# fskovbo/OptimalControlMPS

Hardware: AMD Instinct MI355X
Metric: Hessian-rows/sec (getHessian incl. psi/xi/divT/xiH precompute), N=5 d=4 chi=80 T=2.0 (higher is better)
Workload: dtype c128/f64

## Files before the change

### optimalcontrolmps_amd/csrc/fast.hpp

```cpp
#pragma once

namespace ocg {
namespace fastp {

constexpr int kMaxOps = 16;
constexpr int kMaxDm = 4;
constexpr int kMaxDot = 16;
constexpr int kMaxGram = 4;
constexpr int kItTh = 2;
constexpr int kItF = 4;
constexpr int kItS = 4;
constexpr int kItMps = 4;

enum {
  kHNp = 0,
  kHNblk,
  kHBlk,
  kHLs,
  kHSite,
  kHSiteN,
  kHNops,
  kHZMps,
  kHZTh,
  kHZTg,
  kHZW,
  kHZX,
  kHZGt,
  kHZPh,
  kHZTot,
  kHNint,
  kHCentre,
  kHThZ,
  kHXsZ,
  kHOps,
  kHdrInts = kHOps + kMaxOps
};
enum { kOpGate = 0, kOpGaugeR = 1, kOpGaugeL = 2 };
enum {
  kOhKind = 0, kOhK, kOhDir, kOhMode,
  kOhLonely, kOhClosing, kOhNth, kOhNewBond,
  kOhMat,
  kOhGate,
  kOhNsec, kOhT,
  kOhNgrp, kOhMaxr,
  kOhO1, kOhNo1,
  kOhEq,
  kOhSecQ,
  kOhF, kOhNf,
  kOhS, kOhNs,
  kOhDot,
  kOhGrp = 24,
  kOpHdr = kOhGrp + 32
};

static_assert(kOhGrp % 4 == 0 && kOhNewBond < 8, "b128 reads of the op header");

constexpr int kOvMaxE = 128;
constexpr int kOvMaxP = 6;
enum {
  kOvL = 0, kOvQ1, kOvP, kOvNp, kOvNblk,
  kOvMaxSite,
  kOvMaxEn,
  kOvD,
  kOvEo,
  kOvEn,
  kOvPo,
  kOvSb,
  kOvElo,
  kOvEl,
  kOvLs,
  kOvBlk,
  kOvNint,
  kOvHdr = 20
};
}
}
```

### optimalcontrolmps_amd/csrc/fast_chain.hpp

```cpp
#pragma once

#include "engine_device.hpp"
#include "fast.hpp"

namespace ocg {

struct FastChain {
  using CH = Chain<64>;
  const OcgParams& P;
  const int lane;
  const bool act;
  lzp MP, TH, TG, WB, XS, GT, PH;
  LDS double *LAM, *SIG, *SIGI, *MCB, *MCF;
  LDS int* MCE;
  LDS int *DIM, *BOF, *KQ, *WIDX, *PL;
  int np, nblk, o_blk, o_ls, o_site, o_siten, nops, centre_open;
  int thz, xsz;
  double ph_u = __builtin_nan("");
  int ph_dir = -1;
  int dims_epoch = 0, bof_epoch = -1;
  int trace_op = -1;
  double m_bytes = 0, m_flops = 0;
  LDS double* PROF = nullptr;
  unsigned long long pf_last = 0;
  int pf_cur = 0;
  __device__ __forceinline__ void pf(int cat) {
#ifdef OCG_PROFILE
    if (threadIdx.x == 0 && PROF) {
      const unsigned long long t = __builtin_amdgcn_s_memtime();
      if (pf_last) PROF[pf_cur] += double(t - pf_last);
      pf_last = t;
      pf_cur = cat;
    }
#else
    (void)cat;
#endif
  }
  __device__ __forceinline__ void cnt(int slot, double v) {
#ifdef OCG_PROFILE
    if (threadIdx.x == 0 && PROF) PROF[slot] += v;
#else
    (void)slot;
    (void)v;
#endif
  }

  __device__ OCG_INLINE FastChain(const OcgParams& P_, char* base, const int* gplan, LDS double* prof = nullptr)
      : P(P_), lane(threadIdx.x & 63), act(threadIdx.x < 64), PROF(prof) {
    using namespace fastp;
    if (!gplan) return;
    np = gplan[kHNp]; nblk = gplan[kHNblk]; o_blk = gplan[kHBlk]; o_ls = gplan[kHLs]; o_site = gplan[kHSite];
    o_siten = gplan[kHSiteN]; nops = gplan[kHNops]; centre_open = gplan[kHCentre];
    thz = gplan[kHThZ]; xsz = gplan[kHXsZ];
    lzp cb{(LDS double*)base};
    MP = cb + gplan[kHZMps]; TH = cb + gplan[kHZTh]; TG = cb + gplan[kHZTg]; WB = cb + gplan[kHZW];
    XS = cb + gplan[kHZX]; GT = cb + gplan[kHZGt]; PH = cb + gplan[kHZPh];
    LDS double* db = (cb + gplan[kHZTot]).p;
    LAM = db; SIG = db + 64; SIGI = db + 128;
    MCB = db + 200; MCF = db + 200 + fastp::kMaxOps;
    LDS int* ib = (LDS int*)(db + 200 + 2 * fastp::kMaxOps);
    MCE = ib; ib += fastp::kMaxOps;
    auto al = [](int x) { return (x + 3) & ~3; };
    DIM = ib; ib += al(P.nsq);
    BOF = ib; ib += al(nblk);
    KQ = ib; ib += 64;
    WIDX = ib; ib += 64;
    ib += 4;
    PL = ib;
  }
  __device__ __forceinline__ void wsync() const {
    __builtin_amdgcn_fence(__ATOMIC_RELEASE, "workgroup");
    __builtin_amdgcn_wave_barrier();
    __builtin_amdgcn_fence(__ATOMIC_ACQUIRE, "workgroup");
  }
  __device__ __forceinline__ static i4 ld4(const LDS int* p) { return *(const LDS i4*)p; }
  __device__ __forceinline__ static int uni(int v) { return __builtin_amdgcn_readfirstlane(v); }
  __device__ OCG_INLINE void init(const int* gplan, const zc* gf, const zc* gb) {
    if (!act) return;
    const int ni = gplan[fastp::kHNint];
    for (int i = lane; i < ni; i += 64) PL[i] = gplan[i];
    for (int i = lane; i < P.gtotal; i += 64) { GT[i] = gf[i]; GT[P.gtotal + i] = gb[i]; }
    if (lane < fastp::kMaxOps) MCE[lane] = -1;
    if (lane == 0) {
      WB[64] = c2(1.0, 0.0);
      MP[np] = c2(0.0, 0.0);
      TH[thz] = c2(0.0, 0.0);
      TG[thz] = c2(0.0, 0.0);
      XS[xsz] = c2(0.0, 0.0);
    }
    wsync();
  }
  __device__ __forceinline__ int dim(int b, int q) const { return (q < 0 || q > P.Q) ? 0 : DIM[b * P.Q1 + q]; }

  __device__ OCG_INLINE void block_offsets() {
    if (bof_epoch == dims_epoch) return;
    int carry = 0;
    for (int b0 = 0; b0 < nblk; b0 += 64) {
      const int b = b0 + lane, bb = b < nblk ? b : nblk - 1;
      const i4 t = ld4(PL + o_blk + 4 * bb);
      const int sz = b < nblk ? DIM[t[1]] * DIM[t[2]] : 0;
      const int inc = wscan(sz);
      if (b < nblk) BOF[b] = carry + inc - sz;
      carry += rdlane(inc, 63);
    }
    bof_epoch = dims_epoch;
    wsync();
  }
  template <class PI, class PZ>
  __device__ OCG_INLINE void load(const PI* gdims, const PZ* gdata) {
    if (!act) return;
    pf(10);
    for (int i = lane; i < P.nsq; i += 64) DIM[i] = gdims[i];
    ++dims_epoch;
    wsync();
    block_offsets();
    i4 d[fastp::kItMps];
#pragma unroll
    for (int it = 0; it < fastp::kItMps; ++it) {
      const int x = lane + 64 * it;
      d[it] = ld4(PL + o_ls + 4 * (x < np ? x : np - 1));
    }
#pragma unroll
    for (int it = 0; it < fastp::kItMps; ++it) {
      const int x = lane + 64 * it;
      const int dl = DIM[d[it][0] & 0xffff], dr = DIM[unsigned(d[it][0]) >> 16];
      const int b = d[it][1] & 0xffff, f = unsigned(d[it][1]) >> 16, a = d[it][2] & 0xff, c = unsigned(d[it][2]) >> 8;
      const bool ok = x < np && a < dl && c < dr;
      const int idx = d[it][3] + BOF[b] - BOF[f] + a * dr + c;
      zc v = c2(0.0, 0.0);
      if (ok) v = c2(gdata[idx].x, gdata[idx].y);
      if (x < np) MP[x] = v;
    }
    wsync();
  }
  __device__ OCG_INLINE void store(int* gdims, zc* gdata, bool wt = false) {
    if (!act) return;
    pf(10);
    block_offsets();
    for (int i = lane; i < P.nsq; i += 64) {
      if (wt) __hip_atomic_store(gdims + i, DIM[i], __ATOMIC_RELAXED, __HIP_MEMORY_SCOPE_AGENT);
      else gdims[i] = DIM[i];
    }
    i4 d[fastp::kItMps];
#pragma unroll
    for (int it = 0; it < fastp::kItMps; ++it) {
      const int x = lane + 64 * it;
      d[it] = ld4(PL + o_ls + 4 * (x < np ? x : np - 1));
    }
#pragma unroll
    for (int it = 0; it < fastp::kItMps; ++it) {
      const int x = lane + 64 * it;
      const int dl = DIM[d[it][0] & 0xffff], dr = DIM[unsigned(d[it][0]) >> 16];
      const int b = d[it][1] & 0xffff, f = unsigned(d[it][1]) >> 16, a = d[it][2] & 0xff, c = unsigned(d[it][2]) >> 8;
      const int idx = d[it][3] + BOF[b] - BOF[f] + a * dr + c;
      const zc v = MP[x < np ? x : 0];
      if (x < np && a < dl && c < dr) {
        if (wt) {
          double* dd = (double*)(gdata + idx);
          __hip_atomic_store(dd, v.x, __ATOMIC_RELAXED, __HIP_MEMORY_SCOPE_AGENT);
          __hip_atomic_store(dd + 1, v.y, __ATOMIC_RELAXED, __HIP_MEMORY_SCOPE_AGENT);
        } else {
          gdata[idx] = v;
        }
      }
    }
  }

  __device__ OCG_INLINE void model_totals(double& b, double& f) const {
    b = wsum(m_bytes);
    f = wsum(m_flops);
  }
  __device__ OCG_INLINE void model_gate(int o, int i1) {
    using namespace fastp;
    if (uni(MCE[o]) == dims_epoch) {
      if (lane == 0) {
        m_bytes += MCB[o];
        m_flops += MCF[o];
      }
      return;
    }
    const int p = P.p, Q = P.Q, Q1 = P.Q1, q = lane < Q1 ? lane : 0;
    const LDS int* d0 = DIM + (i1 - 1) * Q1;
    const LDS int* d1 = DIM + i1 * Q1;
    const LDS int* d2 = DIM + (i1 + 1) * Q1;
    int l[6], a[6], r[6];
#pragma unroll
    for (int n = 0; n < 6; ++n) {
      const int qm = q - n, qp = q + n;
      const bool okm = n < p && qm >= 0, okp = n < p && qp <= Q;
      const int lm = d0[okm ? qm : 0], ap = d1[okp ? qp : 0], rp = d2[okp ? qp : 0];
      l[n] = okm ? lm : 0;
      a[n] = okp ? ap : 0;
      r[n] = okp ? rp : 0;
    }
    int R = 0, C = 0, u = 0;
    const int m = a[0], dl = l[0];
#pragma unroll
    for (int n = 0; n < 6; ++n) {
      R += l[n];
      C += r[n];
      u += dl * a[n] + m * r[n];
    }
    double fl = 0.0, by = 0.0;
    if (lane < Q1) {
      if (R == 0 || C == 0) { R = 0; C = 0; }
      const double Rd = R, Cd = C, nn = R < C ? R : C;
      fl = 8.0 * (Rd * Cd * m + Rd * Cd * p + nn * nn * (R > C ? Rd : Cd) + 2.0 * Rd * Cd * m);
      by = 32.0 * double(u);
    }
    if (lane == 0) by += 16.0 * P.gtotal;
    const double bt = wsum(by), ft = wsum(fl);
    if (lane == 0) {
      m_bytes += bt;
      m_flops += ft;
      MCB[o] = bt;
      MCF[o] = ft;
      MCE[o] = dims_epoch;
    }
  }

  __device__ OCG_INLINE void theta(const LDS int* oh) {
    using namespace fastp;
    pf(0);
    const int nth = uni(oh[kOhNth]);
    if (nth <= 64) theta_it<1>(oh, nth);
    else theta_it<kItTh>(oh, nth);
    wsync();
  }
  template <int IT>
  __device__ OCG_INLINE void theta_it(const LDS int* oh, int nth) {
    using namespace fastp;
    const LDS int* md = PL + uni(oh[kOhMat]);
    int d0[IT], d1[IT];
#pragma unroll
    for (int it = 0; it < IT; ++it) {
      const int e = lane + 64 * it, ee = e < nth ? e : nth - 1;
      d0[it] = md[2 * ee];
      d1[it] = md[2 * ee + 1];
    }
#pragma unroll
    for (int it = 0; it < IT; ++it) {
      const int e = lane + 64 * it;
      const int x1 = d0[it] & 0xffff, x2 = unsigned(d0[it]) >> 16, dm = d1[it] & 0xff, drc = unsigned(d1[it]) >> 8;
      const int dmc = dm > 0 ? dm - 1 : 0;
      zc acc = c2(0.0, 0.0);
#pragma unroll
      for (int b = 0; b < kMaxDm; ++b) {
        const int bb = b < dmc ? b : dmc;
        const zc a = MP[b < dm ? x1 + b : np], v = MP[x2 + bb * drc];
        cacc(acc, a, v);
      }
      if (e < nth) TH[e] = acc;
    }
  }
  __device__ OCG_INLINE void gate(const LDS int* oh, int forward) {
    using namespace fastp;
    pf(1);
    const int mode = uni(oh[kOhMode]), lonely = uni(oh[kOhLonely]);
    if (uni(oh[kOhNth]) <= 64) gate_mode<1>(oh, forward, mode, lonely);
    else gate_mode<kItTh>(oh, forward, mode, lonely);
    wsync();
  }
  template <int IT>
  __device__ OCG_INLINE void gate_mode(const LDS int* oh, int forward, int mode, int lonely) {
    if (mode == 0) {
      if (lonely & 1) gate_body<1, 2, IT>(oh, forward);
      else gate_body<1, 0, IT>(oh, forward);
    } else {
      if (lonely & 2) gate_body<2, 1, IT>(oh, forward);
      else gate_body<0, 1, IT>(oh, forward);
    }
  }
  template <int PRE, int POST, int IT>
  __device__ OCG_INLINE void gate_body(const LDS int* oh, int forward) {
    using namespace fastp;
    const int p = P.p, nth = uni(oh[kOhNth]);
    const LDS int* gd = PL + uni(oh[kOhGate]);
    lzp g0 = GT + (forward ? 0 : P.gtotal);
    lzp UF = PH, UT = PH + p, UFF = PH + 2 * p, UTT = PH + 2 * p + p * p;
    i4 d[IT];
#pragma unroll
    for (int it = 0; it < IT; ++it) {
      const int e = lane + 64 * it;
      d[it] = ld4(gd + 4 * (e < nth ? e : nth - 1));
    }
#pragma unroll
    for (int it = 0; it < IT; ++it) {
      const int e = lane + 64 * it;
      const unsigned h = d[it][0];
      const int sz = (h >> 16) & 15, lo = (h >> 20) & 15, a1 = (h >> 24) & 15, a2 = h >> 28, D = a1 + a2;
      lzp g = g0 + int(h & 0xffff);
      zc acc = c2(0.0, 0.0);
#pragma unroll
      for (int x = 0; x < 6; ++x) {
        const int xx = x < sz ? x : sz - 1;
        const int n1 = lo + xx, n2 = D - n1;
        const int ad = (unsigned(d[it][1 + (x >> 1)]) >> (16 * (x & 1))) & 0xffff;
        zc z = TH[x < sz ? ad : thz];
        if (PRE == 1) z = cmul(z, UFF[n1 * p + n2]);
        if (PRE == 2) z = cmul(z, UF[n2]);
        const zc gx = g[xx];
        cacc(acc, gx, z);
      }
      if (POST == 1) acc = cmul(acc, UTT[a1 * p + a2]);
      if (POST == 2) acc = cmul(acc, UT[a2]);
      if (e < nth) TG[e] = acc;
    }
  }
  __device__ OCG_INLINE void matcopy(const LDS int* oh) {
    using namespace fastp;
    pf(7);
    const int nth = uni(oh[kOhNth]);
    if (nth <= 64) matcopy_it<1>(oh, nth);
    else matcopy_it<kItTh>(oh, nth);
    wsync();
  }
  template <int IT>
  __device__ OCG_INLINE void matcopy_it(const LDS int* oh, int nth) {
    using namespace fastp;
    const LDS int* src = PL + uni(oh[kOhMat]);
    int s[IT];
#pragma unroll
    for (int it = 0; it < IT; ++it) {
      const int e = lane + 64 * it;
      s[it] = src[e < nth ? e : nth - 1];
    }
#pragma unroll
    for (int it = 0; it < IT; ++it) {
      const int e = lane + 64 * it;
      const zc v = MP[s[it]];
      if (e < nth) TH[e] = v;
    }
  }

  __device__ OCG_INLINE void decompose(const LDS int* oh, lzp M, int dir, double cutoff, int maxm, bool normalize) {
    using namespace fastp;
    pf(2);
    const i4 h2 = ld4(oh + 8), h3 = ld4(oh + 12), h4 = ld4(oh + 16), h5 = ld4(oh + 20);
    const int newb = uni(oh[kOhNewBond]);
    const int nsec = uni(h2[kOhNsec - 8]), T = uni(h2[kOhT - 8]), maxr = uni(h3[kOhMaxr - 12]),
              no1 = uni(h3[kOhNo1 - 12]), o_o1 = uni(h3[kOhO1 - 12]), o_eq = uni(h4[kOhEq - 16]),
              o_secq = uni(h4[kOhSecQ - 16]), o_f = uni(h4[kOhF - 16]), nf = uni(h4[kOhNf - 16]),
              dot = uni(h5[kOhDot - 20]);
    const int g = lane >> 4, i = (lane >> 2) & 3, j = lane & 3, rb = lane & ~15;
    const i4 ga = ld4(oh + kOhGrp + 8 * g), gb = ld4(oh + kOhGrp + 8 * g + 4);
    const i4 o1 = ld4(PL + o_o1 + 4 * (lane < no1 ? lane : 0));
    const bool ae = lane < T;
    const i4 eq = ld4(PL + o_eq + 4 * (ae ? lane : 0));
    const int sqe = PL[o_secq + (lane < nsec ? lane : 0)];
    const int at_q = newb * P.Q1 + (sqe & 255);
    const int dold = DIM[at_q];
    const bool used = ga[0] >= 0;
    const int n = used ? ga[1] : 0, side = ga[2], tho = ga[3], R = gb[0], C = gb[1], eoff = gb[2];
    const bool valid = i < n && j < n;
    zc gv = c2(0.0, 0.0);
    double lam1 = 0.0;
    {
      const int len = used ? (side == 0 ? C : R) : 0, st = side == 0 ? 1 : C;
      const int bi = side == 0 ? tho + (i < n ? i : 0) * C : tho + (i < n ? i : 0);
      const int bj = side == 0 ? tho + (j < n ? j : 0) * C : tho + (j < n ? j : 0);
      const int len1 = lane < no1 ? o1[1] : 0, b1 = o1[0], s1 = o1[2];
      switch ((dot + 1) >> 1) {
        case 0: case 1: gram_dots<2>(M, len, st, bi, bj, len1, b1, s1, gv, lam1); break;
        case 2: gram_dots<4>(M, len, st, bi, bj, len1, b1, s1, gv, lam1); break;
        case 3: gram_dots<6>(M, len, st, bi, bj, len1, b1, s1, gv, lam1); break;
        case 4: gram_dots<8>(M, len, st, bi, bj, len1, b1, s1, gv, lam1); break;
        case 5: gram_dots<10>(M, len, st, bi, bj, len1, b1, s1, gv, lam1); break;
        case 6: gram_dots<12>(M, len, st, bi, bj, len1, b1, s1, gv, lam1); break;
        case 7: gram_dots<14>(M, len, st, bi, bj, len1, b1, s1, gv, lam1); break;
        default: gram_dots<kMaxDot>(M, len, st, bi, bj, len1, b1, s1, gv, lam1); break;
      }
      if (side == 1) gv.y = -gv.y;
    }
    if (!valid) gv = c2(0.0, 0.0);
    zc w = c2(i == j ? 1.0 : 0.0, 0.0);
    pf(3);
    if (maxr > 0) jacobi(gv, w, valid, i, j, rb, n, maxr);
    cnt(22, 1.0);
    pf(4);
    if (used) WB[16 * g + 4 * i + j] = w;
    if (valid && i == j) LAM[eoff + i] = gv.x > 0 ? gv.x : 0.0;
    if (lane < no1) LAM[o1[3]] = lam1;
    wsync();
    const double lam = ae ? LAM[lane] : 0.0;
    const int i_e = eq[1], eo_e = eq[2], n_e = eq[3] & 255, bound = unsigned(eq[3]) >> 8;
    double lt[kMaxGram];
#pragma unroll
    for (int t = 0; t < kMaxGram; ++t) lt[t] = CH::bperm(lam, ((eo_e + t) & 63) << 2);
    int jb = 0;
#pragma unroll
    for (int t = 0; t < kMaxGram; ++t)
      jb += (ae & (t < n_e) & (t != i_e) & ((lt[t] > lam) | ((lt[t] == lam) & (t < i_e)))) ? 1 : 0;
    const double total = wsum(lam);
    const double cut = cutoff * total, floor_ = 1e-30 * total;
    bool disc = false;
    if (T <= maxm) {
      const double thr = fmax(cut, floor_);
      const bool small = ae && (lam < thr || lam <= floor_);
      unsigned long long Mk = __ballot(small);
      pf(18);
      cnt(17, __popcll(Mk));
      if (Mk) {
        const int nbig = T - __popcll(Mk);
        double S = lam;
        int rs = 0;
        while (Mk) {
          const int f = __ffsll((long long)Mk) - 1;
          Mk &= Mk - 1;
          const double lf = rdlane(lam, f);
          rs += (lf > lam || (lf == lam && f < lane)) ? 1 : 0;
          if (f != lane && (lf < lam || (lf == lam && f > lane))) S += lf;
        }
        disc = small && nbig + rs >= 1 && (S < cut || lam <= floor_);
      }
    } else {
      int rk = 0;
      for (int f = 0; f < T; ++f) {
        const double lf = rdlane(lam, f);
        rk += (lf > lam || (lf == lam && f < lane)) ? 1 : 0;
      }
      const int dst = ((T - 1 - rk) & 63) << 2;
      const long long lb = __double_as_longlong(lam);
      const unsigned lo = unsigned(__builtin_amdgcn_ds_permute(dst, int(lb)));
      const unsigned hi = unsigned(__builtin_amdgcn_ds_permute(dst, int(lb >> 32)));
      const double v = __longlong_as_double((long long)(((unsigned long long)hi << 32) | lo));
      const int jpos = T - 1 - lane;
      const double vv = lane < T ? v : 0.0;
      const double suf = wscan(vv);
      const bool d2 = lane < T && jpos >= 1 && (jpos >= maxm || suf < cut || vv <= floor_);
      const int m = T - __popcll(__ballot(d2));
      disc = ae && rk >= m;
    }
    pf(16);
    const bool kept = ae && !disc && jb < bound;
    if (kept) {
      const double sq = sqrt(lam);
      WIDX[eo_e + jb] = i_e;
      SIG[eo_e + jb] = sq;
      SIGI[eo_e + jb] = sq > 0 ? 1.0 / sq : 0.0;
    }
    const double kw = wsum(kept ? lam : 0.0);
    {
      const unsigned long long K = __ballot(kept);
      const int eo = (sqe >> 8) & 255, ns = (sqe >> 16) & 15;
      const int kq = __popcll((K >> eo) & ((1ull << ns) - 1));
      bool changed = false;
      if (lane < nsec) {
        changed = dold != kq;
        KQ[lane] = kq;
        DIM[at_q] = kq;
      }
      if (__ballot(changed)) ++dims_epoch;
    }
    wsync();
    pf(5);
    const double inv = (normalize && kw > 1e-32) ? 1.0 / sqrt(kw) : 1.0;
    if (nf <= 64) factors<1>(o_f, nf, M, dir, inv);
    else if (nf <= 128) factors<2>(o_f, nf, M, dir, inv);
    else if (nf <= 192) factors<3>(o_f, nf, M, dir, inv);
    else factors<kItF>(o_f, nf, M, dir, inv);
  }

  template <int IF>
  __device__ OCG_INLINE void factors(int o_f, int nf, lzp M, int dir, double inv) {
    using namespace fastp;
    i4 fd[IF];
#pragma unroll
    for (int it = 0; it < IF; ++it) {
      const int e = lane + 64 * it;
      fd[it] = ld4(PL + o_f + 4 * (e < nf ? e : nf - 1));
    }
    int kqs[IF], wvv[IF];
    double sg[IF], isg[IF];
    zc mv[IF][kMaxGram];
#pragma unroll
    for (int it = 0; it < IF; ++it) {
      const int w0 = fd[it][0], w1 = fd[it][1], w2 = fd[it][2];
      const int s = (w0 >> 16) & 15, jj = (w0 >> 20) & 15, eo = w2 & 255;
      const bool exact = (w2 >> 12) & 1;
      const int mb = w1 & 0xffff, terms = (w1 >> 16) & 31, ms = unsigned(w1) >> 21;
      kqs[it] = KQ[s];
      wvv[it] = WIDX[eo + jj];
      sg[it] = SIG[eo + jj];
      isg[it] = SIGI[eo + jj];
#pragma unroll
      for (int x = 0; x < kMaxGram; ++x) mv[it][x] = M[(exact || x >= terms) ? thz : mb + x * ms];
    }
    zc out[IF];
    int dst[IF];
#pragma unroll
    for (int it = 0; it < IF; ++it) {
      const int e = lane + 64 * it;
      const int w0 = fd[it][0], w1 = fd[it][1], w2 = fd[it][2], wbse = fd[it][3];
      const int dest = w0 & 0xffff, jj = (w0 >> 20) & 15;
      const bool isx = (w0 >> 24) & 1, scr = (w0 >> 25) & 1;
      const bool exact = (w2 >> 12) & 1;
      const int terms = exact ? 1 : (w1 >> 16) & 31;
      const int tc = terms > 0 ? terms - 1 : 0;
      const bool live = jj < kqs[it] && e < nf;
      const int wvc = live ? wvv[it] : 0;
      const int base = exact ? w1 : wbse;
      const double cs = isx ? 1.0 : -1.0;
      zc wp[kMaxGram];
#pragma unroll
      for (int x = 0; x < kMaxGram; ++x) {
        const zc t = WB[base + 4 * (x < tc ? x : tc) + wvc];
        wp[x] = c2(t.x, cs * t.y);
      }
      zc acc = c2(0.0, 0.0);
#pragma unroll
      for (int x = 0; x < kMaxGram; ++x) cacc(acc, mv[it][x], wp[x]);
      const double sig = sg[it];
      const zc we = wp[0];
      const bool scl = isx ? dir == kFromright : dir == kFromleft;
      const bool orth = isx ? dir == kFromleft : dir == kFromright;
      const double f = exact ? (scl ? sig * inv : 1.0) : (orth ? (sig > 0 ? isg[it] : 0.0) : inv);
      const zc r = cscale(exact ? we : acc, f);
      out[it] = live ? r : c2(0.0, 0.0);
      dst[it] = e < nf ? (dest | (scr ? 0x10000 : 0)) : -1;
    }
    pf(23);
#pragma unroll
    for (int it = 0; it < IF; ++it)
      if (dst[it] >= 0) ((dst[it] >> 16) ? XS : MP)[dst[it] & 0xffff] = out[it];
    wsync();
  }

  template <int K>
  __device__ __forceinline__ void gram_dots(lzp M, int len, int st, int bi, int bj, int len1, int b1, int s1, zc& gv,
                                            double& lam1) const {
    zc a[K], b[K], z[K];
#pragma unroll
    for (int c = 0; c < K; ++c) {
      const bool in = c < len, in1 = c < len1;
      a[c] = M[in ? bi + c * st : thz];
      b[c] = M[in ? bj + c * st : thz];
      z[c] = M[in1 ? b1 + c * s1 : thz];
    }
#pragma unroll
    for (int c = 0; c < K; ++c) {
      cacc(gv, a[c], cconj(b[c]));
      lam1 += cabs2(z[c]);
    }
  }

  __device__ __forceinline__ void jrot_role(zc bv, double app, double aqq, bool live, bool up, zc& jd, zc& jo,
                                            double& ds) const {
    const double mb = fmax(fabs(bv.x), fabs(bv.y)), sz = fabs(app) + fabs(aqq);
    const bool resc = live && (mb < 1e-120 || mb > 1e120 || sz > 1e120);
    double sc = 1.0;
    if (__ballot(resc)) {
      sc = resc ? ldexp(1.0, -ilogb(fmax(mb, sz))) : 1.0;
      bv = cscale(bv, sc);
      app *= sc;
      aqq *= sc;
    }
    const double r2 = live ? bv.x * bv.x + bv.y * bv.y : 1.0;
    const double rinv = CH::rsq_ref(r2), r = r2 * rinv;
    const double D = aqq - app, sg = D >= 0 ? 1.0 : -1.0;
    const double x = fma(D, D, 4.0 * r2);
    const double E = fabs(D) + x * CH::rsq_ref(x);
    const double h = CH::rsq_ref(fma(E, E, 4.0 * r2));
    const double c = E * h, s = sg * 2.0 * r * h;
    const double ex = bv.x * rinv, ey = bv.y * rinv;
    const double sh = sg * 2.0 * r2 * CH::rcp_ref(E * sc);
    jd = up ? c2(c, 0.0) : c2(ex * c, -ey * c);
    jo = up ? c2(ex * -s, -ey * -s) : c2(s, 0.0);
    ds = up ? -sh : sh;
    jd = live ? jd : c2(1.0, 0.0);
    jo = live ? jo : c2(0.0, 0.0);
    ds = live ? ds : 0.0;
  }

  __device__ OCG_INLINE void jacobi(zc& g, zc& w, bool valid, int i, int j, int rb, int n, int maxr) {
    auto at = [&](int r, int c) { return (rb + r * 4 + c) << 2; };
    double di = CH::bperm(g.x, at(i, i)), dj = CH::bperm(g.x, at(j, j));
    int arow[3], acol[3];
    bool zp[3];
#pragma unroll
    for (int rnd = 0; rnd < 3; ++rnd) {
      const int k = rnd + 1;
      int pi = i, pj = j;
      if (rnd < maxr && valid) {
        if ((i ^ k) < n) pi = i ^ k;
        if ((j ^ k) < n) pj = j ^ k;
      }
      arow[rnd] = at(i, pi);
      acol[rnd] = at(j, pj);
      zp[rnd] = pi == j && i != j;
    }
    const bool up = i < j, dg = i == j;
    int sweep = 0, nr = 0;
    bool done = false;
    for (; sweep < 40; ++sweep) {
      bool flag = false;
#pragma unroll
      for (int rnd = 0; rnd < 3; ++rnd) {
        if (rnd >= maxr) break;
        if (__ballot(valid && up && CH::jneed(cabs2(g), di, dj)) == 0) {
          done = true;
          break;
        }
        ++nr;
        const zc g01 = CH::xcol(g, rnd), g10 = CH::xrow(g, rnd);
        const zc g11 = CH::xrow(g01, rnd), w1 = CH::xcol(w, rnd);
        const zc bv = up ? g : g11;
        const double app = up ? di : dj, aqq = up ? dj : di;
        const bool need = CH::jneed(cabs2(bv), app, aqq);
        zc jd, jo;
        double ds;
        jrot_role(bv, app, aqq, need && !dg, up, jd, jo, ds);
        const zc jdc = CH::bpermz(jd, acol[rnd]), joc = CH::bpermz(jo, acol[rnd]);
        const zc jdr = CH::bpermz(jd, arow[rnd]), jor = CH::bpermz(jo, arow[rnd]);
        const double dsc = CH::bperm(ds, acol[rnd]), dsr = CH::bperm(ds, arow[rnd]);
        zc wn = cmul(w, jdc);
        cacc(wn, w1, joc);
        zc r0 = cmul(g, jdc);
        cacc(r0, g01, joc);
        zc r1 = cmul(g10, jdc);
        cacc(r1, g11, joc);
        zc out = cjmul(jdr, r0);
        cjacc(out, jor, r1);
        const double dj2 = dj + dsc, di2 = di + dsr;
        out = (zp[rnd] && need) ? c2(0.0, 0.0) : out;
        out = dg ? c2(dj2, 0.0) : out;
        if (rnd == maxr - 1) flag = valid && up && CH::jneed(cabs2(out), di2, dj2);
        g = out;
        w = wn;
        di = di2;
        dj = dj2;
      }
      if (done || __ballot(flag) == 0) break;
    }
    if (sweep == 40 && lane == 0 && P.err) atomicOr(P.err, OCG_ERR_JACOBI);
    cnt(21, 1.0);
    cnt(20, double(sweep + 1));
    cnt(30, double(nr));
#ifdef OCG_FAST_TRACE
    if (lane == 0) printf("[jacobi] op %d sweeps %d rounds %d\n", trace_op, sweep + 1, nr);
#endif
  }

  __device__ OCG_INLINE void neighbour(const LDS int* oh) {
    using namespace fastp;
    pf(25);
    const int ns = uni(oh[kOhNs]), kind = uni(oh[kOhKind]);
    if (ns <= 64) neighbour_it<1>(oh, ns, kind);
    else if (ns <= 128) neighbour_it<2>(oh, ns, kind);
    else neighbour_it<kItS>(oh, ns, kind);
  }
  template <int IT>
  __device__ OCG_INLINE void neighbour_it(const LDS int* oh, int ns, int kind) {
    using namespace fastp;
    const LDS int* sl = PL + uni(oh[kOhS]);
    i4 d[IT];
#pragma unroll
    for (int it = 0; it < IT; ++it) {
      const int e = lane + 64 * it;
      d[it] = ld4(sl + 4 * (e < ns ? e : ns - 1));
    }
    zc acc[IT];
#pragma unroll
    for (int it = 0; it < IT; ++it) {
      const int x1 = d[it][0] & 0xffff, x2 = unsigned(d[it][0]) >> 16, len = d[it][1] & 0xffff,
                s2 = unsigned(d[it][1]) >> 16;
      const int lc = len > 0 ? len - 1 : 0;
      acc[it] = c2(0.0, 0.0);
#pragma unroll
      for (int b = 0; b < kMaxDm; ++b) {
        const int bb = b < lc ? b : lc;
        const bool in = b < len;
        const zc a = (kind == kOpGaugeR) ? zc(XS[in ? x1 + b : xsz]) : zc(MP[in ? x1 + b : np]);
        const zc v = (kind == kOpGaugeR) ? zc(MP[x2 + bb * s2]) : zc(XS[x2 + bb * s2]);
        cacc(acc[it], a, v);
      }
    }
    wsync();
#pragma unroll
    for (int it = 0; it < IT; ++it)
      if (lane + 64 * it < ns) MP[d[it][2]] = acc[it];
    wsync();
  }

  __device__ __forceinline__ static void sincos_q(double x, double& s, double& c) {
    constexpr double s3 = -1.0 / 6.0, s5 = 1.0 / 120.0, s7 = -1.0 / 5040.0, s9 = 1.0 / 362880.0,
                     s11 = -1.0 / 39916800.0, s13 = 1.0 / 6227020800.0, s15 = -1.0 / 1307674368000.0,
                     s17 = 1.0 / 355687428096000.0;
    constexpr double c2_ = -0.5, c4 = 1.0 / 24.0, c6 = -1.0 / 720.0, c8 = 1.0 / 40320.0, c10 = -1.0 / 3628800.0,
                     c12 = 1.0 / 479001600.0, c14 = -1.0 / 87178291200.0, c16 = 1.0 / 20922789888000.0;
    const double z = x * x;
    const double ps = fma(z, fma(z, fma(z, fma(z, fma(z, fma(z, fma(z, s17, s15), s13), s11), s9), s7), s5), s3);
    const double pc = fma(z, fma(z, fma(z, fma(z, fma(z, fma(z, fma(z, c16, c14), c12), c10), c8), c6), c4), c2_);
    s = fma(x * z, ps, x);
    c = fma(z, pc, 1.0);
  }

  __device__ OCG_INLINE void step(double ufrom, double uto, int forward, bool final_gauge = true) {
    using namespace fastp;
    if (!act) return;
    pf(29);
    const int p = P.p;
    const double tau = forward ? P.dt : -P.dt;
    {
      const double ta = -0.25 * tau;
      const int a = lane / p, b = lane - a * p;
      const double n1 = lane < p ? double(lane) * double(lane - 1) : 0.0;
      const double n2 = lane < p * p ? double(a) * double(a - 1) + double(b) * double(b - 1) : 0.0;
      const double xf1 = ta * ufrom * n1, xt1 = ta * uto * n1, xf2 = ta * ufrom * n2, xt2 = ta * uto * n2;
      const bool big = fmax(fmax(fabs(xf1), fabs(xt1)), fmax(fabs(xf2), fabs(xt2))) > 0.78;
      double sf1, cf1, st1, ct1, sf2, cf2, st2, ct2;
      if (__ballot(big) == 0) {
        sincos_q(xf1, sf1, cf1);
        sincos_q(xt1, st1, ct1);
        sincos_q(xf2, sf2, cf2);
        sincos_q(xt2, st2, ct2);
      } else {
        sincos(xf1, &sf1, &cf1);
        sincos(xt1, &st1, &ct1);
        sincos(xf2, &sf2, &cf2);
        sincos(xt2, &st2, &ct2);
      }
      if (lane < p) {
        PH[lane] = c2(cf1, sf1);
        PH[p + lane] = c2(ct1, st1);
      }
      if (lane < p * p) {
        PH[2 * p + lane] = c2(cf2, sf2);
        PH[2 * p + p * p + lane] = c2(ct2, st2);
      }
    }
    ph_u = uto;
    ph_dir = forward;
    wsync();
    for (int o = 0; o < nops; ++o) {
      const LDS int* oh = PL + PL[kHOps + o];
      const i4 h0 = ld4(oh), h1 = ld4(oh + 4);
      if (uni(h1[1]) && !final_gauge) continue;
      const int kind = uni(h0[0]), dir = uni(h0[2]);
      trace_op = o;
      if (kind == kOpGate) {
        pf(12);
        model_gate(o, uni(h0[1]));
        theta(oh);
        gate(oh, forward);
        decompose(oh, TG, dir, P.cutoff, P.maxm, true);
      } else {
        matcopy(oh);
        decompose(oh, TH, dir, OCG_GAUGE_CUTOFF, 1 << 30, false);
        neighbour(oh);
      }
    }
    pf(9);
    const int centre = final_gauge ? 1 : centre_open;
    const int s1a = PL[o_site + 1], s1b = PL[o_site + 2];
    for (int x = s1a + lane; x < s1b; x += 64) MP[x] = cmul(MP[x], PH[p + PL[o_siten + x - s1a]]);
    wsync();
    const int ca = PL[o_site + centre], cb = PL[o_site + centre + 1];
    double acc = 0.0;
    zc v[kItMps];
#pragma unroll
    for (int it = 0; it < kItMps; ++it) {
      const int x = ca + lane + 64 * it;
      v[it] = MP[x < cb ? x : ca];
      if (x < cb) acc += cabs2(v[it]);
    }
    const double n2 = wsum(acc);
    if (n2 > 0) {
      const double f = 1.0 / sqrt(n2);
#pragma unroll
      for (int it = 0; it < kItMps; ++it) {
        const int x = ca + lane + 64 * it;
        if (x < cb) MP[x] = cscale(v[it], f);
      }
    }
    wsync();
  }
};

}
```

### optimalcontrolmps_amd/csrc/fast_plan.hpp

```cpp
#pragma once

#include <algorithm>
#include <cstdio>
#include <cstdlib>
#include <string>
#include <vector>

#include "engine.hpp"
#include "fast.hpp"

namespace ocg_host {

struct FastPlanBuild {
  std::vector<int> plan;
  std::string why_not;
};

inline FastPlanBuild build_fast_plan(const OcgParams& P, const std::vector<int>& md) {
  using namespace ocg::fastp;
  FastPlanBuild out;
  const int L = P.L, p = P.p, Q = P.Q, Q1 = P.Q1;
  auto fail = [&](const std::string& m) {
    out.plan.clear();
    out.why_not = m;
    return out;
  };
  if (P.imag) return fail("imaginary-time steps use the general engine");
  if (p > 6) return fail("local dimension above 6");
  if (Q1 > 64) return fail("more than 64 sectors");
  auto D = [&](int b, int q) { return (b < 0 || b > L || q < 0 || q > Q) ? 0 : md[size_t(b) * Q1 + q]; };
  for (int b = 0; b <= L; ++b)
    for (int q = 0; q <= Q; ++q)
      if (D(b, q) > kMaxDm) return fail("bond sector bound above the unrolled maximum");
  std::vector<int> I(kHdrInts, 0);
  auto pad = [&]() {
    while (I.size() & 3) I.push_back(0);
    return int(I.size());
  };
  auto push4 = [&](int a, int b, int c, int d) { I.push_back(a); I.push_back(b); I.push_back(c); I.push_back(d); };
  std::vector<int> poff(size_t(L + 2) * Q1 * p, -1), sbase(L + 2, 0);
  int np = 0;
  std::vector<int> blk_k, blk_q, blk_n;
  for (int k = 1; k <= L; ++k) {
    sbase[k] = np;
    for (int q = 0; q <= Q; ++q)
      for (int n = 0; n < p && q + n <= Q; ++n) {
        const int dl = D(k - 1, q), dr = D(k, q + n);
        if (dl == 0 || dr == 0) continue;
        poff[(size_t(k) * Q1 + q) * p + n] = np;
        blk_k.push_back(k); blk_q.push_back(q); blk_n.push_back(n);
        np += dl * dr;
      }
  }
  sbase[L + 1] = np;
  if (np > 64 * kItMps) return fail("padded MPS above the unrolled maximum");
  auto PO = [&](int k, int q, int n) {
    return (k < 1 || k > L || q < 0 || q > Q || n < 0 || n >= p) ? -1 : poff[(size_t(k) * Q1 + q) * p + n];
  };
  const int nblk = int(blk_k.size());
  if (nblk > 4095) return fail("too many blocks");
  std::vector<int> first(nblk);
  for (int b = 0; b < nblk; ++b) {
    first[b] = b;
    while (first[b] > 0 && blk_k[first[b] - 1] == blk_k[b]) --first[b];
  }
  const int o_blk = pad();
  for (int b = 0; b < nblk; ++b) {
    const int k = blk_k[b], q = blk_q[b], n = blk_n[b];
    push4(k | (q << 8) | (n << 16), (k - 1) * Q1 + q, k * Q1 + q + n, first[b]);
  }
  const int o_ls = pad();
  for (int b = 0; b < nblk; ++b) {
    const int k = blk_k[b], q = blk_q[b], n = blk_n[b];
    for (int a = 0; a < D(k - 1, q); ++a)
      for (int c = 0; c < D(k, q + n); ++c)
        push4(((k - 1) * Q1 + q) | ((k * Q1 + q + n) << 16), b | (first[b] << 16), a | (c << 8), P.site_base[k]);
  }
  const int o_site = pad();
  for (int k = 0; k <= L + 1; ++k) I.push_back(sbase[k]);
  const int o_siten = pad();
  for (int b = 0; b < nblk; ++b)
    if (blk_k[b] == 1)
      for (int x = 0; x < D(0, blk_q[b]) * D(1, blk_q[b] + blk_n[b]); ++x) I.push_back(blk_n[b]);

  struct Op { int kind, k, dir, mode, lonely, closing; };
  std::vector<Op> ops;
  {
    int centre = 1;
    bool mfl = true;
    for (int g = 0; g < P.ngates; ++g) {
      const int i1 = P.gate_i1[g], i2 = i1 + 1;
      const bool more = g + 1 < P.ngates;
      const int ni1 = more ? P.gate_i1[g + 1] : 0, ni2 = ni1 + 1;
      const int dir = (more && ni1 >= i2) ? 0 : 1;
      Op o{kOpGate, i1, dir, mfl ? 0 : 1, 0, 0};
      if (mfl) o.lonely = (i2 == L && L % 2 == 0) ? 1 : 0;
      else o.lonely = (L % 2 != 0 && i2 == L) ? 2 : 0;
      ops.push_back(o);
      centre = dir == 0 ? i2 : i1;
      const int target = !more ? 1 : (dir == 0 ? ni1 : ni2);
      while (centre != target) {
        if (centre < target) { ops.push_back({kOpGaugeR, centre, 0, 0, 0, more ? 0 : 1}); ++centre; }
        else { ops.push_back({kOpGaugeL, centre, 1, 0, 0, more ? 0 : 1}); --centre; }
      }
      if (more && (i2 == ni1 || i1 == ni2)) mfl = false;
    }
  }
  if (int(ops.size()) > kMaxOps) return fail("too many step operations");
  int thmax = 1, xsmax = 1, last_gate = 0;
  std::vector<int> op_off;
  for (const Op& o : ops) {
    if (o.kind == kOpGate) last_gate = o.k;
    int bl, br, prow, pcol;
    if (o.kind == kOpGate) { bl = o.k - 1; br = o.k + 1; prow = p; pcol = p; }
    else if (o.kind == kOpGaugeR) { bl = o.k - 1; br = o.k; prow = p; pcol = 1; }
    else { bl = o.k - 1; br = o.k; prow = 1; pcol = p; }
    const int newb = (o.kind == kOpGaugeL) ? o.k - 1 : o.k;
    std::vector<int> R(Q1, 0), C(Q1, 0), THO(Q1 + 1, 0);
    std::vector<std::vector<int>> RS(Q1, std::vector<int>(p, -1)), CS(Q1, std::vector<int>(p, -1));
    for (int q = 0; q <= Q; ++q) {
      for (int n = 0; n < prow; ++n) {
        const int d = D(bl, q - n);
        if (d > 0) { RS[q][n] = R[q]; R[q] += d; }
      }
      for (int n = 0; n < pcol; ++n) {
        const int d = D(br, q + n);
        if (d > 0) { CS[q][n] = C[q]; C[q] += d; }
      }
      if (R[q] == 0 || C[q] == 0) { R[q] = 0; C[q] = 0; }
      THO[q + 1] = THO[q] + R[q] * C[q];
    }
    const int nth = THO[Q1];
    thmax = std::max(thmax, nth);
    if (nth > 64 * kItTh) return fail("matricisation above the unrolled maximum");
    const int hpos = pad();
    op_off.push_back(hpos);
    I.resize(I.size() + kOpHdr, 0);
    auto setH = [&](int f, int v) { I[hpos + f] = v; };
    setH(kOhKind, o.kind); setH(kOhK, o.k); setH(kOhDir, o.dir); setH(kOhMode, o.mode);
    setH(kOhLonely, o.lonely); setH(kOhClosing, o.closing); setH(kOhNth, nth); setH(kOhNewBond, newb);
    setH(kOhMat, pad());
    for (int q = 0; q <= Q; ++q) {
      if (R[q] == 0) continue;
      for (int nr = 0; nr < prow; ++nr) {
        if (RS[q][nr] < 0) continue;
        for (int a = 0; a < D(bl, q - nr); ++a)
          for (int nc = 0; nc < pcol; ++nc) {
            if (CS[q][nc] < 0) continue;
            for (int c = 0; c < D(br, q + nc); ++c) {
              if (o.kind == kOpGate) {
                const int dm = D(o.k, q);
                const int x1 = dm > 0 ? PO(o.k, q - nr, nr) + a * dm : 0;
                const int drc = D(o.k + 1, q + nc);
                const int x2 = dm > 0 ? PO(o.k + 1, q, nc) + c : 0;
                I.push_back(x1 | (x2 << 16));
                I.push_back(dm | (drc << 8));
              } else if (o.kind == kOpGaugeR) {
                I.push_back(PO(o.k, q - nr, nr) + a * D(o.k, q) + c);
              } else {
                I.push_back(PO(o.k, q, nc) + a * D(o.k, q + nc) + c);
              }
            }
          }
      }
    }
    if (o.kind == kOpGate) {
      setH(kOhGate, pad());
      for (int q = 0; q <= Q; ++q) {
        if (R[q] == 0) continue;
        for (int a1 = 0; a1 < p; ++a1) {
          if (RS[q][a1] < 0) continue;
// ... 11 lines not shown
                    return fail("internal: gate input outside Θ");
                  const int ad = THO[qs] + (RS[qs][n1] + a) * C[qs] + CS[qs][n2] + c;
                  if (ad > 65535) return fail("Θ offset above 16 bits");
                  w[1 + x / 2] |= ad << (16 * (x & 1));
                }
                push4(w[0], w[1], w[2], w[3]);
              }
            }
        }
      }
    }
    std::vector<int> sq, secn(Q1, 0), seco(Q1, -1), secside(Q1, 0), secgrp(Q1, -1), seceoff(Q1, 0);
    int ngrp = 0, T = 0, maxn = 0;
    for (int q = 0; q <= Q; ++q) {
      if (R[q] == 0) continue;
      const int n = std::min(R[q], C[q]);
      if (n > kMaxGram) return fail("Gram block above the register Jacobi's order");
      if (std::max(R[q], C[q]) > kMaxDot) return fail("Gram dot product above the unrolled maximum");
      int grp = -1;
      if (n >= 2) {
        if (ngrp >= 4) return fail("more than four Gram blocks of order >= 2");
        grp = ngrp++;
      }
      seco[q] = int(sq.size());
      int side = R[q] < C[q] ? 0 : (R[q] > C[q] ? 1 : 0);
      if (R[q] == C[q] && o.kind == kOpGaugeR) side = 1;
      secn[q] = n; secside[q] = side; secgrp[q] = grp; seceoff[q] = T;
      sq.push_back(q);
      T += n;
      maxn = std::max(maxn, n);
    }
    const int nsec = int(sq.size());
    int maxdot = 1;
    for (int q : sq) maxdot = std::max(maxdot, std::max(R[q], C[q]));
    setH(kOhDot, maxdot);
    if (nsec > 15) return fail("more than 15 sectors");
    if (T > 64) return fail("more than 64 eigenvalues per decomposition");
    setH(kOhNsec, nsec); setH(kOhT, T); setH(kOhNgrp, ngrp);
    setH(kOhMaxr, maxn >= 3 ? 3 : (maxn == 2 ? 1 : 0));
    for (int g = 0; g < 4; ++g) I[hpos + kOhGrp + 8 * g] = -1;
    for (int s = 0; s < nsec; ++s) {
      const int q = sq[s], g = secgrp[q];
      if (g < 0) continue;
      int* G = &I[hpos + kOhGrp + 8 * g];
      G[0] = s; G[1] = secn[q]; G[2] = secside[q]; G[3] = THO[q]; G[4] = R[q]; G[5] = C[q]; G[6] = seceoff[q];
    }
    setH(kOhO1, pad());
    int no1 = 0;
    for (int s = 0; s < nsec; ++s) {
      const int q = sq[s];
      if (secn[q] != 1) continue;
      const bool rowv = secside[q] == 0;
      push4(THO[q], rowv ? C[q] : R[q], rowv ? 1 : C[q], seceoff[q]);
      ++no1;
    }
    setH(kOhNo1, no1);
    if (no1 > 64) return fail("too many order-1 sectors");
    setH(kOhEq, pad());
    for (int s = 0; s < nsec; ++s) {
      const int q = sq[s];
      for (int i = 0; i < secn[q]; ++i) push4(s, i, seceoff[q], secn[q] | (D(newb, q) << 8));
    }
    setH(kOhSecQ, pad());
    for (int s = 0; s < nsec; ++s) I.push_back(sq[s] | (seceoff[sq[s]] << 8) | (secn[sq[s]] << 16));
    std::vector<int> XS_off(Q1, 0), YS_off(Q1, 0);
    int xs_tot = 0, ys_tot = 0, nf = 0;
    setH(kOhF, pad());
    bool ok = true;
    auto pushf = [&](int dest, int q, int j, bool isx, bool scratch, int idx) {
      const int s = seco[q], n = secn[q], side = secside[q], g = secgrp[q];
      const bool exact = isx ? side == 0 : side == 1;
      const int wb = g >= 0 ? 16 * g : 64;
      int w1;
      if (exact) {
        w1 = wb + (g >= 0 ? 4 * idx : 0);
      } else if (isx) {
        w1 = (THO[q] + idx * C[q]) | (n << 16) | (1 << 21);
      } else {
        w1 = (THO[q] + idx) | (n << 16) | (C[q] << 21);
      }
      if (dest > 65535 || j > 15 || C[q] > 255 || THO[q] + idx * C[q] > 65535) ok = false;
      push4(dest | (s << 16) | (j << 20) | (isx ? 1 << 24 : 0) | (scratch ? 1 << 25 : 0), w1,
            seceoff[q] | (n << 8) | (exact ? 1 << 12 : 0), wb);
      ++nf;
    };
    for (int q = 0; q <= Q; ++q) {
      if (R[q] == 0) continue;
      const int jb = D(newb, q);
      if (o.kind == kOpGaugeL) {
        XS_off[q] = xs_tot;
        for (int row = 0; row < R[q]; ++row)
          for (int j = 0; j < jb; ++j) pushf(xs_tot + row * jb + j, q, j, true, true, row);
        xs_tot += R[q] * jb;
      } else {
        for (int nr = 0; nr < prow; ++nr) {
          if (RS[q][nr] < 0) continue;
          for (int a = 0; a < D(bl, q - nr); ++a)
            for (int j = 0; j < jb; ++j)
              pushf(PO(o.k, q - nr, nr) + a * D(o.k, q) + j, q, j, true, false, RS[q][nr] + a);
        }
      }
      if (o.kind == kOpGaugeR) {
        YS_off[q] = ys_tot;
        for (int j = 0; j < jb; ++j)
          for (int col = 0; col < C[q]; ++col) pushf(ys_tot + j * C[q] + col, q, j, false, true, col);
        ys_tot += jb * C[q];
      } else {
        const int site = (o.kind == kOpGate) ? o.k + 1 : o.k;
        for (int nc = 0; nc < pcol; ++nc) {
          if (CS[q][nc] < 0) continue;
          for (int j = 0; j < jb; ++j)
            for (int c = 0; c < D(br, q + nc); ++c)
              pushf(PO(site, q, nc) + j * D(site, q + nc) + c, q, j, false, false, CS[q][nc] + c);
        }
      }
    }
    if (!ok) return fail("factor descriptor overflow");
    if (nf > 64 * kItF) return fail("factor list above the unrolled maximum");
    setH(kOhNf, nf);
    xsmax = std::max(xsmax, std::max(xs_tot, ys_tot));
    if (o.kind != kOpGate) {
      setH(kOhS, pad());
      const int nb = (o.kind == kOpGaugeR) ? o.k + 1 : o.k - 1;
      int cnt = 0;
      for (int q = 0; q <= Q; ++q)
        for (int n = 0; n < p && q + n <= Q; ++n) {
          const int po = PO(nb, q, n);
          if (po < 0) continue;
          const int dl = D(nb - 1, q), dr = D(nb, q + n);
          for (int a = 0; a < dl; ++a)
            for (int c = 0; c < dr; ++c) {
              int x1, x2, len, s2;
              if (o.kind == kOpGaugeR) {
                len = R[q] == 0 ? 0 : D(o.k, q);
                x1 = YS_off[q] + a * C[q];
                x2 = po + c;
                s2 = dr;
              } else {
                const int qq = q + n;
                len = R[qq] == 0 ? 0 : D(o.k - 1, qq);
                x1 = po + a * dr;
                x2 = XS_off[qq] + c;
                s2 = D(newb, qq);
              }
              if (x1 > 65535 || x2 > 65535 || len > kMaxDm || s2 > 65535) return fail("product descriptor overflow");
              push4(x1 | (x2 << 16), len | (s2 << 16), po + a * dr + c, 0);
              ++cnt;
            }
        }
      if (cnt > 64 * kItS) return fail("gauge product above the unrolled maximum");
      setH(kOhNs, cnt);
    }
  }
  int zc_off = 0;
  auto take = [&](int n) { const int o = zc_off; zc_off += (n + 1) & ~1; return o; };
  I[kHNp] = np;
  I[kHNblk] = nblk;
  I[kHBlk] = o_blk;
  I[kHLs] = o_ls;
  I[kHSite] = o_site;
  I[kHSiteN] = o_siten;
  I[kHNops] = int(ops.size());
  for (size_t i = 0; i < ops.size(); ++i) I[kHOps + int(i)] = op_off[i];
  I[kHZMps] = take(np + 1);
  I[kHZTh] = take(thmax + 1);
  I[kHZTg] = take(thmax + 1);
  I[kHZW] = take(65);
  I[kHZX] = take(xsmax + 1);
  I[kHThZ] = thmax;
  I[kHXsZ] = xsmax;
  I[kHZGt] = take(2 * P.gtotal);
  I[kHZPh] = take(2 * p + 2 * p * p);
  I[kHZTot] = zc_off;
  I[kHCentre] = last_gate;
  pad();
  I[kHNint] = int(I.size());
  if (I.size() > 65535) return fail("plan too large");
  if (std::getenv("OCG_FAST_DUMP")) {
    std::fprintf(stderr, "[fast plan] np %d nblk %d ints %zu zc %d\n", np, nblk, I.size(), zc_off);
    for (size_t i = 0; i < ops.size(); ++i) {
      const int* h = &I[op_off[i]];
      std::fprintf(stderr, "[fast plan] op %zu kind %d k %d nth %d nsec %d T %d ngrp %d maxr %d dot %d no1 %d nf %d ns %d\n",
                   i, h[kOhKind], h[kOhK], h[kOhNth], h[kOhNsec], h[kOhT], h[kOhNgrp], h[kOhMaxr], h[kOhDot],
                   h[kOhNo1], h[kOhNf], h[kOhNs]);
    }
  }
  out.plan = I;
  return out;
}

constexpr int kFastDbl = 64 + 64 + 64 + 8 + 2 * ocg::fastp::kMaxOps;
inline int fast_int_words(const OcgParams& P, int nblk) {
  auto al = [](int x) { return (x + 3) & ~3; };
  return ocg::fastp::kMaxOps  + al(P.nsq) + al(nblk) + 64  + 64  + 4 ;
}
inline int fast_lds_bytes(const std::vector<int>& plan, const OcgParams& P) {
  using namespace ocg::fastp;
  return plan[kHZTot] * 16 + kFastDbl * 8 + (fast_int_words(P, plan[kHNblk]) + int(plan.size())) * 4;
}

inline std::vector<int> build_overlap_plan(const OcgParams& P, const std::vector<int>& md) {
  using namespace ocg::fastp;
  const int L = P.L, p = P.p, Q = P.Q, Q1 = P.Q1;
  auto D = [&](int b, int q) { return (b < 0 || b > L || q < 0 || q > Q) ? 0 : md[size_t(b) * Q1 + q]; };
  if (p > kOvMaxP) return {};
  std::vector<int> eo(size_t(L + 1) * Q1, 0), en(L + 1, 0);
  int maxen = 1;
  for (int b = 0; b <= L; ++b) {
    int o = 0;
    for (int q = 0; q <= Q; ++q) {
      if (D(b, q) > kMaxDm) return {};
      eo[size_t(b) * Q1 + q] = o;
      o += D(b, q) * D(b, q);
    }
    en[b] = o;
    maxen = std::max(maxen, o);
    if (o > kOvMaxE) return {};
  }
  if (en[0] != 1 || en[L] != 1) return {};
  std::vector<int> po(size_t(L + 2) * Q1 * p, -1), sb(L + 2, 0), ls, blk;
  int np = 0, maxsite = 1;
  for (int k = 1; k <= L; ++k) {
    sb[k] = np;
    const int b0 = int(blk.size());
    for (int q = 0; q <= Q; ++q)
      for (int n = 0; n < p && q + n <= Q; ++n) {
        const int dl = D(k - 1, q), dr = D(k, q + n);
        if (dl == 0 || dr == 0) continue;
        const int b = int(blk.size()), ri = (k - 1) * Q1 + q, ci = k * Q1 + q + n;
        blk.push_back(ri | (ci << 16));
        po[(size_t(k) * Q1 + q) * p + n] = np - sb[k];
        for (int a = 0; a < dl; ++a)
          for (int c = 0; c < dr; ++c) {
            ls.push_back(ri | (ci << 16));
            ls.push_back(b | (b0 << 16));
            ls.push_back(a | (c << 4) | (dl << 8) | (dr << 12) | (eo[size_t(k - 1) * Q1 + q] << 16));
            ls.push_back(P.site_base[k]);
          }
        np += dl * dr;
      }
    maxsite = std::max(maxsite, np - sb[k]);
  }
  sb[L + 1] = np;
  if (np == 0 || np > 4096 || int(blk.size()) > 32767 || (L + 1) * Q1 > 32767) return {};
  std::vector<int> elo(L + 2, 0), el;
  for (int b = 0; b <= L; ++b) {
    elo[b] = int(el.size());
    for (int q = 0; q <= Q; ++q)
      for (int c = 0; c < D(b, q); ++c)
        for (int d = 0; d < D(b, q); ++d) el.push_back(q | (c << 8) | (d << 12) | (D(b, q) << 16));
  }
  elo[L + 1] = int(el.size());
  std::vector<int> Dv(size_t(L + 1) * Q1);
  for (int b = 0; b <= L; ++b)
    for (int q = 0; q <= Q; ++q) Dv[size_t(b) * Q1 + q] = D(b, q);
  std::vector<int> I(kOvHdr, 0);
  auto sec = [&](int slot, const std::vector<int>& v) {
    while (I.size() & 3) I.push_back(0);
    I[slot] = int(I.size());
    I.insert(I.end(), v.begin(), v.end());
  };
  I[kOvL] = L;
  I[kOvQ1] = Q1;
  I[kOvP] = p;
  I[kOvNp] = np;
  I[kOvNblk] = int(blk.size());
  I[kOvMaxSite] = maxsite;
  I[kOvMaxEn] = maxen;
  sec(kOvD, Dv);
  sec(kOvEo, eo);
  sec(kOvEn, en);
  sec(kOvPo, po);
  sec(kOvSb, sb);
  sec(kOvElo, elo);
  sec(kOvEl, el);
  sec(kOvLs, ls);
  sec(kOvBlk, blk);
  while (I.size() & 3) I.push_back(0);
  I[kOvNint] = int(I.size());
  return I;
}
inline int overlap_lds_bytes(const std::vector<int>& I, const OcgParams& P, bool with_dH = false) {
  using namespace ocg::fastp;
  auto al = [](int x) { return (x + 3) & ~3; };
  const int ints = I[kOvNint] + 2 * al(P.nsq) + 2 * al(I[kOvNblk] + 1);
  int zs = 2 * (I[kOvNp] + 2) + (I[kOvMaxSite] + 2) + 2 * (I[kOvMaxEn] + 2);
  if (with_dH) zs += (I[kOvMaxSite] + 2) + 2 * (I[kOvMaxEn] + 2);
  return ints * 4 + zs * 16;
}

}
```

### optimalcontrolmps_amd/csrc/kernels.hpp

```cpp
#pragma once

#include "engine_device.hpp"
#include "fast_chain.hpp"
#include "fast_overlap.hpp"

namespace ocg {

__device__ __forceinline__ int* flat(LDS int* p) { return (int*)p; }
__device__ __forceinline__ zc* flat(lzp p) { return (zc*)(double*)p.p; }
__device__ __forceinline__ bool fast_on(const OcgParams& P) { return P.fplan != nullptr && !P.imag; }
__device__ __forceinline__ void publish_flag_wt(int* flag, int epoch, int* progress) {
  if (threadIdx.x < 64) {
#ifndef OCG_EMU
    asm volatile("s_waitcnt vmcnt(0)" ::: "memory");
#endif
    if (threadIdx.x == 0) {
      __hip_atomic_store(flag, epoch, __ATOMIC_RELAXED, __HIP_MEMORY_SCOPE_AGENT);
      __hip_atomic_fetch_add(progress, 1, __ATOMIC_RELAXED, __HIP_MEMORY_SCOPE_AGENT);
    }
  }
}

struct StatAcc {
  double bytes = 0, flops = 0, steps = 0;
};

#ifdef OCG_PROFILE
__device__ double g_ocg_prof[32];
#endif

template <class CH>
__device__ inline void flush_stats(CH& c, double* stats, double bytes, double flops, double steps) {
#ifdef OCG_PROFILE
  c.pf(12);
  if (threadIdx.x == 0)
    for (int i = 0; i < 32; ++i) atomicAdd(&g_ocg_prof[i], c.PROF[i]);
#endif
  if (threadIdx.x == 0 && stats) {
    atomicAdd(stats + 0, bytes);
    atomicAdd(stats + 1, flops);
    atomicAdd(stats + 2, steps);
  }
}

struct Pool {
  int* dims;
  zc* data;
};

#define SLOT_D(pool, P, s) ((pool).dims + (size_t)(s) * (P).nsq)
#define SLOT_X(pool, P, s) ((pool).data + (size_t)(s) * (P).cap)

template <int NT>
__device__ OCG_INLINE void body_trajectory(char* smem, OcgParams P, const zc* gf, const zc* gb, const int* md,
                                                   Pool pool, int slot_init, int slot_target, int psi_base0,
                                                   int xi_base0, const double* u0, int N, int which, double* stats,
                                                   int cs) {
  Chain<NT> c(P, smem);
  c.load_tables(gf, gb, md);
  int chain = (which == 3) ? (blockIdx.x & 1) : (which == 1 ? 0 : 1);
  const int kc = (which == 3) ? (blockIdx.x >> 1) : 0;
  const int psi_base = psi_base0 + kc * cs, xi_base = xi_base0 + kc * cs;
  const double* u = u0 + (size_t)kc * N;
  const int fwd = (chain == 0) ? 1 : 0;
  const int base = fwd ? psi_base : xi_base;
  const int src = fwd ? slot_init : slot_target;
  double bytes = 0, flops = 0;
  int t = fwd ? 0 : N - 1;
  if (fast_on(P)) {
    FastChain f(P, smem + P.fast_off, P.fplan, c.PROF);
    __syncthreads();
    f.init(P.fplan, gf, gb);
    f.load(SLOT_D(pool, P, src), SLOT_X(pool, P, src));
    f.store(SLOT_D(pool, P, base + t), SLOT_X(pool, P, base + t));
    for (int s = 0; s + 1 < N; ++s) {
      const int tn = fwd ? t + 1 : t - 1;
      f.step(u[t], u[tn], fwd, s + 2 == N);
      f.store(SLOT_D(pool, P, base + tn), SLOT_X(pool, P, base + tn));
      t = tn;
    }
    f.model_totals(bytes, flops);
    __syncthreads();
  } else {
    c.load(SLOT_D(pool, P, src), SLOT_X(pool, P, src));
    c.store(SLOT_D(pool, P, base + t), SLOT_X(pool, P, base + t));
    for (int s = 0; s + 1 < N; ++s) {
      const int tn = fwd ? t + 1 : t - 1;
      c.step(u[t], u[tn], fwd, s + 2 == N);
      c.store(SLOT_D(pool, P, base + tn), SLOT_X(pool, P, base + tn));
      t = tn;
    }
    c.model_totals(bytes, flops);
  }
  flush_stats(c, stats, bytes, flops, double(N - 1));
}

template <int NT>
__device__ OCG_INLINE void body_overlaps(char* smem, OcgParams P, const zc* gf, const zc* gb, const int* md,
                                                 Pool pool, const int* xs, const int* ys, int npairs, int with_dH,
                                                 zc* out, double* stats) {
  Chain<NT, true> c(P, smem);
  c.load_tables(gf, gb, md);
  int i = blockIdx.x;
  if (i >= npairs) return;
  c.load(SLOT_D(pool, P, ys[i]), SLOT_X(pool, P, ys[i]));
  zc r = c.overlap(SLOT_D(pool, P, xs[i]), SLOT_X(pool, P, xs[i]), with_dH);
  const double b = 32.0 * c.mps_used();
  if (threadIdx.x == 0) out[i] = r;
  flush_stats(c, stats, b, 8.0 * b / 16.0 * 4.0, 0.0);
}

__device__ inline OCG_INLINE void body_overlaps_pad(char* smem, OcgParams P, Pool pool, const int* xs, const int* ys,
                                                    int npairs, int with_dH, zc* out, double* stats) {
  FastOverlap o(P, smem, P.oplan, true);
  o.init(P.oplan);
  double b = 0;
  for (int i = blockIdx.x; i < npairs; i += gridDim.x) {
    const int ny = o.load(SLOT_D(pool, P, xs[i]), SLOT_X(pool, P, xs[i]), SLOT_D(pool, P, ys[i]),
                          SLOT_X(pool, P, ys[i]));
    const zc r = with_dH ? o.contract_dH(o.YP, P.dH) : o.contract(o.YP);
    b += 32.0 * ny;
    if (threadIdx.x == 0) out[i] = r;
    o.wsync();
  }
  if (threadIdx.x == 0 && stats) {
    atomicAdd(stats + 0, b);
    atomicAdd(stats + 1, 8.0 * b / 16.0 * 4.0);
  }
}

template <int NT>
__device__ OCG_INLINE void body_apply_dH(char* smem, OcgParams P, const zc* gf, const zc* gb, const int* md,
                                                 Pool pool, const int* in, const int* outs, int n, double* norms,
                                                 double* stats) {
  Chain<NT> c(P, smem);
  c.load_tables(gf, gb, md);
  int i = blockIdx.x;
  if (i >= n) return;
  c.load(SLOT_D(pool, P, in[i]), SLOT_X(pool, P, in[i]));
  const double b0 = 16.0 * c.mps_used();
  c.apply_dH();
  double n2 = c.site_norm2(1);
  c.store(SLOT_D(pool, P, outs[i]), SLOT_X(pool, P, outs[i]));
  const double b = b0 + 16.0 * c.mps_used();
  if (threadIdx.x == 0 && norms) norms[i] = sqrt(n2);
  flush_stats(c, stats, b, 8.0 * b, 0.0);
}

template <int NT>
__device__ OCG_INLINE void body_hessian_rows(char* smem, OcgParams P, const zc* gf, const zc* gb, const int* md, Pool pool,
                                  int psih_base, int xih_base, const int* rows, int nrows, const double* norms,
                                  const double* u, int N, const zc* divT, zc F, double* H, double* stats) {
  Chain<NT> c(P, smem);
  c.load_tables(gf, gb, md);
  int r = blockIdx.x;
  if (r >= nrows) return;
  const int i = rows[r];
  const double dt2 = P.dt * P.dt;
  const double normiH = norms[i];
  c.load(SLOT_D(pool, P, psih_base + i), SLOT_X(pool, P, psih_base + i));
  double bytes = 0, flops = 0;
  const bool fo = fast_on(P);
  FastChain f(P, smem + P.fast_off, P.fplan, c.PROF);
  const bool po = fo && P.oplan != nullptr;
  FastOverlap o(P, smem, po ? P.oplan : nullptr);
  if (fo) {
    if (po) {
      __syncthreads();
      o.init(P.oplan);
    }
    f.init(P.fplan, gf, gb);
    f.load(SLOT_D(pool, P, psih_base + i), SLOT_X(pool, P, psih_base + i));
  }
  for (int j = i; j + 1 < N; ++j) {
    if (j > i) {
      if (fo) {
        f.step(u[j - 1], u[j], 1, false);
        if (!po) {
          f.store(flat(c.DIMS), flat(c.A));
          __syncthreads();
          c.load(flat(c.DIMS), flat(c.A));
        }
      } else {
        c.step(u[j - 1], u[j], 1, false);
      }
    }
    zc ov;
    double used;
    if (po) {
      o.load(SLOT_D(pool, P, xih_base + j), SLOT_X(pool, P, xih_base + j), nullptr, nullptr);
      ov = o.contract(f.MP);
      used = o.compact_size(f.DIM);
    } else {
      ov = c.overlap(SLOT_D(pool, P, xih_base + j), SLOT_X(pool, P, xih_base + j), 0);
      used = c.mps_used();
    }
    if (threadIdx.x == 0) {
      zc di = divT[i], dj = divT[j];
      double v1 = (F.x * ov.x - F.y * ov.y) * (j > i ? normiH : 1.0);
      double v2 = -(di.x * dj.x + di.y * dj.y);
      double res = dt2 * (v1 + v2);
      H[(size_t)i * N + j] = res;
      if (j > i) H[(size_t)j * N + i] = res;
      bytes += 32.0 * used;
    }
  }
  double mb, mf;
  if (fo) f.model_totals(mb, mf);
  else c.model_totals(mb, mf);
  bytes += mb;
  flops += mf;
  flush_stats(c, stats, bytes, flops, double(N - 2 - i > 0 ? N - 2 - i : 0));
}

__device__ __forceinline__ void publish_flag(int* flag, int epoch, int* progress) {
  __threadfence();
  __syncthreads();
  if (threadIdx.x == 0) {
    __hip_atomic_store(flag, epoch, __ATOMIC_RELEASE, __HIP_MEMORY_SCOPE_AGENT);
    __hip_atomic_fetch_add(progress, 1, __ATOMIC_RELAXED, __HIP_MEMORY_SCOPE_AGENT);
  }
}
template <int NT>
__device__ OCG_INLINE bool await_flag(Chain<NT>& c, const int* flag, int epoch, int* err, const int* progress) {
  if (threadIdx.x == 0) {
    int ok = 1;
    long spins = 0;
    int seen = __hip_atomic_load(progress, __ATOMIC_RELAXED, __HIP_MEMORY_SCOPE_AGENT);
    while (__hip_atomic_load(flag, __ATOMIC_RELAXED, __HIP_MEMORY_SCOPE_AGENT) < epoch) {
      __builtin_amdgcn_s_sleep(32);
      const int now = __hip_atomic_load(progress, __ATOMIC_RELAXED, __HIP_MEMORY_SCOPE_AGENT);
      if (now != seen) {
        seen = now;
        spins = 0;
      }
      if (++spins > (1L << 24) || __hip_atomic_load(err, __ATOMIC_RELAXED, __HIP_MEMORY_SCOPE_AGENT)) {
        ok = 0;
        atomicOr(err, OCG_ERR_WATCHDOG);
        break;
      }
    }
    __atomic_thread_fence(__ATOMIC_ACQUIRE);
    c.ISCAL[15] = ok;
  }
  __syncthreads();
  const int ok = c.ISCAL[15];
  __syncthreads();
  return ok != 0;
}

template <int NT>
__device__ OCG_INLINE void body_pipeline(char* smem, OcgParams P, const zc* gf, const zc* gb, const int* md,
                                         Pool pool, int slot_init, int slot_target, int psi_base0, int xi_base0,
                                         int xih_base0, const double* u0, int N, const int* rows, int nrows,
                                         const int* rbase, Pool rs, double* rnorm0, int* flags0, int epoch, int* err,
                                         int nxw, double* stats, int K, int cs) {
  Chain<NT> c(P, smem);
  if (threadIdx.x == 0)
    c.ISCAL[14] = __hip_atomic_fetch_add(flags0 + K * (2 * N + 2), 1, __ATOMIC_RELAXED, __HIP_MEMORY_SCOPE_AGENT);
  __syncthreads();
  const int tk = c.ISCAL[14];
  __syncthreads();
  int kc, b;
  if (tk < 2 * K) { kc = tk >> 1; b = tk & 1; }
  else if (tk < 2 * K + K * nxw) { kc = (tk - 2 * K) / nxw; b = 2 + (tk - 2 * K) % nxw; }
  else { const int t = tk - 2 * K - K * nxw; kc = t % K; b = 2 + nxw + t / K; }
  const int psi_base = psi_base0 + kc * cs, xi_base = xi_base0 + kc * cs, xih_base = xih_base0 + kc * cs;
  const double* u = u0 + (size_t)kc * N;
  int* const flags = flags0 + (size_t)kc * (2 * N + 2);
  c.load_tables(gf, gb, md);
  int* const progress = flags + 2 * N;
  double bytes = 0, flops = 0, nsteps = 0;
  const bool fo = fast_on(P);
  FastChain f(P, smem + P.fast_off, P.fplan, c.PROF);
  if (fo && b < 2) {
    __syncthreads();
    f.init(P.fplan, gf, gb);
  }
  if (b < 2 && fo) {
    const int fwd = (b == 0) ? 1 : 0;
    const int base = fwd ? psi_base : xi_base;
    int* fl = flags + (fwd ? 0 : N);
    const int src = fwd ? slot_init : slot_target;
    f.load(SLOT_D(pool, P, src), SLOT_X(pool, P, src));
    int t = fwd ? 0 : N - 1;
    f.store(SLOT_D(pool, P, base + t), SLOT_X(pool, P, base + t), true);
    for (int s = 0; s + 1 < N; ++s) {
      const int tn = fwd ? t + 1 : t - 1;
      f.step(u[t], u[tn], fwd, s + 2 == N);
      publish_flag_wt(fl + t, epoch, progress);
      f.store(SLOT_D(pool, P, base + tn), SLOT_X(pool, P, base + tn), true);
      t = tn;
    }
    publish_flag_wt(fl + t, epoch, progress);
    nsteps = N - 1;
    f.model_totals(bytes, flops);
    __syncthreads();
    flush_stats(c, stats, bytes, flops, nsteps);
    return;
  }
  if (b < 2) {
    const int fwd = (b == 0) ? 1 : 0;
    const int base = fwd ? psi_base : xi_base;
    int* fl = flags + (fwd ? 0 : N);
    const int src = fwd ? slot_init : slot_target;
    c.load(SLOT_D(pool, P, src), SLOT_X(pool, P, src));
    int t = fwd ? 0 : N - 1;
    c.store(SLOT_D(pool, P, base + t), SLOT_X(pool, P, base + t));
    publish_flag(fl + t, epoch, progress);
    for (int s = 0; s + 1 < N; ++s) {
      const int tn = fwd ? t + 1 : t - 1;
      c.step(u[t], u[tn], fwd, s + 2 == N);
      c.store(SLOT_D(pool, P, base + tn), SLOT_X(pool, P, base + tn));
      publish_flag(fl + tn, epoch, progress);
      t = tn;
    }
    nsteps = N - 1;
  } else if (b < 2 + nxw) {
    for (int t = N - 1 - (b - 2); t >= 0; t -= nxw) {
      if (!await_flag(c, flags + N + t, epoch, err, progress)) return;
      c.load(SLOT_D(pool, P, xi_base + t), SLOT_X(pool, P, xi_base + t));
      c.apply_dH();
      c.store(SLOT_D(pool, P, xih_base + t), SLOT_X(pool, P, xih_base + t));
    }
  } else {
    const int r = b - 2 - nxw;
    if (r >= nrows) return;
    const int i = rows[r];
    if (!await_flag(c, flags + i, epoch, err, progress)) return;
    c.load(SLOT_D(pool, P, psi_base + i), SLOT_X(pool, P, psi_base + i));
    c.apply_dH();
    const double n2 = c.site_norm2(1);
    if (threadIdx.x == 0) rnorm0[(size_t)kc * nrows + r] = sqrt(n2);
    int k = kc * rbase[nrows] + rbase[r];
    c.store(SLOT_D(rs, P, k), SLOT_X(rs, P, k));
    if (fo) {
      __syncthreads();
      f.init(P.fplan, gf, gb);
      f.load(SLOT_D(rs, P, k), SLOT_X(rs, P, k));
      for (int j = i + 1; j + 1 < N; ++j) {
        f.step(u[j - 1], u[j], 1, false);
        ++k;
        f.store(SLOT_D(rs, P, k), SLOT_X(rs, P, k));
      }
      double fb, ff;
      f.model_totals(fb, ff);
      bytes += fb;
      flops += ff;
      __syncthreads();
    } else {
      for (int j = i + 1; j + 1 < N; ++j) {
        c.step(u[j - 1], u[j], 1, false);
        ++k;
        c.store(SLOT_D(rs, P, k), SLOT_X(rs, P, k));
      }
    }
    nsteps = N - 2 - i;
  }
  double mb, mf;
  c.model_totals(mb, mf);
  flush_stats(c, stats, bytes + mb, flops + mf, nsteps);
}

template <int NT>
__device__ OCG_INLINE void body_row_overlaps(char* smem, OcgParams P, const zc* gf, const zc* gb, const int* md,
                                             Pool pool, int xih_base0, const int* rows, int nrows, const int* rbase,
                                             Pool rs, const double* rnorm0, const zc* divT0, const zc* Fp, int N,
                                             double* H0, double* stats, int K, int cs) {
  Chain<NT, true> c(P, smem);
  c.load_tables(gf, gb, md);
  const int total = rbase[nrows];
  double b = 0;
  for (int g = blockIdx.x; g < K * total; g += gridDim.x) {
    const int kc = g / total, gl = g - kc * total;
    int lo = 0, hi = nrows - 1;
    while (lo < hi) {
      const int mid = (lo + hi + 1) >> 1;
      if (rbase[mid] <= gl) lo = mid;
      else hi = mid - 1;
    }
    const int r = lo, i = rows[r], j = i + (gl - rbase[r]);
    const int xih_base = xih_base0 + kc * cs;
    c.load(SLOT_D(rs, P, g), SLOT_X(rs, P, g));
    const zc ov = c.overlap(SLOT_D(pool, P, xih_base + j), SLOT_X(pool, P, xih_base + j), 0);
    b += 32.0 * c.mps_used();
    if (threadIdx.x == 0) {
      const zc* divT = divT0 + (size_t)kc * N;
      double* H = H0 + (size_t)kc * N * N;
      const zc F = Fp[kc], di = divT[i], dj = divT[j];
      const double v1 = (F.x * ov.x - F.y * ov.y) * (j > i ? rnorm0[(size_t)kc * nrows + r] : 1.0);
      const double v2 = -(di.x * dj.x + di.y * dj.y);
      const double res = P.dt * P.dt * (v1 + v2);
      H[(size_t)i * N + j] = res;
      if (j > i) H[(size_t)j * N + i] = res;
    }
    c.sync();
  }
  flush_stats(c, stats, b, 8.0 * b / 16.0 * 4.0, 0.0);
}

__device__ inline OCG_INLINE void body_row_overlaps_pad(char* smem, OcgParams P, Pool pool, int xih_base0,
                                                        const int* rows, int nrows, const int* rbase, Pool rs,
                                                        const double* rnorm0, const zc* divT0, const zc* Fp, int N,
                                                        double* H0, double* stats, int K, int cs) {
  FastOverlap o(P, smem, P.oplan);
  LDS int* RB = (LDS int*)(smem + P.ovl_bytes);
  LDS int* RW = RB + nrows + 1;
  o.init(P.oplan);
  for (int x = threadIdx.x; x <= nrows; x += 64) {
    RB[x] = rbase[x];
    if (x < nrows) RW[x] = rows[x];
  }
  o.wsync();
  const int total = RB[nrows];
  double b = 0;
  for (int g = blockIdx.x; g < K * total; g += gridDim.x) {
    const int kc = g / total, gl = g - kc * total;
    int lo = 0, hi = nrows - 1;
    while (lo < hi) {
      const int mid = (lo + hi + 1) >> 1;
      if (RB[mid] <= gl) lo = mid;
      else hi = mid - 1;
    }
    const int r = lo, i = RW[r], j = i + (gl - RB[r]);
    const int xih_base = xih_base0 + kc * cs;
    const zc* divT = divT0 + (size_t)kc * N;
    const zc F = Fp[kc], di = divT[i], dj = divT[j];
    const double rn = rnorm0[(size_t)kc * nrows + r];
    const int ny = o.load(SLOT_D(pool, P, xih_base + j), SLOT_X(pool, P, xih_base + j), SLOT_D(rs, P, g),
                          SLOT_X(rs, P, g));
    const zc ov = o.contract(o.YP);
    b += 32.0 * ny;
    if (threadIdx.x == 0) {
      double* H = H0 + (size_t)kc * N * N;
      const double v1 = (F.x * ov.x - F.y * ov.y) * (j > i ? rn : 1.0);
      const double v2 = -(di.x * dj.x + di.y * dj.y);
      const double res = P.dt * P.dt * (v1 + v2);
      H[(size_t)i * N + j] = res;
      if (j > i) H[(size_t)j * N + i] = res;
    }
    o.wsync();
  }
  if (threadIdx.x == 0 && stats) {
    atomicAdd(stats + 0, b);
    atomicAdd(stats + 1, 8.0 * b / 16.0 * 4.0);
  }
}

template <int NT>
__device__ OCG_INLINE void body_steps(char* smem, OcgParams P, const zc* gf, const zc* gb, const int* md,
                                              Pool pool, const int* slots, int n, const double* u, int u_stride,
                                              int nsteps, int forward, double* stats) {
  Chain<NT> c(P, smem);
  c.load_tables(gf, gb, md);
  int i = blockIdx.x;
  if (i >= n) return;
  double bytes = 0, flops = 0;
  const double* ui = u + (size_t)i * u_stride;
  if (fast_on(P)) {
    FastChain f(P, smem + P.fast_off, P.fplan, c.PROF);
    __syncthreads();
    f.init(P.fplan, gf, gb);
    f.load(SLOT_D(pool, P, slots[i]), SLOT_X(pool, P, slots[i]));
    for (int s = 0; s < nsteps; ++s) f.step(ui[s], ui[s + 1], forward);
    f.store(SLOT_D(pool, P, slots[i]), SLOT_X(pool, P, slots[i]));
    f.model_totals(bytes, flops);
    __syncthreads();
    flush_stats(c, stats, bytes, flops, double(nsteps));
    return;
  }
  c.load(SLOT_D(pool, P, slots[i]), SLOT_X(pool, P, slots[i]));
  for (int s = 0; s < nsteps; ++s) {
    c.step(ui[s], ui[s + 1], forward);
  }
  c.store(SLOT_D(pool, P, slots[i]), SLOT_X(pool, P, slots[i]));
  c.model_totals(bytes, flops);
  flush_stats(c, stats, bytes, flops, double(nsteps));
}


}
```

### optimalcontrolmps_amd/csrc/ocmps.hip

```cpp
#include <hip/hip_runtime.h>

#include <algorithm>
#include <cmath>
#include <complex>
#include <cstdio>
#include <cstdlib>
#include <cstring>
#include <string>
#include <vector>

#include "../../include/ocmps.h"
#include "engine.hpp"
#include "hbm.hpp"
#include "engine_device.hpp"
#include "params.hpp"
#include "fast_plan.hpp"
#include "observe.hpp"

using ocg::Chain;
using ocg::zc;
static inline zc mkz(double x, double y) { zc r; r.x = x; r.y = y; return r; }

#ifndef OCG_NT
#define OCG_NT 128
#endif
static constexpr int NT = OCG_NT;
static constexpr int kXiHWorkers = 12;

#include "kernels.hpp"
using ocg::Pool;

__global__ __launch_bounds__(NT) void k_trajectory(OcgParams P, const zc* gf, const zc* gb, const int* md,
                                                   Pool pool, int slot_init, int slot_target, int psi_base,
                                                   int xi_base, const double* u, int N, int which, double* stats,
                                                   int cs) {
  extern __shared__ __align__(16) char smem[];
  ocg::body_trajectory<NT>(smem, P, gf, gb, md, pool, slot_init, slot_target, psi_base, xi_base, u, N, which, stats,
                           cs);
}

__global__ __launch_bounds__(NT) void k_overlaps(OcgParams P, const zc* gf, const zc* gb, const int* md,
                                                 Pool pool, const int* xs, const int* ys, int npairs, int with_dH,
                                                 zc* out, double* stats) {
  extern __shared__ __align__(16) char smem[];
  ocg::body_overlaps<NT>(smem, P, gf, gb, md, pool, xs, ys, npairs, with_dH, out, stats);
}

__global__ __launch_bounds__(NT) void k_apply_dH(OcgParams P, const zc* gf, const zc* gb, const int* md,
                                                 Pool pool, const int* in, const int* outs, int n, double* norms,
                                                 double* stats) {
  extern __shared__ __align__(16) char smem[];
  ocg::body_apply_dH<NT>(smem, P, gf, gb, md, pool, in, outs, n, norms, stats);
}

__global__ __launch_bounds__(NT) void k_hessian_rows(OcgParams P, const zc* gf, const zc* gb, const int* md,
                                                     Pool pool, int psih_base, int xih_base, const int* rows,
                                                     int nrows, const double* norms, const double* u, int N,
                                                     const zc* divT, zc F, double* H, double* stats) {
  extern __shared__ __align__(16) char smem[];
  ocg::body_hessian_rows<NT>(smem, P, gf, gb, md, pool, psih_base, xih_base, rows, nrows, norms, u, N, divT, F, H,
                             stats);
}

__global__ __launch_bounds__(NT) void k_pipeline(OcgParams P, const zc* gf, const zc* gb, const int* md, Pool pool,
                                                 int slot_init, int slot_target, int psi_base, int xi_base,
                                                 int xih_base, const double* u, int N, const int* rows, int nrows,
                                                 const int* rbase, Pool rs, double* rnorm, int* flags, int epoch,
                                                 int* err, int nxw, double* stats, int K, int cs) {
  extern __shared__ __align__(16) char smem[];
  ocg::body_pipeline<NT>(smem, P, gf, gb, md, pool, slot_init, slot_target, psi_base, xi_base, xih_base, u, N, rows,
                         nrows, rbase, rs, rnorm, flags, epoch, err, nxw, stats, K, cs);
}

__global__ __launch_bounds__(NT) void k_row_overlaps(OcgParams P, const zc* gf, const zc* gb, const int* md,
                                                     Pool pool, int xih_base, const int* rows, int nrows,
                                                     const int* rbase, Pool rs, const double* rnorm,
                                                     const zc* divT, const zc* F, int N, double* H, double* stats,
                                                     int K, int cs) {
  extern __shared__ __align__(16) char smem[];
  ocg::body_row_overlaps<NT>(smem, P, gf, gb, md, pool, xih_base, rows, nrows, rbase, rs, rnorm, divT, F, N, H,
                             stats, K, cs);
}

__global__ __launch_bounds__(64) void k_row_overlaps_w(OcgParams P, const zc* gf, const zc* gb, const int* md,
                                                       Pool pool, int xih_base, const int* rows, int nrows,
                                                       const int* rbase, Pool rs, const double* rnorm,
                                                       const zc* divT, const zc* F, int N, double* H, double* stats,
                                                       int K, int cs) {
  extern __shared__ __align__(16) char smem[];
  ocg::body_row_overlaps<64>(smem, P, gf, gb, md, pool, xih_base, rows, nrows, rbase, rs, rnorm, divT, F, N, H,
                             stats, K, cs);
}

__global__ __launch_bounds__(64) void k_row_overlaps_pad(OcgParams P, Pool pool, int xih_base, const int* rows,
                                                         int nrows, const int* rbase, Pool rs, const double* rnorm,
                                                         const zc* divT, const zc* F, int N, double* H,
                                                         double* stats, int K, int cs) {
  extern __shared__ __align__(16) char smem[];
  ocg::body_row_overlaps_pad(smem, P, pool, xih_base, rows, nrows, rbase, rs, rnorm, divT, F, N, H, stats, K, cs);
}

__global__ __launch_bounds__(64) void k_overlaps_pad(OcgParams P, Pool pool, const int* xs, const int* ys, int n,
                                                     int with_dH, zc* out, double* stats) {
  extern __shared__ __align__(16) char smem[];
  ocg::body_overlaps_pad(smem, P, pool, xs, ys, n, with_dH, out, stats);
}

__global__ __launch_bounds__(NT) void k_steps(OcgParams P, const zc* gf, const zc* gb, const int* md,
                                              Pool pool, const int* slots, int n, const double* u, int u_stride,
                                              int nsteps, int forward, double* stats) {
  extern __shared__ __align__(16) char smem[];
  ocg::body_steps<NT>(smem, P, gf, gb, md, pool, slots, n, u, u_stride, nsteps, forward, stats);
}

__global__ __launch_bounds__(256) void k_project_hv(const double* Hu, const double* Vt, int N, int M, double* HV) {
#pragma clang fp contract(off)
  extern __shared__ __align__(16) char smem[];
  double* row = (double*)smem;
  const int k = blockIdx.x;
  for (int l = threadIdx.x; l < N; l += blockDim.x) row[l] = Hu[(size_t)k * N + l];
  __syncthreads();
  for (int j = threadIdx.x; j < M; j += blockDim.x) {
    double acc = 0.0;
    for (int l = 0; l < N; ++l) acc = acc + row[l] * Vt[(size_t)l * M + j];
    HV[(size_t)j * N + k] = acc;
  }
}
__global__ __launch_bounds__(256) void k_project_c(const double* V, const double* HV, int N, int M, double* Hc) {
#pragma clang fp contract(off)
  const int t = blockIdx.x * blockDim.x + threadIdx.x;
  if (t >= M * M) return;
  const int i = t / M, j = t % M;
  if (j < i) return;
  double acc = 0.0;
  for (int k = 0; k < N; ++k) acc = acc + V[(size_t)i * N + k] * HV[(size_t)j * N + k];
  Hc[(size_t)i * M + j] = acc;
  Hc[(size_t)j * M + i] = acc;
}

namespace {

thread_local std::string g_create_error;

struct KStat {
  double ms = 0;
  long launches = 0;
};

}

struct ocg_ctx {
  int device = 0;
  hbm_engine* hbm = nullptr;
  OcgParams P{};
  int lds_np = 0;
  int lds_ovl = 0;
  OcgParams Po() const {
    OcgParams q = P;
    q.fplan = nullptr;
    q.nplan = 0;
    q.plan_pe = 0;
    q.lds_bytes = lds_ovl;
    return q;
  }
  int plan_pe2 = 0, lds2 = 0;
  int lds_alias = 0;
  OcgParams Pa() const {
    OcgParams q = P;
    if (P.fplan && lds_alias > 0) {
      q.fast_off = 0;
      q.lds_bytes = lds_alias;
    }
    return q;
  }
  OcgParams P2() const {
    OcgParams q = P;
    if (P.fplan) return Pa();
    if (plan_pe2 >= 32) {
      q.plan_pe = plan_pe2;
      q.lds_bytes = lds2;
    } else {
      q.nplan = 0;
      q.plan_pe = 0;
      q.lds_bytes = lds_np;
    }
    return q;
  }
  OcgParams Pn() const {
    OcgParams q = P;
    q.fplan = nullptr;
    q.nplan = 0;
    q.plan_pe = 0;
    q.lds_bytes = lds_np;
    return q;
  }
  double J = 1.0;
  std::vector<int> md;
  std::string err;
  long pipe_runs = 0, pipe_fallbacks = 0, ckpt_runs = 0, ckpt_k = 0;
  hipStream_t stream = nullptr;
  hipEvent_t ev0 = nullptr, ev1 = nullptr;
  hipEvent_t evh[4] = {nullptr, nullptr, nullptr, nullptr};
  zc *d_gf = nullptr, *d_gb = nullptr;
  int* d_md = nullptr;
  Pool pool{nullptr, nullptr};
  int nslots = 0;
  double* d_stats = nullptr;
  int* d_idx = nullptr;
  int idx_cap = 0;
  double* d_u = nullptr;
  int u_cap = 0;
  zc* d_c = nullptr;
  int c_cap = 0;
  double* d_H = nullptr;
  size_t H_cap = 0;
  double* d_norms = nullptr;
  int norms_cap = 0;
  double* d_rnorm = nullptr;
  int rnorm_cap = 0;
  int* d_idx2 = nullptr;
  int idx2_cap = 0;
  Pool rs{nullptr, nullptr};
  size_t rs_cap = 0;
  char* h_pin = nullptr;
  size_t pin_cap = 0;
  int* d_flags = nullptr;
  int flags_cap = 0;
  int flags_N = -1, flags_K = -1;
  int epoch = 0;
  int* d_err = nullptr;
  int* d_rows = nullptr;
  int rows_cap = 0;
  double* d_proj = nullptr;
  size_t proj_cap = 0;
  zc* d_pc = nullptr;
  int pc_cap = 0;
  double* d_prn = nullptr;
  int prn_cap = 0;
  int* d_fplan = nullptr;
  int* d_oplan = nullptr;
  std::string fast_why;
  int N = 0;
  std::vector<double> u_psi, u_xi;
  bool have_states = false, have_psi = false, have_xi = false, have_xih = false;
  KStat kst[10];
  char* d_obs = nullptr;
  size_t obs_cap = 0;
  obs::Traffic obs_tr;
  int slot_init() const { return 0; }
  int slot_target() const { return 1; }
  int slot_tmp(int i) const { return 2 + i; }
  int psi_base() const { return 6; }
  int xi_base() const { return 6 + N; }
  int xih_base() const { return 6 + 2 * N; }
  int psih_base() const { return 6 + 3 * N; }
};

#define HIPCHK(ctx, expr)                                                               \
  do {                                                                                  \
    hipError_t e_ = (expr);                                                             \
    if (e_ != hipSuccess) {                                                             \
      (ctx)->err = std::string(#expr) + ": " + hipGetErrorString(e_);                   \
      return OCG_EHIP;                                                                  \
    }                                                                                   \
  } while (0)

static int fail(ocg_ctx* c, int code, const std::string& m) {
  c->err = m;
  return code;
}

static int upload_gates(ocg_ctx* c) {
  std::vector<double> gf, gb;
  ocg_host::gate_tables(c->P, c->J, gf, gb);
  const int off = c->P.gtotal;
  if (!c->d_gf) {
    HIPCHK(c, hipMalloc(&c->d_gf, sizeof(zc) * off));
    HIPCHK(c, hipMalloc(&c->d_gb, sizeof(zc) * off));
  }
  HIPCHK(c, hipMemcpyAsync(c->d_gf, gf.data(), sizeof(zc) * off, hipMemcpyHostToDevice, c->stream));
  HIPCHK(c, hipMemcpyAsync(c->d_gb, gb.data(), sizeof(zc) * off, hipMemcpyHostToDevice, c->stream));
  HIPCHK(c, hipStreamSynchronize(c->stream));
  return 0;
}

static int build_params(ocg_ctx* c, int L, int p, int npart, double tstep, double cutoff, int maxm) {
  std::string e = ocg_host::build_params(c->P, c->md, L, p, npart, tstep, cutoff, maxm);
  if (!e.empty()) return fail(c, e.find("too large") != std::string::npos ? OCG_ECAP : OCG_EINVAL, e);
  return 0;
}

static int ensure_slots(ocg_ctx* c, int nslots) {
  if (nslots <= c->nslots) return 0;
  int n = std::max(nslots, 2 * c->nslots);
  int* nd = nullptr;
  zc* nx = nullptr;
  HIPCHK(c, hipMalloc(&nd, sizeof(int) * size_t(n) * c->P.nsq));
  HIPCHK(c, hipMalloc(&nx, sizeof(zc) * size_t(n) * c->P.cap));
  HIPCHK(c, hipMemsetAsync(nd, 0, sizeof(int) * size_t(n) * c->P.nsq, c->stream));
  if (c->nslots) {
    HIPCHK(c, hipMemcpyAsync(nd, c->pool.dims, sizeof(int) * size_t(c->nslots) * c->P.nsq, hipMemcpyDeviceToDevice,
                             c->stream));
    HIPCHK(c, hipMemcpyAsync(nx, c->pool.data, sizeof(zc) * size_t(c->nslots) * c->P.cap, hipMemcpyDeviceToDevice,
                             c->stream));
  }
  HIPCHK(c, hipStreamSynchronize(c->stream));
  if (c->nslots) {
    (void)hipFree(c->pool.dims);
    (void)hipFree(c->pool.data);
  }
  c->pool.dims = nd;
  c->pool.data = nx;
  c->nslots = n;
  return 0;
}

template <class T>
static int ensure_buf(ocg_ctx* c, T*& ptr, int& cap, int n) {
  if (n <= cap) return 0;
  HIPCHK(c, hipStreamSynchronize(c->stream));
  if (ptr) (void)hipFree(ptr);
  ptr = nullptr;
  int m = std::max(n, 2 * cap);
  HIPCHK(c, hipMalloc(&ptr, sizeof(T) * size_t(m)));
  cap = m;
  return 0;
}

static int ensure_pin(ocg_ctx* c, size_t bytes) {
  if (bytes <= c->pin_cap) return 0;
  HIPCHK(c, hipStreamSynchronize(c->stream));
  const size_t m = std::max(bytes, 2 * c->pin_cap);
  if (c->h_pin) (void)hipHostFree(c->h_pin);
  c->h_pin = nullptr;
  c->pin_cap = 0;
  HIPCHK(c, hipHostMalloc((void**)&c->h_pin, m, hipHostMallocDefault));
  c->pin_cap = m;
  return 0;
}

static size_t nelem_of(const OcgParams& P, const int* dims, int k) {
  size_t s = 0;
  for (int q = 0; q < P.Q1; ++q)
    for (int n = 0; n < P.p && q + n <= P.Q; ++n) s += size_t(dims[(k - 1) * P.Q1 + q]) * dims[k * P.Q1 + q + n];
  return s;
}

static int validate_dims(ocg_ctx* c, const int* dims) {
  const OcgParams& P = c->P;
  if (dims[0] != 1) return fail(c, OCG_EINVAL, "bond 0 must be one state with q = 0");
  for (int q = 1; q < P.Q1; ++q)
    if (dims[q] != 0) return fail(c, OCG_EINVAL, "bond 0 must be one state with q = 0");
  for (int q = 0; q < P.Q1; ++q)
    if (dims[P.L * P.Q1 + q] != (q == P.Q ? 1 : 0))
      return fail(c, OCG_EINVAL, "bond L must be one state with q = Q (particle number mismatch?)");
  for (int b = 0; b <= P.L; ++b)
    for (int q = 0; q < P.Q1; ++q) {
      int v = dims[b * P.Q1 + q];
      if (v < 0) return fail(c, OCG_EINVAL, "negative bond dimension");
      if (v > c->md[b * P.Q1 + q])
        return fail(c, OCG_ECAP, "bond " + std::to_string(b) + " sector " + std::to_string(q) +
                                      " exceeds its Schmidt-rank bound");
    }
  return 0;
}

static int upload_mps(ocg_ctx* c, int slot, const int* dims, const double* data) {
  const OcgParams& P = c->P;
  if (int rc = validate_dims(c, dims)) return rc;
  std::vector<zc> buf(P.cap, mkz(0, 0));
  size_t off = 0;
  for (int k = 1; k <= P.L; ++k) {
    size_t n = nelem_of(P, dims, k);
    if (n > size_t(P.site_cap[k])) return fail(c, OCG_ECAP, "site tensor exceeds capacity");
    for (size_t i = 0; i < n; ++i) buf[P.site_base[k] + i] = mkz(data[2 * (off + i)], data[2 * (off + i) + 1]);
    off += n;
  }
  HIPCHK(c, hipMemcpyAsync(SLOT_D(c->pool, P, slot), dims, sizeof(int) * P.nsq, hipMemcpyHostToDevice, c->stream));
  HIPCHK(c, hipMemcpyAsync(SLOT_X(c->pool, P, slot), buf.data(), sizeof(zc) * P.cap, hipMemcpyHostToDevice,
                           c->stream));
  HIPCHK(c, hipStreamSynchronize(c->stream));
  return 0;
}

static int download_mps(ocg_ctx* c, int slot, int* dims, double* data, size_t cap, size_t* nelem) {
  const OcgParams& P = c->P;
  std::vector<int> d(P.nsq);
  std::vector<zc> buf(P.cap);
  HIPCHK(c, hipMemcpyAsync(d.data(), SLOT_D(c->pool, P, slot), sizeof(int) * P.nsq, hipMemcpyDeviceToHost, c->stream));
  HIPCHK(c, hipMemcpyAsync(buf.data(), SLOT_X(c->pool, P, slot), sizeof(zc) * P.cap, hipMemcpyDeviceToHost,
                           c->stream));
  HIPCHK(c, hipStreamSynchronize(c->stream));
  size_t tot = 0;
  for (int k = 1; k <= P.L; ++k) tot += nelem_of(P, d.data(), k);
  if (nelem) *nelem = tot;
  if (tot > cap) return fail(c, OCG_ECAP, "output buffer too small");
  std::memcpy(dims, d.data(), sizeof(int) * P.nsq);
  size_t off = 0;
  for (int k = 1; k <= P.L; ++k) {
    size_t n = nelem_of(P, d.data(), k);
    for (size_t i = 0; i < n; ++i) {
      data[2 * (off + i)] = buf[P.site_base[k] + i].x;
      data[2 * (off + i) + 1] = buf[P.site_base[k] + i].y;
    }
    off += n;
  }
  return 0;
}

static int begin_kernel(ocg_ctx* c) {
  HIPCHK(c, hipEventRecord(c->ev0, c->stream));
  return 0;
}
static int check_err(ocg_ctx* c) {
  int err = 0;
  HIPCHK(c, hipMemcpyAsync(&err, c->d_err, sizeof(int), hipMemcpyDeviceToHost, c->stream));
  HIPCHK(c, hipStreamSynchronize(c->stream));
  if (!err) return 0;
  HIPCHK(c, hipMemsetAsync(c->d_err, 0, sizeof(int), c->stream));
  HIPCHK(c, hipStreamSynchronize(c->stream));
  c->have_psi = c->have_xi = c->have_xih = false;
  std::string m;
  if (err & OCG_ERR_JACOBI) m += "eigensolver did not converge within its sweep cap; ";
  if (err & OCG_ERR_WATCHDOG) m += "pipeline watchdog: a consumer saw no producer progress for ~15 s; ";
  return fail(c, OCG_ENUM, m.empty() ? std::string("kernel error flag set") : m);
}

static int end_kernel(ocg_ctx* c, int kind) {
  HIPCHK(c, hipGetLastError());
  HIPCHK(c, hipEventRecord(c->ev1, c->stream));
  HIPCHK(c, hipEventSynchronize(c->ev1));
  float ms = 0;
  HIPCHK(c, hipEventElapsedTime(&ms, c->ev0, c->ev1));
  c->kst[kind].ms += ms;
  c->kst[kind].launches += 1;
  return check_err(c);
}

static int set_lds(ocg_ctx* c) {
  const int bytes = c->P.lds_bytes;
  HIPCHK(c, hipFuncSetAttribute((const void*)k_trajectory, hipFuncAttributeMaxDynamicSharedMemorySize, bytes));
  HIPCHK(c, hipFuncSetAttribute((const void*)k_overlaps, hipFuncAttributeMaxDynamicSharedMemorySize, bytes));
  HIPCHK(c, hipFuncSetAttribute((const void*)k_apply_dH, hipFuncAttributeMaxDynamicSharedMemorySize, bytes));
  HIPCHK(c, hipFuncSetAttribute((const void*)k_hessian_rows, hipFuncAttributeMaxDynamicSharedMemorySize, bytes));
  HIPCHK(c, hipFuncSetAttribute((const void*)k_steps, hipFuncAttributeMaxDynamicSharedMemorySize, bytes));
  HIPCHK(c, hipFuncSetAttribute((const void*)k_pipeline, hipFuncAttributeMaxDynamicSharedMemorySize, bytes));
  HIPCHK(c, hipFuncSetAttribute((const void*)k_row_overlaps, hipFuncAttributeMaxDynamicSharedMemorySize, bytes));
  HIPCHK(c, hipFuncSetAttribute((const void*)k_row_overlaps_w, hipFuncAttributeMaxDynamicSharedMemorySize, bytes));
  return 0;
}

static int finish_params(ocg_ctx* c) {
  if (c->P.gtotal <= 0) return fail(c, OCG_ESTATE, "internal: gate tables must be built before the LDS layout");
  c->P.nplan = 0;
  c->P.plan_pe = 0;
  c->lds_ovl = ocg::lds_layout_ovl(c->P, NT).bytes;
  ocg::LdsLayout l = ocg::lds_layout(c->P, NT);
  c->P.lds_bytes = l.bytes;
  c->lds_np = l.bytes;
  hipDeviceProp_t prop;
  HIPCHK(c, hipGetDeviceProperties(&prop, c->device));
  size_t limit = prop.sharedMemPerBlock;
  if (prop.maxSharedMemoryPerMultiProcessor > limit) limit = prop.maxSharedMemoryPerMultiProcessor;
  const char* np = std::getenv("OCG_NO_PLANS");
  const bool plans_off = np && np[0] && np[0] != '0';
  auto plan_fit = [&](size_t lim, int& bytes) {
    if (plans_off || !(c->P.cap < 65536 && c->P.thcap < 65536 && c->P.evcap < 4096)) return 0;
    OcgParams q = c->P;
    q.nplan = q.ngates + ocg_host::step_gauge_moves(q);
    q.plan_pe = 0;
    const int b0 = ocg::lds_layout(q, NT).bytes;
    q.plan_pe = 64;
    const int per = (ocg::lds_layout(q, NT).bytes - b0 + 63) / 64;
    const int want = std::max(q.th2cap, q.max_site_cap);
    q.plan_pe = std::min(want, per > 0 ? int((long(lim) - b0) / per) - 8 : 0);
    while (q.plan_pe >= 32 && size_t(ocg::lds_layout(q, NT).bytes) > lim) q.plan_pe -= 8;
    if (q.plan_pe < 32) return 0;
    bytes = ocg::lds_layout(q, NT).bytes;
    return q.plan_pe;
  };
  const int nplan = c->P.ngates + ocg_host::step_gauge_moves(c->P);
  int b1 = 0, b2 = 0;
  const int pe1 = plan_fit(limit, b1);
  c->plan_pe2 = plan_fit(std::max<size_t>(size_t(l.bytes), limit / 2), b2);
  c->lds2 = b2;
  if (pe1 >= 32) {
    c->P.nplan = nplan;
    c->P.plan_pe = pe1;
    c->P.lds_bytes = b1;
  }
  if (size_t(l.bytes) > limit)
    return fail(c, OCG_ECAP,
                "chain workgroup needs " + std::to_string(l.bytes) + " B of LDS (> " + std::to_string(limit) +
                    "): configuration exceeds the single-workgroup engine (see DESIGN.md §Scope)");
  c->P.fplan = nullptr;
  c->P.fast_off = 0;
  c->P.oplan = nullptr;
  c->P.ovl_bytes = 0;
  c->P.ovl_dh_bytes = 0;
  const char* nf = std::getenv("OCG_NO_FAST");
  if (nf && nf[0] && nf[0] != '0') {
    c->fast_why = "OCG_NO_FAST";
    return 0;
  }
  ocg_host::FastPlanBuild fb = ocg_host::build_fast_plan(c->P, c->md);
  if (!fb.why_not.empty()) {
    c->fast_why = fb.why_not;
    return 0;
  }
  const int off = (l.bytes + 255) & ~255;
  const int fbytes = ocg_host::fast_lds_bytes(fb.plan, c->P);
  if (size_t(off + fbytes) > limit) {
    c->fast_why = "LDS";
    return 0;
  }
  HIPCHK(c, hipMalloc(&c->d_fplan, sizeof(int) * fb.plan.size()));
  HIPCHK(c, hipMemcpyAsync(c->d_fplan, fb.plan.data(), sizeof(int) * fb.plan.size(), hipMemcpyHostToDevice,
                           c->stream));
  HIPCHK(c, hipStreamSynchronize(c->stream));
  c->P.fplan = c->d_fplan;
  c->P.fast_off = off;
  c->P.nplan = 0;
  c->P.plan_pe = 0;
  c->P.lds_bytes = off + fbytes;
  c->plan_pe2 = 0;
  c->lds2 = 0;
#ifndef OCG_PROFILE
  {
    const char* no = std::getenv("OCG_NO_FAST_OVL");
    const std::vector<int> ov = ocg_host::build_overlap_plan(c->P, c->md);
    const int ob = ov.empty() ? 0 : ocg_host::overlap_lds_bytes(ov, c->P);
    const int obd = ov.empty() ? 0 : ocg_host::overlap_lds_bytes(ov, c->P, true);
    if (!ov.empty() && ob <= off && obd <= 65536 && !(no && no[0] && no[0] != '0')) {
      HIPCHK(c, hipMalloc(&c->d_oplan, sizeof(int) * ov.size()));
      HIPCHK(c, hipMemcpyAsync(c->d_oplan, ov.data(), sizeof(int) * ov.size(), hipMemcpyHostToDevice, c->stream));
      HIPCHK(c, hipStreamSynchronize(c->stream));
      c->P.oplan = c->d_oplan;
      c->P.ovl_bytes = ob;
      c->P.ovl_dh_bytes = obd;
      if (std::getenv("OCG_FAST_DUMP"))
        std::fprintf(stderr, "[fast ovl] np %d nblk %d ints %d bytes %d\n", ov[ocg::fastp::kOvNp],
                     ov[ocg::fastp::kOvNblk], ov[ocg::fastp::kOvNint], ob);
    }
  }
#endif
#ifdef OCG_PROFILE
  c->lds_alias = 0;
#else
  c->lds_alias = std::max(l.bytes, fbytes);
  if (const char* e = std::getenv("OCG_FAST_ALIAS"))
    if (e[0] == '0') c->lds_alias = 0;
#endif
  return 0;
}


static bool make_stream(ocg_ctx* c) {
  if (hipStreamCreateWithFlags(&c->stream, hipStreamNonBlocking) != hipSuccess ||
      hipEventCreate(&c->ev0) != hipSuccess || hipEventCreate(&c->ev1) != hipSuccess ||
      hipEventCreate(&c->evh[0]) != hipSuccess || hipEventCreate(&c->evh[1]) != hipSuccess ||
      hipEventCreate(&c->evh[2]) != hipSuccess || hipEventCreate(&c->evh[3]) != hipSuccess) {
    c->err = "stream/event creation failed";
    return false;
  }
  return true;
}

static void note_u(ocg_ctx* c, const double* u, int N, int which) {
  if (which & 1) c->u_psi.assign(u, u + N);
  if (which & 2) c->u_xi.assign(u, u + N);
}
static bool same_u(const std::vector<double>& a, const double* u, int N) {
  return a.size() == size_t(N) && std::memcmp(a.data(), u, sizeof(double) * N) == 0;
}

static int hb(ocg_ctx* c, int rc) {
  if (rc) c->err = hbm_last_error(c->hbm);
  return rc;
}
extern "C" {

const char* ocg_last_error(const ocg_ctx* ctx) { return ctx ? ctx->err.c_str() : g_create_error.c_str(); }

size_t ocg_mps_nelem(int L, int p, int Q, const int* dims) {
  size_t s = 0;
  int Q1 = Q + 1;
  for (int k = 1; k <= L; ++k)
    for (int q = 0; q < Q1; ++q)
      for (int n = 0; n < p && q + n <= Q; ++n) s += size_t(dims[(k - 1) * Q1 + q]) * dims[k * Q1 + q + n];
  return s;
}

int ocg_device_count(int* n) {
  if (!n) return OCG_EINVAL;
  *n = 0;
  hipError_t e = hipGetDeviceCount(n);
  if (e != hipSuccess || *n <= 0) {
    g_create_error = std::string("no HIP device available: ") + hipGetErrorString(e);
    *n = 0;
    return OCG_EHIP;
  }
  return OCG_OK;
}

static int create_hbm(ocg_ctx* c, int L, int p, int npart, double tstep, double cutoff, int maxm) {
  std::vector<int> md, mdz;
  ocg_host::rank_bounds(L, p, npart, md, mdz);
  OcgParams G{};
  G.p = p;
  G.dt = tstep;
  std::vector<double> gf, gb;
  ocg_host::gate_tables(G, c->J, gf, gb);
  std::string err;
  const int rc = hbm_create(c->device, L, p, npart, c->J, tstep, cutoff, maxm, md, mdz, gf, gb, G.glo, G.gsz,
                            G.goff, G.gtotal, ocg_host::gate_order(L), &c->hbm, err);
  if (rc) return fail(c, rc, "HBM engine: " + err);
  c->P.L = L; c->P.p = p; c->P.Q = npart; c->P.Q1 = npart + 1; c->P.nsq = (L + 1) * (npart + 1);
  c->P.dt = tstep; c->P.cutoff = cutoff; c->P.maxm = maxm > 0 ? maxm : 5000;
  return 0;
}

int ocg_create_ex(int device, int L, int p, int npart, double J, double tstep, double cutoff, int maxm, int engine,
                  ocg_ctx** out) {
  if (!out) { g_create_error = "out is NULL"; return OCG_EINVAL; }
  *out = nullptr;
  if (engine < 0 || engine > 2) { g_create_error = "engine must be 0 (auto), 1 (LDS) or 2 (HBM)"; return OCG_EINVAL; }
  auto* c = new ocg_ctx;
  c->device = device;
  c->J = J;
  auto bail = [&](int code) {
    g_create_error = c->err;
    ocg_destroy(c);
    return code;
  };
  const bool lds_fits = L <= OCG_MAXL && npart + 1 <= OCG_MAXQ1;
  if (L < 2 || L > 63 || p < 2 || p > OCG_MAXP || npart < 0 || npart + 1 > 1024 || npart > L * (p - 1) ||
      !(tstep == tstep) || !(cutoff >= 0) || (engine == 1 && !lds_fits)) {
    int rc = build_params(c, L, p, npart, tstep, cutoff, maxm);
    if (!rc) { c->err = "bad argument"; rc = OCG_EINVAL; }
    return bail(rc);
  }
  int ndev = 0;
  hipError_t e = hipGetDeviceCount(&ndev);
  if (e != hipSuccess || ndev <= 0) {
    c->err = std::string("no HIP device available: ") + hipGetErrorString(e);
    return bail(OCG_EHIP);
  }
  if (device < 0 || device >= ndev) { c->err = "device index out of range"; return bail(OCG_EINVAL); }
  if (hipSetDevice(device) != hipSuccess) { c->err = "hipSetDevice failed"; return bail(OCG_EHIP); }
  if (!make_stream(c)) return bail(OCG_EHIP);
  int rc = 0;
  if (engine != 2 && lds_fits) {
    rc = build_params(c, L, p, npart, tstep, cutoff, maxm);
    if (!rc) rc = upload_gates(c);
    if (!rc) rc = finish_params(c);
    if (rc == OCG_ECAP && engine == 0) {
      const std::string why = c->err;
      ocg_ctx* h = new ocg_ctx;
      h->device = device;
      h->J = J;
      if (!make_stream(h)) {
        ocg_destroy(h);
        return bail(OCG_EHIP);
      }
      std::swap(c, h);
      ocg_destroy(h);
      if ((rc = create_hbm(c, L, p, npart, tstep, cutoff, maxm))) return bail(rc);
    } else if (rc) {
      return bail(rc);
    }
  } else if ((rc = create_hbm(c, L, p, npart, tstep, cutoff, maxm))) {
    return bail(rc);
  }
  if (c->hbm) {
// ... 203 lines not shown
                     size_t* out_nelem, int* steps_done) {
  if (!c || !dims || !data || !out_dims || !out_data || ntau < 0 || (ntau > 0 && !taus) || block < 1 ||
      max_steps < 0)
    return c ? fail(c, OCG_EINVAL, "bad argument") : OCG_EINVAL;
  for (int s = 0; s < ntau; ++s)
    if (!(taus[s] > 0)) return fail(c, OCG_EINVAL, "tau must be > 0");
  HIPCHK(c, hipSetDevice(c->device));
  const double dt0 = c->P.dt;
  if (c->hbm) {
    OcgParams G{};
    G.p = c->P.p;
    G.imag = 1;
    std::vector<std::vector<double>> gf(ntau), gb(ntau);
    for (int s = 0; s < ntau; ++s) {
      G.dt = taus[s];
      ocg_host::gate_tables(G, c->J, gf[s], gb[s]);
    }
    G.dt = dt0;
    G.imag = 0;
    std::vector<double> gf0, gb0;
    ocg_host::gate_tables(G, c->J, gf0, gb0);
    return hb(c, hbm_ground_state(c->hbm, dims, data, U, ntau, taus, gf, gb, G.glo, G.gsz, G.goff, G.gtotal, dt0,
                                  gf0, gb0, block, tol, max_steps, out_dims, out_data, out_cap, out_nelem, steps_done));
  }
  const OcgParams& P = c->P;
  const int a = c->slot_tmp(0), b = c->slot_tmp(1);
  if (int rc = upload_mps(c, a, dims, data)) return rc;
  const std::vector<double> u(size_t(block) + 1, U);
  int done = 0, rc = 0;
  for (int s = 0; s < ntau && !rc; ++s) {
    c->P.dt = taus[s];
    c->P.imag = 1;
    if ((rc = upload_gates(c))) break;
    for (int d = 0; d < max_steps; d += block) {
      hipError_t e = hipMemcpyAsync(SLOT_D(c->pool, P, b), SLOT_D(c->pool, P, a), sizeof(int) * P.nsq,
                                    hipMemcpyDeviceToDevice, c->stream);
      if (e == hipSuccess)
        e = hipMemcpyAsync(SLOT_X(c->pool, P, b), SLOT_X(c->pool, P, a), sizeof(zc) * P.cap, hipMemcpyDeviceToDevice,
                           c->stream);
      if (e != hipSuccess) {
        rc = fail(c, OCG_EHIP, std::string("slot copy: ") + hipGetErrorString(e));
        break;
      }
      if ((rc = launch_steps(c, a, u.data(), block, 1))) break;
      done += block;
      std::vector<zc> ov;
      if ((rc = launch_overlaps(c, {b}, {a}, 0, ov))) break;
      if (1.0 - std::hypot(ov[0].x, ov[0].y) < tol) break;
    }
  }
  c->P.dt = dt0;
  c->P.imag = 0;
  const int rc2 = upload_gates(c);
  if (steps_done) *steps_done = done;
  if (rc || rc2) return rc ? rc : rc2;
  return download_mps(c, a, out_dims, out_data, out_cap, out_nelem);
}

int ocg_step_batch(ocg_ctx* c, int n, const int* dims, const double* const* data, const double* u_from,
                   const double* u_to, int forward, int* out_dims, double* const* out_data, const size_t* out_cap,
                   size_t* out_nelem) {
  if (!c || n < 0 || (n > 0 && (!dims || !data || !u_from || !u_to || !out_dims || !out_data || !out_cap)))
    return c ? fail(c, OCG_EINVAL, "null argument") : OCG_EINVAL;
  if (n == 0) return 0;
  if (c->hbm) {
    std::vector<double> uu(2 * size_t(n));
    std::vector<int> fw(n, forward);
    for (int i = 0; i < n; ++i) { uu[2 * i] = u_from[i]; uu[2 * i + 1] = u_to[i]; }
    return hb(c, hbm_steps(c->hbm, n, dims, data, uu.data(), 2, 1, fw.data(), out_dims, out_data, out_cap, out_nelem));
  }
  HIPCHK(c, hipSetDevice(c->device));
  const OcgParams& P = c->P;
  const int base = 6 + 4 * c->N;
  if (int rc = ensure_slots(c, base + n)) return rc;
  std::vector<int> slots(n);
  std::vector<double> uu(2 * size_t(n));
  for (int i = 0; i < n; ++i) {
    slots[i] = base + i;
    if (int rc = upload_mps(c, slots[i], dims + size_t(i) * P.nsq, data[i])) return rc;
    uu[2 * i] = u_from[i];
    uu[2 * i + 1] = u_to[i];
  }
  if (int rc = ensure_buf(c, c->d_u, c->u_cap, 2 * n)) return rc;
  if (int rc = ensure_buf(c, c->d_idx, c->idx_cap, n)) return rc;
  HIPCHK(c, hipMemcpyAsync(c->d_u, uu.data(), sizeof(double) * 2 * n, hipMemcpyHostToDevice, c->stream));
  HIPCHK(c, hipMemcpyAsync(c->d_idx, slots.data(), sizeof(int) * n, hipMemcpyHostToDevice, c->stream));
  if (int rc = begin_kernel(c)) return rc;
  const OcgParams Pa = c->Pa();
  hipLaunchKernelGGL(k_steps, dim3(n), dim3(NT), Pa.lds_bytes, c->stream, Pa, c->d_gf, c->d_gb, c->d_md, c->pool,
                     c->d_idx, n, c->d_u, 2, 1, forward, c->d_stats + 4 * 3);
  if (int rc = end_kernel(c, 4)) return rc;
  for (int i = 0; i < n; ++i)
    if (int rc = download_mps(c, slots[i], out_dims + size_t(i) * P.nsq, out_data[i], out_cap[i],
                              out_nelem ? out_nelem + i : nullptr))
      return rc;
  return 0;
}

static void ovl_pairs(ocg_ctx* c, const int* xs, const int* ys, int n, int with_dH, zc* out) {
  if (n <= 0) return;
  if (c->P.oplan) {
    hipLaunchKernelGGL(k_overlaps_pad, dim3(unsigned(n)), dim3(64), c->P.ovl_dh_bytes, c->stream, c->P, c->pool, xs,
                       ys, n, with_dH, out, c->d_stats + 1 * 3);
    return;
  }
  const OcgParams Po = c->Po();
  hipLaunchKernelGGL(k_overlaps, dim3(unsigned(n)), dim3(NT), Po.lds_bytes, c->stream, Po, c->d_gf, c->d_gb, c->d_md,
                     c->pool, xs, ys, n, with_dH, out, c->d_stats + 1 * 3);
}

static int launch_overlaps(ocg_ctx* c, const std::vector<int>& xs, const std::vector<int>& ys, int with_dH,
                           std::vector<zc>& out) {
  const OcgParams& P = c->P;
  int n = int(xs.size());
  if (n == 0) return 0;
  if (int rc = ensure_buf(c, c->d_idx, c->idx_cap, 2 * n)) return rc;
  if (int rc = ensure_buf(c, c->d_c, c->c_cap, n)) return rc;
  std::vector<int> idx(xs);
  idx.insert(idx.end(), ys.begin(), ys.end());
  HIPCHK(c, hipMemcpyAsync(c->d_idx, idx.data(), sizeof(int) * 2 * n, hipMemcpyHostToDevice, c->stream));
  if (int rc = begin_kernel(c)) return rc;
  ovl_pairs(c, c->d_idx, c->d_idx + n, n, with_dH, c->d_c);
  if (int rc = end_kernel(c, 1)) return rc;
  out.resize(n);
  HIPCHK(c, hipMemcpyAsync(out.data(), c->d_c, sizeof(zc) * n, hipMemcpyDeviceToHost, c->stream));
  HIPCHK(c, hipStreamSynchronize(c->stream));
  return 0;
}

int ocg_overlap(ocg_ctx* c, const int* dims_x, const double* x, const int* dims_y, const double* y, int with_dH,
                double* out) {
  if (!c || !dims_x || !x || !dims_y || !y || !out) return c ? fail(c, OCG_EINVAL, "null argument") : OCG_EINVAL;
  if (c->hbm) return hb(c, hbm_overlap(c->hbm, dims_x, x, dims_y, y, with_dH, out));
  HIPCHK(c, hipSetDevice(c->device));
  if (int rc = upload_mps(c, c->slot_tmp(0), dims_x, x)) return rc;
  if (int rc = upload_mps(c, c->slot_tmp(1), dims_y, y)) return rc;
  std::vector<zc> r;
  if (int rc = launch_overlaps(c, {c->slot_tmp(0)}, {c->slot_tmp(1)}, with_dH, r)) return rc;
  out[0] = r[0].x;
  out[1] = r[0].y;
  return 0;
}

static int launch_apply_dH(ocg_ctx* c, const std::vector<int>& in, const std::vector<int>& outs, double* norms) {
  const OcgParams& P = c->P;
  int n = int(in.size());
  if (int rc = ensure_buf(c, c->d_idx, c->idx_cap, 2 * n)) return rc;
  if (norms)
    if (int rc = ensure_buf(c, c->d_norms, c->norms_cap, n)) return rc;
  std::vector<int> idx(in);
  idx.insert(idx.end(), outs.begin(), outs.end());
  HIPCHK(c, hipMemcpyAsync(c->d_idx, idx.data(), sizeof(int) * 2 * n, hipMemcpyHostToDevice, c->stream));
  if (int rc = begin_kernel(c)) return rc;
  const OcgParams Pn = c->Pn();
  hipLaunchKernelGGL(k_apply_dH, dim3(n), dim3(NT), Pn.lds_bytes, c->stream, Pn, c->d_gf, c->d_gb, c->d_md, c->pool,
                     c->d_idx, c->d_idx + n, n, norms ? c->d_norms : nullptr, c->d_stats + 2 * 3);
  if (int rc = end_kernel(c, 2)) return rc;
  if (norms) {
    HIPCHK(c, hipMemcpyAsync(norms, c->d_norms, sizeof(double) * n, hipMemcpyDeviceToHost, c->stream));
    HIPCHK(c, hipStreamSynchronize(c->stream));
  }
  return 0;
}

int ocg_apply_dH(ocg_ctx* c, const int* dims, const double* data, int* out_dims, double* out_data, size_t out_cap,
                 size_t* out_nelem, double* norm) {
  if (!c || !dims || !data) return c ? fail(c, OCG_EINVAL, "null argument") : OCG_EINVAL;
  if (c->hbm) return hb(c, hbm_apply_dH(c->hbm, dims, data, out_dims, out_data, out_cap, out_nelem, norm));
  HIPCHK(c, hipSetDevice(c->device));
  if (int rc = upload_mps(c, c->slot_tmp(0), dims, data)) return rc;
  double nrm = 0;
  if (int rc = launch_apply_dH(c, {c->slot_tmp(0)}, {c->slot_tmp(1)}, &nrm)) return rc;
  if (norm) *norm = nrm;
  return download_mps(c, c->slot_tmp(1), out_dims, out_data, out_cap, out_nelem);
}

int ocg_set_states(ocg_ctx* c, const int* dims_target, const double* target, const int* dims_init,
                   const double* init) {
  if (!c || !dims_target || !target || !dims_init || !init) return c ? fail(c, OCG_EINVAL, "null argument") : OCG_EINVAL;
  c->u_psi.clear();
  c->u_xi.clear();
  if (c->hbm) return hb(c, hbm_set_states(c->hbm, dims_target, target, dims_init, init));
  HIPCHK(c, hipSetDevice(c->device));
  if (int rc = upload_mps(c, c->slot_target(), dims_target, target)) return rc;
  if (int rc = upload_mps(c, c->slot_init(), dims_init, init)) return rc;
  c->have_states = true;
  c->have_psi = c->have_xi = c->have_xih = false;
  return 0;
}

int ocg_propagate(ocg_ctx* c, const double* u, int N, int which) {
  if (!c || !u || N < 2 || which < 1 || which > 3) return c ? fail(c, OCG_EINVAL, "bad argument") : OCG_EINVAL;
  if (which & 1) c->u_psi.clear();
  if (which & 2) c->u_xi.clear();
  if (c->hbm) {
    const int rc = hb(c, hbm_propagate(c->hbm, u, N, which));
    if (!rc) note_u(c, u, N, which);
    return rc;
  }
  if (!c->have_states) return fail(c, OCG_ESTATE, "ocg_set_states first");
  HIPCHK(c, hipSetDevice(c->device));
  const OcgParams& P = c->P;
  if (N != c->N) {
    c->N = N;
    c->have_psi = c->have_xi = c->have_xih = false;
  }
  if (int rc = ensure_slots(c, 6 + 4 * N)) return rc;
  if (int rc = ensure_buf(c, c->d_u, c->u_cap, N)) return rc;
  HIPCHK(c, hipMemcpyAsync(c->d_u, u, sizeof(double) * N, hipMemcpyHostToDevice, c->stream));
  int grid = (which == 3) ? 2 : 1;
  if (int rc = begin_kernel(c)) return rc;
  const OcgParams Pa = c->Pa();
  hipLaunchKernelGGL(k_trajectory, dim3(grid), dim3(NT), Pa.lds_bytes, c->stream, Pa, c->d_gf, c->d_gb, c->d_md,
                     c->pool, c->slot_init(), c->slot_target(), c->psi_base(), c->xi_base(), c->d_u, N, which,
                     c->d_stats + 0 * 3, 0);
  if (int rc = end_kernel(c, 0)) return rc;
  if (which & 1) { c->have_psi = true; c->have_xih = c->have_xih && (which & 2); }
  if (which & 2) { c->have_xi = true; c->have_xih = false; }
  note_u(c, u, N, which);
  return 0;
}

int ocg_gradient(ocg_ctx* c, const double* u, int N, double* divT, double* F) {
  if (!c || !u || !divT || !F || N < 2) return c ? fail(c, OCG_EINVAL, "bad argument") : OCG_EINVAL;
  if (c->hbm) {
    const char* e = std::getenv("OCG_HBM_MID");
    int mid = e ? std::atoi(e) : -1;
    if (mid < 0) {
      size_t fr = 0, tot = 0;
      HIPCHK(c, hipSetDevice(c->device));
      HIPCHK(c, hipMemGetInfo(&fr, &tot));
      mid = hbm_traj_bytes(c->hbm, N) > 0.5 * double(fr) ? 1 : 0;
    }
    if (mid == 1) {
      c->u_psi.clear();
      c->u_xi.clear();
      return hb(c, hbm_gradient_mid(c->hbm, u, N, divT, F));
    }
  }
  if (int rc = ocg_propagate(c, u, N, 3)) return rc;
  if (int rc = ocg_div_t(c, divT)) return rc;
  return ocg_overlap_factor(c, F);
}

int ocg_gradient_multi(ocg_ctx* c, int K, const double* u, int N, double* divT, double* F) {
  if (!c || !u || !divT || !F || N < 2 || K < 1) return c ? fail(c, OCG_EINVAL, "bad argument") : OCG_EINVAL;
  if (size_t(K) * 4 * size_t(N) + 6 > size_t(INT32_MAX)) return fail(c, OCG_EINVAL, "K * N too large");
  if (c->hbm && K > 1) {
    size_t fr = 0, tot = 0;
    HIPCHK(c, hipSetDevice(c->device));
    HIPCHK(c, hipMemGetInfo(&fr, &tot));
    if (hbm_gradient_multi_bytes(c->hbm, K, N) <= 0.5 * double(fr)) {
      c->u_psi.clear();
      c->u_xi.clear();
      if (hb(c, hbm_gradient_multi(c->hbm, K, u, N, divT, F)) == 0) {
        note_u(c, u, N, 3);
        return 0;
      }
    }
  }
  bool lds_batch = !c->hbm && K > 1;
  if (lds_batch) {
    size_t fr = 0, tot = 0;
    HIPCHK(c, hipSetDevice(c->device));
    HIPCHK(c, hipMemGetInfo(&fr, &tot));
    const double need = (6.0 + 2.0 * N * K) * (sizeof(zc) * double(c->P.cap) + sizeof(int) * double(c->P.nsq));
    lds_batch = 6 + 2 * N * K <= c->nslots || need <= 0.5 * double(fr);
  }
  if (!lds_batch) {
    for (int k = K - 1; k >= 0; --k) {
      if (int rc = ocg_propagate(c, u + size_t(k) * N, N, 3)) return rc;
      if (int rc = ocg_div_t(c, divT + size_t(k) * 2 * N)) return rc;
      if (int rc = ocg_overlap_factor(c, F + 2 * k)) return rc;
    }
    return 0;
  }
  if (!c->have_states) return fail(c, OCG_ESTATE, "ocg_set_states first");
  HIPCHK(c, hipSetDevice(c->device));
  const OcgParams& P = c->P;
  if (N != c->N) {
    c->N = N;
    c->have_psi = c->have_xi = c->have_xih = false;
  }
  c->u_psi.clear();
  c->u_xi.clear();
  const int cs = 2 * N;
  if (int rc = ensure_slots(c, 6 + cs * K)) return rc;
  if (int rc = ensure_buf(c, c->d_u, c->u_cap, K * N)) return rc;
  HIPCHK(c, hipMemcpyAsync(c->d_u, u, sizeof(double) * K * N, hipMemcpyHostToDevice, c->stream));
  if (int rc = begin_kernel(c)) return rc;
  const OcgParams Pa = c->Pa();
  hipLaunchKernelGGL(k_trajectory, dim3(2 * K), dim3(NT), Pa.lds_bytes, c->stream, Pa, c->d_gf, c->d_gb, c->d_md,
                     c->pool, c->slot_init(), c->slot_target(), c->psi_base(), c->xi_base(), c->d_u, N, 3,
                     c->d_stats + 0 * 3, cs);
  if (int rc = end_kernel(c, 0)) return rc;
  c->have_psi = c->have_xi = true;
  c->have_xih = false;
  note_u(c, u, N, 3);
  std::vector<int> xs(size_t(K) * N), ys(size_t(K) * N);
  for (int k = 0; k < K; ++k)
    for (int i = 0; i < N; ++i) {
      xs[size_t(k) * N + i] = c->xi_base() + k * cs + i;
      ys[size_t(k) * N + i] = c->psi_base() + k * cs + i;
    }
  std::vector<zc> r;
  if (int rc = launch_overlaps(c, xs, ys, 1, r)) return rc;
  for (size_t e = 0; e < size_t(K) * N; ++e) { divT[2 * e] = r[e].x; divT[2 * e + 1] = r[e].y; }
  std::vector<int> fx(K), fy(K, c->slot_target());
  for (int k = 0; k < K; ++k) fx[k] = c->psi_base() + k * cs + N - 1;
  if (int rc = launch_overlaps(c, fx, fy, 0, r)) return rc;
  for (int k = 0; k < K; ++k) { F[2 * k] = r[k].x; F[2 * k + 1] = r[k].y; }
  return 0;
}

int ocg_overlap_factor(ocg_ctx* c, double* F) {
  if (!c || !F) return OCG_EINVAL;
  if (c->hbm) return hb(c, hbm_overlap_factor(c->hbm, F));
  if (!c->have_psi) return fail(c, OCG_ESTATE, "psi_t not propagated");
  HIPCHK(c, hipSetDevice(c->device));
  std::vector<zc> r;
  if (int rc = launch_overlaps(c, {c->psi_base() + c->N - 1}, {c->slot_target()}, 0, r)) return rc;
  F[0] = r[0].x;
  F[1] = r[0].y;
  return 0;
}

int ocg_fidelities(ocg_ctx* c, double* fid) {
  if (!c || !fid) return OCG_EINVAL;
  if (c->hbm) return hb(c, hbm_fidelities(c->hbm, fid));
  if (!c->have_psi) return fail(c, OCG_ESTATE, "psi_t not propagated");
  HIPCHK(c, hipSetDevice(c->device));
  std::vector<int> xs(c->N, c->slot_target()), ys(c->N);
  for (int i = 0; i < c->N; ++i) ys[i] = c->psi_base() + i;
  std::vector<zc> r;
  if (int rc = launch_overlaps(c, xs, ys, 0, r)) return rc;
  for (int i = 0; i < c->N; ++i) fid[i] = r[i].x * r[i].x + r[i].y * r[i].y;
  return 0;
}

int ocg_div_t(ocg_ctx* c, double* divT) {
  if (!c || !divT) return OCG_EINVAL;
  if (c->hbm) return hb(c, hbm_div_t(c->hbm, divT));
  if (!c->have_psi || !c->have_xi) return fail(c, OCG_ESTATE, "psi_t and xi_t must be propagated");
  HIPCHK(c, hipSetDevice(c->device));
  std::vector<int> xs(c->N), ys(c->N);
  for (int i = 0; i < c->N; ++i) { xs[i] = c->xi_base() + i; ys[i] = c->psi_base() + i; }
  std::vector<zc> r;
  if (int rc = launch_overlaps(c, xs, ys, 1, r)) return rc;
  for (int i = 0; i < c->N; ++i) { divT[2 * i] = r[i].x; divT[2 * i + 1] = r[i].y; }
  return 0;
}

int ocg_xi_dH(ocg_ctx* c) {
  if (!c) return OCG_EINVAL;
  if (c->hbm) return hb(c, hbm_xi_dH(c->hbm));
  if (!c->have_xi) return fail(c, OCG_ESTATE, "xi_t not propagated");
  HIPCHK(c, hipSetDevice(c->device));
  std::vector<int> in(c->N), outs(c->N);
  for (int i = 0; i < c->N; ++i) { in[i] = c->xi_base() + i; outs[i] = c->xih_base() + i; }
  if (int rc = launch_apply_dH(c, in, outs, nullptr)) return rc;
  c->have_xih = true;
  return 0;
}

int ocg_hessian_rows(ocg_ctx* c, const double* u, int N, const int* rows, int nrows, const double* F,
                     const double* divT, double* H) {
  if (!c || !u || !rows || !F || !divT || !H || nrows < 0) return c ? fail(c, OCG_EINVAL, "null argument") : OCG_EINVAL;
  if (c->hbm) {
    for (int r = 0; r < nrows; ++r)
      if (rows[r] < 1 || rows[r] > N - 2) return fail(c, OCG_EINVAL, "row index out of [1, N-2]");
    return hb(c, hbm_hessian_rows(c->hbm, u, N, rows, nrows, F, divT, H));
  }
  if (N != c->N || !c->have_psi || !c->have_xih) return fail(c, OCG_ESTATE, "propagate(3) + xi_dH first");
  for (int r = 0; r < nrows; ++r)
    if (rows[r] < 1 || rows[r] > N - 2) return fail(c, OCG_EINVAL, "row index out of [1, N-2]");
  if (nrows == 0) return 0;
  HIPCHK(c, hipSetDevice(c->device));
  const OcgParams& P = c->P;
  if (int rc = ensure_buf(c, c->d_idx, c->idx_cap, nrows)) return rc;
  if (int rc = ensure_buf(c, c->d_u, c->u_cap, N)) return rc;
  if (int rc = ensure_buf(c, c->d_c, c->c_cap, N)) return rc;
  size_t hn = size_t(N) * N;
  if (hn > c->H_cap) {
    if (c->d_H) (void)hipFree(c->d_H);
    HIPCHK(c, hipMalloc(&c->d_H, sizeof(double) * hn));
    c->H_cap = hn;
  }
  HIPCHK(c, hipMemcpyAsync(c->d_idx, rows, sizeof(int) * nrows, hipMemcpyHostToDevice, c->stream));
  HIPCHK(c, hipMemcpyAsync(c->d_u, u, sizeof(double) * N, hipMemcpyHostToDevice, c->stream));
  HIPCHK(c, hipMemcpyAsync(c->d_c, divT, sizeof(zc) * N, hipMemcpyHostToDevice, c->stream));
  HIPCHK(c, hipMemsetAsync(c->d_H, 0, sizeof(double) * hn, c->stream));
  {
    std::vector<int> in(nrows), outs(nrows);
    for (int r = 0; r < nrows; ++r) { in[r] = c->psi_base() + rows[r]; outs[r] = c->psih_base() + rows[r]; }
    if (int rc = ensure_buf(c, c->d_rnorm, c->rnorm_cap, N)) return rc;
    if (int rc = ensure_buf(c, c->d_idx2, c->idx2_cap, 2 * nrows)) return rc;
    in.insert(in.end(), outs.begin(), outs.end());
    HIPCHK(c, hipMemcpyAsync(c->d_idx2, in.data(), sizeof(int) * 2 * nrows, hipMemcpyHostToDevice, c->stream));
    if (int rc = begin_kernel(c)) return rc;
    const OcgParams Pn = c->Pn();
    hipLaunchKernelGGL(k_apply_dH, dim3(nrows), dim3(NT), Pn.lds_bytes, c->stream, Pn, c->d_gf, c->d_gb, c->d_md,
                       c->pool, c->d_idx2, c->d_idx2 + nrows, nrows, c->d_rnorm, c->d_stats + 2 * 3);
    if (int rc = end_kernel(c, 2)) return rc;
    std::vector<double> nr(nrows), ni(N, 0.0);
    HIPCHK(c, hipMemcpyAsync(nr.data(), c->d_rnorm, sizeof(double) * nrows, hipMemcpyDeviceToHost, c->stream));
    HIPCHK(c, hipStreamSynchronize(c->stream));
    for (int r = 0; r < nrows; ++r) ni[rows[r]] = nr[r];
    HIPCHK(c, hipMemcpyAsync(c->d_rnorm, ni.data(), sizeof(double) * N, hipMemcpyHostToDevice, c->stream));
    HIPCHK(c, hipStreamSynchronize(c->stream));
  }
  zc f2 = mkz(F[0], F[1]);
  if (int rc = begin_kernel(c)) return rc;
  hipLaunchKernelGGL(k_hessian_rows, dim3(nrows), dim3(NT), P.lds_bytes, c->stream, P, c->d_gf, c->d_gb, c->d_md,
                     c->pool, c->psih_base(), c->xih_base(), c->d_idx, nrows, c->d_rnorm, c->d_u, N, c->d_c, f2,
                     c->d_H, c->d_stats + 3 * 3);
  if (int rc = end_kernel(c, 3)) return rc;
  std::vector<double> h(hn);
  HIPCHK(c, hipMemcpyAsync(h.data(), c->d_H, sizeof(double) * hn, hipMemcpyDeviceToHost, c->stream));
  HIPCHK(c, hipStreamSynchronize(c->stream));
  for (int r = 0; r < nrows; ++r) {
    int i = rows[r];
    for (int j = i; j + 1 < N; ++j) {
      H[size_t(i) * N + j] = h[size_t(i) * N + j];
      H[size_t(j) * N + i] = h[size_t(j) * N + i];
    }
  }
  return 0;
}

static int hessian_unfused(ocg_ctx* c, const double* u, int N, const int* rows, int nrows, double* H, double* divT,
                           double* F) {
  const bool have_psi = c->hbm ? hbm_have(c->hbm, 1) : c->have_psi;
  const bool have_xi = c->hbm ? hbm_have(c->hbm, 2) : c->have_xi;
  const bool reuse = have_psi && have_xi && same_u(c->u_psi, u, N) && same_u(c->u_xi, u, N);
  if (!reuse)
    if (int rc = ocg_propagate(c, u, N, 3)) return rc;
  if (int rc = ocg_div_t(c, divT)) return rc;
  if (int rc = ocg_overlap_factor(c, F)) return rc;
  const bool have_xih = c->hbm ? hbm_have(c->hbm, 3) : c->have_xih;
  if (!(reuse && have_xih))
    if (int rc = ocg_xi_dH(c)) return rc;
  return ocg_hessian_rows(c, u, N, rows, nrows, F, divT, H);
}

static int hessian_fused(ocg_ctx* c, int K, const double* u, int N, const int* rows, int nrows, double* H,
                         double* divT, double* F);

int ocg_hessian(ocg_ctx* c, const double* u, int N, const int* rows, int nrows, double* H, double* divT,
                double* F) {
  if (!c || !u || !H || !divT || !F || (nrows > 0 && !rows) || nrows < 0 || N < 4)
    return c ? fail(c, OCG_EINVAL, "bad argument") : OCG_EINVAL;
  if (c->hbm) {
    for (int r = 0; r < nrows; ++r)
      if (rows[r] < 1 || rows[r] > N - 2) return fail(c, OCG_EINVAL, "row index out of [1, N-2]");
    int K = 0;
    if (const char* e = std::getenv("OCG_HBM_CKPT")) K = std::atoi(e);
    if (K <= 0) {
      size_t fr = 0, tot = 0;
      HIPCHK(c, hipSetDevice(c->device));
      HIPCHK(c, hipMemGetInfo(&fr, &tot));
      if (hbm_traj_bytes(c->hbm, N) > 0.5 * double(fr)) K = std::max(1, int(std::ceil(std::sqrt(double(N)))));
    }
    if (K > 0) {
      c->u_psi.clear();
      c->u_xi.clear();
      const int rc = hb(c, hbm_hessian_ckpt(c->hbm, u, N, rows, nrows, H, divT, F, K));
      if (rc == 0) {
        ++c->ckpt_runs;
        c->ckpt_k = K;
      }
      return rc;
    }
    const char* pe = std::getenv("OCG_HBM_PIPE");
    const int pipe_env = pe ? std::atoi(pe) : -1;
    const bool reuse = hbm_have(c->hbm, 1) && hbm_have(c->hbm, 2) && same_u(c->u_psi, u, N) && same_u(c->u_xi, u, N);
    if (pipe_env != 0 && !reuse && nrows > 0) {
      size_t fr = 0, tot = 0;
      HIPCHK(c, hipMemGetInfo(&fr, &tot));
      if (pipe_env == 1 || hbm_pipe_bytes(c->hbm, N, rows, nrows) <= 0.5 * double(fr)) {
        c->u_psi.clear();
        c->u_xi.clear();
        const int rc = hb(c, hbm_hessian_pipe(c->hbm, u, N, rows, nrows, H, divT, F));
        if (rc == 0) {
          ++c->pipe_runs;
          note_u(c, u, N, 3);
          return 0;
        }
        if (rc != OCG_ENOMEM || pipe_env == 1) return rc;
        ++c->pipe_fallbacks;
        const int rc2 = hessian_unfused(c, u, N, rows, nrows, H, divT, F);
        if (rc2 == 0) c->err.clear();
        return rc2;
      }
    }
    return hessian_unfused(c, u, N, rows, nrows, H, divT, F);
  }
  return hessian_fused(c, 1, u, N, rows, nrows, H, divT, F);
}

static int hessian_fused(ocg_ctx* c, int K, const double* u, int N, const int* rows, int nrows, double* H,
                         double* divT, double* F) {
  if (!c->have_states) return fail(c, OCG_ESTATE, "ocg_set_states first");
  for (int r = 0; r < nrows; ++r)
    if (rows[r] < 1 || rows[r] > N - 2) return fail(c, OCG_EINVAL, "row index out of [1, N-2]");
  HIPCHK(c, hipSetDevice(c->device));
  const OcgParams& P = c->P;
  if (N != c->N) {
    c->N = N;
    c->have_psi = c->have_xi = c->have_xih = false;
  }
  const int cs = 4 * N;
  if (int rc = ensure_slots(c, 6 + cs * K)) return rc;
  if (int rc = ensure_buf(c, c->d_u, c->u_cap, K * N)) return rc;
  if (int rc = ensure_buf(c, c->d_pc, c->pc_cap, K * (N + 1))) return rc;
  if (int rc = ensure_buf(c, c->d_rows, c->rows_cap, 2 * nrows + 2)) return rc;
  if (int rc = ensure_buf(c, c->d_prn, c->prn_cap, K * nrows + 1)) return rc;
  const int nflags = K * (2 * N + 2) + 1;
  if (nflags > c->flags_cap) {
    if (c->d_flags) (void)hipFree(c->d_flags);
    c->d_flags = nullptr;
    c->flags_cap = 0;
    if (int rc = ensure_buf(c, c->d_flags, c->flags_cap, nflags)) return rc;
    c->flags_N = -1;
  }
  if (c->flags_N != N || c->flags_K != K) {
    HIPCHK(c, hipMemsetAsync(c->d_flags, 0, sizeof(int) * c->flags_cap, c->stream));
    c->epoch = 0;
    c->flags_N = N;
    c->flags_K = K;
  }
  size_t total = 0;
  for (int r = 0; r < nrows; ++r) total += size_t(N - 1 - rows[r]);
  {
    static const double budget_mb = [] {
      const char* e = std::getenv("OCG_RS_BUDGET_MB");
      return e ? std::atof(e) : 16384.0;
    }();
    const double need = double(K) * double(total) * (sizeof(zc) * double(P.cap) + sizeof(int) * double(P.nsq));
    if (size_t(K) * total > size_t(INT32_MAX / 2) || need > budget_mb * 1048576.0) {
      for (int k = 0; k < K; ++k) {
        const int kk = K - 1 - k;
        if (int rc = hessian_unfused(c, u + size_t(kk) * N, N, rows, nrows, H + size_t(kk) * N * N,
                                     divT + size_t(kk) * 2 * N, F + 2 * kk))
          return rc;
      }
      return 0;
    }
  }
  std::vector<int> rb(2 * nrows + 1);
  total = 0;
  for (int r = 0; r < nrows; ++r) rb[r] = rows[r];
  for (int r = 0; r < nrows; ++r) {
    rb[nrows + r] = int(total);
    total += size_t(N - 1 - rows[r]);
  }
  rb[2 * nrows] = int(total);
  if (size_t(K) * total > c->rs_cap) {
    if (c->rs.dims) (void)hipFree(c->rs.dims);
    if (c->rs.data) (void)hipFree(c->rs.data);
    c->rs = Pool{nullptr, nullptr};
    c->rs_cap = 0;
    HIPCHK(c, hipMalloc(&c->rs.dims, sizeof(int) * K * total * P.nsq));
    HIPCHK(c, hipMalloc(&c->rs.data, sizeof(zc) * K * total * P.cap));
    c->rs_cap = size_t(K) * total;
  }
  size_t hn = size_t(K) * N * N;
  if (hn > c->H_cap) {
    if (c->d_H) (void)hipFree(c->d_H);
    HIPCHK(c, hipMalloc(&c->d_H, sizeof(double) * hn));
    c->H_cap = hn;
  }
  const int epoch = ++c->epoch;
  auto al = [](size_t b) { return (b + 255) & ~size_t(255); };
  const size_t nidx = 2 * size_t(K) * N + 2 * K;
  const size_t o_rb = al(sizeof(double) * K * N), o_idx = o_rb + al(sizeof(int) * rb.size());
  const size_t o_err = o_idx + al(sizeof(int) * nidx), o_pc = o_err + 256;
  const size_t o_h = o_pc + al(sizeof(zc) * K * (N + 1)), pin_bytes = o_h + sizeof(double) * hn;
  if (int rc = ensure_pin(c, pin_bytes)) return rc;
  HIPCHK(c, hipStreamSynchronize(c->stream));
  std::memcpy(c->h_pin, u, sizeof(double) * K * N);
  std::memcpy(c->h_pin + o_rb, rb.data(), sizeof(int) * rb.size());
  HIPCHK(c, hipMemcpyAsync(c->d_u, c->h_pin, sizeof(double) * K * N, hipMemcpyHostToDevice, c->stream));
  HIPCHK(c, hipMemcpyAsync(c->d_rows, c->h_pin + o_rb, sizeof(int) * rb.size(), hipMemcpyHostToDevice, c->stream));
  HIPCHK(c, hipMemsetAsync(c->d_err, 0, sizeof(int), c->stream));
  HIPCHK(c, hipMemsetAsync(c->d_H, 0, sizeof(double) * hn, c->stream));
  HIPCHK(c, hipMemsetAsync(c->d_flags + K * (2 * N + 2), 0, sizeof(int), c->stream));
  const int* d_rows = c->d_rows;
  const int* d_rbase = c->d_rows + nrows;
  int* idx = (int*)(c->h_pin + o_idx);
  for (int k = 0; k < K; ++k) {
    for (int i = 0; i < N; ++i) {
      idx[k * N + i] = c->xi_base() + k * cs + i;
      idx[K * N + k * N + i] = c->psi_base() + k * cs + i;
    }
    idx[2 * K * N + k] = c->psi_base() + k * cs + N - 1;
    idx[2 * K * N + K + k] = c->slot_target();
  }
  if (int rc = ensure_buf(c, c->d_idx, c->idx_cap, int(nidx))) return rc;
  HIPCHK(c, hipMemcpyAsync(c->d_idx, idx, sizeof(int) * nidx, hipMemcpyHostToDevice, c->stream));
  HIPCHK(c, hipEventRecord(c->evh[0], c->stream));
  static const int xiw = [] {
    const char* e = std::getenv("OCG_XIH_WORKERS");
    const int v = e ? std::atoi(e) : kXiHWorkers;
    return v > 0 ? v : kXiHWorkers;
  }();
  const int nxw = std::min(N, xiw);
  static const int share_k = [] {
    const char* e = std::getenv("OCG_MULTI_SHARE_K");
    return e ? std::atoi(e) : 8;
  }();
  const OcgParams Pl = (share_k > 0 && K >= share_k) ? c->P2() : c->Pa();
  hipLaunchKernelGGL(k_pipeline, dim3(K * (2 + nxw + nrows)), dim3(NT), Pl.lds_bytes, c->stream, Pl, c->d_gf,
                     c->d_gb, c->d_md, c->pool, c->slot_init(), c->slot_target(), c->psi_base(), c->xi_base(),
                     c->xih_base(), c->d_u, N, d_rows, nrows, d_rbase, c->rs, c->d_prn, c->d_flags, epoch, c->d_err,
                     nxw, c->d_stats + 5 * 3, K, cs);
  HIPCHK(c, hipGetLastError());
  HIPCHK(c, hipEventRecord(c->evh[1], c->stream));
  const OcgParams Po = c->Po();
  ovl_pairs(c, c->d_idx, c->d_idx + K * N, K * N, 1, c->d_pc);
  ovl_pairs(c, c->d_idx + 2 * K * N, c->d_idx + 2 * K * N + K, K, 0, c->d_pc + K * N);
  HIPCHK(c, hipGetLastError());
  HIPCHK(c, hipEventRecord(c->evh[2], c->stream));
  static const int rov_w = [] {
    const char* e = std::getenv("OCG_ROWOV_WAVE");
    return (e && e[0] == '0') ? 0 : 1;
  }();
  static const int rov_env = [] {
    const char* e = std::getenv("OCG_ROWOV_GRID");
    return e ? std::atoi(e) : -1;
  }();
  int rov_grid = rov_env;
  if (rov_grid < 0) {
    int ncu = 0, lds_cu = 0;
    (void)hipDeviceGetAttribute(&ncu, hipDeviceAttributeMultiprocessorCount, c->device);
    (void)hipDeviceGetAttribute(&lds_cu, hipDeviceAttributeMaxSharedMemoryPerMultiprocessor, c->device);
    const int per = (Po.lds_bytes > 0 && lds_cu > 0) ? std::max(1, lds_cu / Po.lds_bytes) : 6;
    rov_grid = std::max(1, ncu) * std::min(per, 16);
  }
  const size_t ktotal = size_t(K) * total;
  const int rgrid = (rov_grid > 0 && size_t(rov_grid) < ktotal) ? rov_grid : int(ktotal);
  if (total > 0 && c->P.oplan) {
    int ncu = 0, lds_cu = 0;
    (void)hipDeviceGetAttribute(&ncu, hipDeviceAttributeMultiprocessorCount, c->device);
    (void)hipDeviceGetAttribute(&lds_cu, hipDeviceAttributeMaxSharedMemoryPerMultiprocessor, c->device);
    const int pb = c->P.ovl_bytes + 4 * (2 * nrows + 1);
    const int per = lds_cu > 0 ? std::max(1, lds_cu / pb) : 8;
    const size_t pg = rov_env > 0 ? size_t(rov_env) : size_t(std::max(1, ncu)) * std::min(per, 16);
    const int pgrid = int(std::min(pg, ktotal));
    if (pb > 65536) HIPCHK(c, hipFuncSetAttribute((const void*)k_row_overlaps_pad,
                                                   hipFuncAttributeMaxDynamicSharedMemorySize, pb));
    hipLaunchKernelGGL(k_row_overlaps_pad, dim3(unsigned(pgrid)), dim3(64), pb, c->stream, c->P,
                       c->pool, c->xih_base(), d_rows, nrows, d_rbase, c->rs, c->d_prn, c->d_pc, c->d_pc + K * N, N,
                       c->d_H, c->d_stats + 6 * 3, K, cs);
  } else if (total > 0 && rov_w)
    hipLaunchKernelGGL(k_row_overlaps_w, dim3(unsigned(rgrid)), dim3(64), Po.lds_bytes, c->stream, Po, c->d_gf,
                       c->d_gb, c->d_md, c->pool, c->xih_base(), d_rows, nrows, d_rbase, c->rs, c->d_prn, c->d_pc,
                       c->d_pc + K * N, N, c->d_H, c->d_stats + 6 * 3, K, cs);
  else if (total > 0)
    hipLaunchKernelGGL(k_row_overlaps, dim3(unsigned(rgrid)), dim3(NT), Po.lds_bytes, c->stream, Po, c->d_gf,
                       c->d_gb, c->d_md, c->pool, c->xih_base(), d_rows, nrows, d_rbase, c->rs, c->d_prn, c->d_pc,
                       c->d_pc + K * N, N, c->d_H, c->d_stats + 6 * 3, K, cs);
  HIPCHK(c, hipGetLastError());
  HIPCHK(c, hipEventRecord(c->evh[3], c->stream));
  const zc* pc = (const zc*)(c->h_pin + o_pc);
  const double* h = (const double*)(c->h_pin + o_h);
  HIPCHK(c, hipMemcpyAsync(c->h_pin + o_err, c->d_err, sizeof(int), hipMemcpyDeviceToHost, c->stream));
  HIPCHK(c, hipMemcpyAsync(c->h_pin + o_pc, c->d_pc, sizeof(zc) * K * (N + 1), hipMemcpyDeviceToHost, c->stream));
  HIPCHK(c, hipMemcpyAsync(c->h_pin + o_h, c->d_H, sizeof(double) * hn, hipMemcpyDeviceToHost, c->stream));
  HIPCHK(c, hipStreamSynchronize(c->stream));
  const int err = *(const int*)(c->h_pin + o_err);
  const int kinds[3] = {5, 1, 6};
  for (int k = 0; k < 3; ++k) {
    if (k == 2 && total == 0) break;
    float ms = 0;
    HIPCHK(c, hipEventElapsedTime(&ms, c->evh[k], c->evh[k + 1]));
    c->kst[kinds[k]].ms += ms;
    c->kst[kinds[k]].launches += 1;
  }
  if (err) {
    c->have_psi = c->have_xi = c->have_xih = false;
    HIPCHK(c, hipMemsetAsync(c->d_err, 0, sizeof(int), c->stream));
    HIPCHK(c, hipStreamSynchronize(c->stream));
    return fail(c, OCG_ENUM, std::string((err & OCG_ERR_WATCHDOG) ? "pipeline watchdog: a consumer saw no producer "
                                                                    "progress for ~15 s; " : "") +
                                 ((err & OCG_ERR_JACOBI) ? "eigensolver did not converge within its sweep cap" : ""));
  }
  c->have_psi = c->have_xi = c->have_xih = true;
  note_u(c, u, N, 3);
  for (int k = 0; k < K; ++k) {
    double* Hk = H + size_t(k) * N * N;
    const double* hk = h + size_t(k) * N * N;
    for (int i = 0; i < N; ++i) {
      divT[2 * (size_t(k) * N + i)] = pc[size_t(k) * N + i].x;
      divT[2 * (size_t(k) * N + i) + 1] = pc[size_t(k) * N + i].y;
    }
    F[2 * k] = pc[size_t(K) * N + k].x;
    F[2 * k + 1] = pc[size_t(K) * N + k].y;
    for (int r = 0; r < nrows; ++r) {
      const int i = rows[r];
      for (int j = i; j + 1 < N; ++j) {
        Hk[size_t(i) * N + j] = hk[size_t(i) * N + j];
        Hk[size_t(j) * N + i] = hk[size_t(j) * N + i];
      }
    }
  }
  return 0;
}

int ocg_hessian_multi(ocg_ctx* c, int K, const double* u, int N, const int* rows, int nrows, double* H,
                      double* divT, double* F) {
  if (!c || !u || !H || !divT || !F || (nrows > 0 && !rows) || nrows < 0 || N < 4 || K < 1)
    return c ? fail(c, OCG_EINVAL, "bad argument") : OCG_EINVAL;
  if (size_t(K) * 4 * size_t(N) + 6 > size_t(INT32_MAX) || size_t(K) * N * N > (size_t(1) << 40))
    return fail(c, OCG_EINVAL, "K * N too large");
  if (c->hbm || K == 1) {
    for (int k = K - 1; k >= 0; --k)
      if (int rc = ocg_hessian(c, u + size_t(k) * N, N, rows, nrows, H + size_t(k) * N * N, divT + size_t(k) * 2 * N,
                               F + 2 * k))
        return rc;
    return 0;
  }
  for (int r = 0; r < nrows; ++r)
    if (rows[r] < 1 || rows[r] > N - 2) return fail(c, OCG_EINVAL, "row index out of [1, N-2]");
  return hessian_fused(c, K, u, N, rows, nrows, H, divT, F);
}

int ocg_convert_hessian(ocg_ctx* c, const double* Hu, int N, const double* V, int M, double* Hc) {
  if (!c || !Hu || !V || !Hc || N < 1 || M < 1) return c ? fail(c, OCG_EINVAL, "bad argument") : OCG_EINVAL;
  HIPCHK(c, hipSetDevice(c->device));
  const size_t nn = size_t(N) * N, mn = size_t(M) * N, need = nn + 3 * mn + size_t(M) * M;
  if (need > c->proj_cap) {
    HIPCHK(c, hipStreamSynchronize(c->stream));
    if (c->d_proj) (void)hipFree(c->d_proj);
    c->d_proj = nullptr;
    c->proj_cap = 0;
    HIPCHK(c, hipMalloc(&c->d_proj, sizeof(double) * need));
    c->proj_cap = need;
  }
  double *dH = c->d_proj, *dV = dH + nn, *dVt = dV + mn, *dHV = dVt + mn, *dHc = dHV + mn;
  std::vector<double> vt(mn);
  for (int j = 0; j < M; ++j)
    for (int l = 0; l < N; ++l) vt[size_t(l) * M + j] = V[size_t(j) * N + l];
  HIPCHK(c, hipMemcpyAsync(dH, Hu, sizeof(double) * nn, hipMemcpyHostToDevice, c->stream));
  HIPCHK(c, hipMemcpyAsync(dV, V, sizeof(double) * mn, hipMemcpyHostToDevice, c->stream));
  HIPCHK(c, hipMemcpyAsync(dVt, vt.data(), sizeof(double) * mn, hipMemcpyHostToDevice, c->stream));
  const int bt = std::min(256, ((M + 63) / 64) * 64);
  hipLaunchKernelGGL(k_project_hv, dim3(N), dim3(bt), sizeof(double) * N, c->stream, dH, dVt, N, M, dHV);
  hipLaunchKernelGGL(k_project_c, dim3((M * M + 255) / 256), dim3(256), 0, c->stream, dV, dHV, N, M, dHc);
  HIPCHK(c, hipGetLastError());
  HIPCHK(c, hipMemcpyAsync(Hc, dHc, sizeof(double) * M * M, hipMemcpyDeviceToHost, c->stream));
  HIPCHK(c, hipStreamSynchronize(c->stream));
  return 0;
}

int ocg_denmat_decomp(ocg_ctx* c, int nm, const int* rows, const int* cols, const double* const* M, double cutoff,
                      int maxm, int* kept, double* const* w, double* const* A, double* const* B) {
  if (!c || nm < 0 || (nm > 0 && (!rows || !cols || !M || !kept)))
    return c ? fail(c, OCG_EINVAL, "bad argument") : OCG_EINVAL;
  if (!c->hbm) return fail(c, OCG_EINVAL, "ocg_denmat_decomp: HBM engine contexts only (ocg_create_ex engine 2)");
  if (nm == 0) return 0;
  return hb(c, hbm_denmat_decomp(c->hbm, nm, rows, cols, M, cutoff, maxm, kept, w, A, B));
}

int ocg_get_state(ocg_ctx* c, int which, int t, int* dims, double* data, size_t cap, size_t* nelem) {
  if (!c || !dims || !data) return OCG_EINVAL;
// ... 519 lines not shown
```

Measured before the change: 25440.

## Add fast-plan dH application path with zip-up decomposition and wide Jacobi

Adds a single-wave fast-plan implementation of applying dH to an MPS. It uses zip-up matrix ops, an 8x8 wide Jacobi eigensolver for larger Gram blocks, and precomputed plan entries. A dedicated pipeline kernel runs the xiH and row dH work through this fast path instead of the general engine. The forward-step flag publish is also reordered so consumers can start earlier. This is meant to cut the general-engine overhead in the dH/xiH precompute, at the cost of more LDS plan space and new code paths that fall back when bounds are exceeded.

```diff
diff --git a/optimalcontrolmps_amd/csrc/fast.hpp b/optimalcontrolmps_amd/csrc/fast.hpp
--- a/optimalcontrolmps_amd/csrc/fast.hpp
+++ b/optimalcontrolmps_amd/csrc/fast.hpp
@@ -11,6 +11,11 @@
 constexpr int kItF = 4;
 constexpr int kItS = 4;
 constexpr int kItMps = 4;
+constexpr int kDhMaxGram = 8;
+constexpr int kDhMaxWide = 2;
+constexpr int kDhItTh = 4;
+constexpr int kDhMaxDot = 32;
+constexpr int kDhMaxF = 1024;
 
 enum {
   kHNp = 0,
@@ -32,10 +37,12 @@
   kHCentre,
   kHThZ,
   kHXsZ,
+  kHDhN,
+  kHDhOps,
   kHOps,
   kHdrInts = kHOps + kMaxOps
 };
-enum { kOpGate = 0, kOpGaugeR = 1, kOpGaugeL = 2 };
+enum { kOpGate = 0, kOpGaugeR = 1, kOpGaugeL = 2, kOpZip = 3, kOpZipLast = 4 };
 enum {
   kOhKind = 0, kOhK, kOhDir, kOhMode,
   kOhLonely, kOhClosing, kOhNth, kOhNewBond,
@@ -49,6 +56,7 @@
   kOhF, kOhNf,
   kOhS, kOhNs,
   kOhDot,
+  kOhWide,
   kOhGrp = 24,
   kOpHdr = kOhGrp + 32
 };
diff --git a/optimalcontrolmps_amd/csrc/fast_chain.hpp b/optimalcontrolmps_amd/csrc/fast_chain.hpp
--- a/optimalcontrolmps_amd/csrc/fast_chain.hpp
+++ b/optimalcontrolmps_amd/csrc/fast_chain.hpp
@@ -13,8 +13,9 @@
   lzp MP, TH, TG, WB, XS, GT, PH;
   LDS double *LAM, *SIG, *SIGI, *MCB, *MCF;
   LDS int* MCE;
-  LDS int *DIM, *BOF, *KQ, *WIDX, *PL;
+  LDS int *DIM, *BOF, *KQ, *WIDX, *FLG, *PL;
   int np, nblk, o_blk, o_ls, o_site, o_siten, nops, centre_open;
+  int ndh = 0, o_dh = 0;
   int thz, xsz;
   double ph_u = __builtin_nan("");
   int ph_dir = -1;
@@ -52,6 +53,7 @@
     np = gplan[kHNp]; nblk = gplan[kHNblk]; o_blk = gplan[kHBlk]; o_ls = gplan[kHLs]; o_site = gplan[kHSite];
     o_siten = gplan[kHSiteN]; nops = gplan[kHNops]; centre_open = gplan[kHCentre];
     thz = gplan[kHThZ]; xsz = gplan[kHXsZ];
+    ndh = gplan[kHDhN]; o_dh = gplan[kHDhOps];
     lzp cb{(LDS double*)base};
     MP = cb + gplan[kHZMps]; TH = cb + gplan[kHZTh]; TG = cb + gplan[kHZTg]; WB = cb + gplan[kHZW];
     XS = cb + gplan[kHZX]; GT = cb + gplan[kHZGt]; PH = cb + gplan[kHZPh];
@@ -65,7 +67,7 @@
     BOF = ib; ib += al(nblk);
     KQ = ib; ib += 64;
     WIDX = ib; ib += 64;
-    ib += 4;
+    FLG = ib; ib += 4;
     PL = ib;
   }
   __device__ __forceinline__ void wsync() const {
@@ -333,6 +335,7 @@
     }
   }
 
+  template <int NG = fastp::kMaxGram>
   __device__ OCG_INLINE void decompose(const LDS int* oh, lzp M, int dir, double cutoff, int maxm, bool normalize) {
     using namespace fastp;
     pf(2);
@@ -381,15 +384,38 @@
     if (used) WB[16 * g + 4 * i + j] = w;
     if (valid && i == j) LAM[eoff + i] = gv.x > 0 ? gv.x : 0.0;
     if (lane < no1) LAM[o1[3]] = lam1;
+    if constexpr (NG > kMaxGram) {
+      const LDS int* wt = PL + uni(oh[kOhWide]);
+      const int nw = uni(wt[0]);
+      for (int b = 0; b < nw; ++b) {
+        const i4 wa = ld4(wt + 4 + 8 * b), wc = ld4(wt + 8 + 8 * b);
+        const int wtho = uni(wa[0]), wR = uni(wa[1]), wC = uni(wa[2]), wside = uni(wa[3]), weoff = uni(wc[0]),
+                  wn = uni(wc[1]);
+        const int wi = lane >> 3, wj = lane & 7;
+        const bool wvalid = wi < wn && wj < wn;
+        const int len = wside == 0 ? wC : wR, st = wside == 0 ? 1 : wC;
+        const int bi = wtho + (wi < wn ? wi : 0) * (wside == 0 ? wC : 1);
+        const int bj = wtho + (wj < wn ? wj : 0) * (wside == 0 ? wC : 1);
+        zc gw = c2(0.0, 0.0);
+        double unused = 0.0;
+        for (int c0 = 0; c0 < len; c0 += 8) gram_dots<8>(M, len - c0, st, bi + c0 * st, bj + c0 * st, 0, 0, 0, gw, unused);
+        if (wside == 1) gw.y = -gw.y;
+        if (!wvalid) gw = c2(0.0, 0.0);
+        zc ww = c2(wi == wj ? 1.0 : 0.0, 0.0);
+        jacobi_wide(gw, ww, wvalid, wn);
+        WB[66 + 64 * b + lane] = ww;
+        if (wvalid && wi == wj) LAM[weoff + wi] = gw.x > 0 ? gw.x : 0.0;
+      }
+    }
     wsync();
     const double lam = ae ? LAM[lane] : 0.0;
     const int i_e = eq[1], eo_e = eq[2], n_e = eq[3] & 255, bound = unsigned(eq[3]) >> 8;
-    double lt[kMaxGram];
-#pragma unroll
-    for (int t = 0; t < kMaxGram; ++t) lt[t] = CH::bperm(lam, ((eo_e + t) & 63) << 2);
+    double lt[NG];
+#pragma unroll
+    for (int t = 0; t < NG; ++t) lt[t] = CH::bperm(lam, ((eo_e + t) & 63) << 2);
     int jb = 0;
 #pragma unroll
-    for (int t = 0; t < kMaxGram; ++t)
+    for (int t = 0; t < NG; ++t)
       jb += (ae & (t < n_e) & (t != i_e) & ((lt[t] > lam) | ((lt[t] == lam) & (t < i_e)))) ? 1 : 0;
     const double total = wsum(lam);
     const double cut = cutoff * total, floor_ = 1e-30 * total;
@@ -455,13 +481,17 @@
     wsync();
     pf(5);
     const double inv = (normalize && kw > 1e-32) ? 1.0 / sqrt(kw) : 1.0;
-    if (nf <= 64) factors<1>(o_f, nf, M, dir, inv);
-    else if (nf <= 128) factors<2>(o_f, nf, M, dir, inv);
-    else if (nf <= 192) factors<3>(o_f, nf, M, dir, inv);
-    else factors<kItF>(o_f, nf, M, dir, inv);
-  }
-
-  template <int IF>
+    if constexpr (NG > kMaxGram) {
+      for (int e0 = 0; e0 < nf; e0 += 128) factors<2, NG>(o_f + 4 * e0, nf - e0 < 128 ? nf - e0 : 128, M, dir, inv);
+    } else {
+      if (nf <= 64) factors<1>(o_f, nf, M, dir, inv);
+      else if (nf <= 128) factors<2>(o_f, nf, M, dir, inv);
+      else if (nf <= 192) factors<3>(o_f, nf, M, dir, inv);
+      else factors<kItF>(o_f, nf, M, dir, inv);
+    }
+  }
+
+  template <int IF, int NG = fastp::kMaxGram>
   __device__ OCG_INLINE void factors(int o_f, int nf, lzp M, int dir, double inv) {
     using namespace fastp;
     i4 fd[IF];
@@ -472,7 +502,7 @@
     }
     int kqs[IF], wvv[IF];
     double sg[IF], isg[IF];
-    zc mv[IF][kMaxGram];
+    zc mv[IF][NG];
 #pragma unroll
     for (int it = 0; it < IF; ++it) {
       const int w0 = fd[it][0], w1 = fd[it][1], w2 = fd[it][2];
@@ -484,7 +514,7 @@
       sg[it] = SIG[eo + jj];
       isg[it] = SIGI[eo + jj];
 #pragma unroll
-      for (int x = 0; x < kMaxGram; ++x) mv[it][x] = M[(exact || x >= terms) ? thz : mb + x * ms];
+      for (int x = 0; x < NG; ++x) mv[it][x] = M[(exact || x >= terms) ? thz : mb + x * ms];
     }
     zc out[IF];
     int dst[IF];
@@ -501,15 +531,16 @@
       const int wvc = live ? wvv[it] : 0;
       const int base = exact ? w1 : wbse;
       const double cs = isx ? 1.0 : -1.0;
-      zc wp[kMaxGram];
-#pragma unroll
-      for (int x = 0; x < kMaxGram; ++x) {
-        const zc t = WB[base + 4 * (x < tc ? x : tc) + wvc];
+      const int ws = (NG > kMaxGram && ((w2 >> 13) & 1)) ? 8 : 4;
+      zc wp[NG];
+#pragma unroll
+      for (int x = 0; x < NG; ++x) {
+        const zc t = WB[base + ws * (x < tc ? x : tc) + wvc];
         wp[x] = c2(t.x, cs * t.y);
       }
       zc acc = c2(0.0, 0.0);
 #pragma unroll
-      for (int x = 0; x < kMaxGram; ++x) cacc(acc, mv[it][x], wp[x]);
+      for (int x = 0; x < NG; ++x) cacc(acc, mv[it][x], wp[x]);
       const double sig = sg[it];
       const zc we = wp[0];
       const bool scl = isx ? dir == kFromright : dir == kFromleft;
@@ -641,6 +672,163 @@
 #endif
   }
 
+  __device__ OCG_INLINE void jacobi_wide(zc& g, zc& w, bool valid, int n) {
+    const int i = lane >> 3, j = lane & 7;
+    auto at = [&](int r, int c) { return (r * 8 + c) << 2; };
+    double di = CH::bperm(g.x, at(i, i)), dj = CH::bperm(g.x, at(j, j));
+    const bool up = i < j, dg = i == j;
+    int sweep = 0, nr = 0;
+    bool done = false;
+    for (; sweep < 40; ++sweep) {
+      bool flag = false;
+      for (int rnd = 0; rnd < 7; ++rnd) {
+        if (__ballot(valid && up && CH::jneed(cabs2(g), di, dj)) == 0) {
+          done = true;
+          break;
+        }
+        ++nr;
+        const int k = rnd + 1;
+        int pi = i, pj = j;
+        if (valid) {
+          if ((i ^ k) < n) pi = i ^ k;
+          if ((j ^ k) < n) pj = j ^ k;
+        }
+        const int arow = at(i, pi), acol = at(j, pj);
+        const bool zp = pi == j && i != j;
+        const zc g01 = CH::bpermz(g, at(i, j ^ k)), g10 = CH::bpermz(g, at(i ^ k, j));
+        const zc g11 = CH::bpermz(g, at(i ^ k, j ^ k)), w1 = CH::bpermz(w, at(i, j ^ k));
+        const zc bv = up ? g : g11;
+        const double app = up ? di : dj, aqq = up ? dj : di;
+        const bool need = CH::jneed(cabs2(bv), app, aqq);
+        zc jd, jo;
+        double ds;
+        jrot_role(bv, app, aqq, need && !dg, up, jd, jo, ds);
+        const zc jdc = CH::bpermz(jd, acol), joc = CH::bpermz(jo, acol);
+        const zc jdr = CH::bpermz(jd, arow), jor = CH::bpermz(jo, arow);
+        const double dsc = CH::bperm(ds, acol), dsr = CH::bperm(ds, arow);
+        zc wn = cmul(w, jdc);
+        cacc(wn, w1, joc);
+        zc r0 = cmul(g, jdc);
+        cacc(r0, g01, joc);
+        zc r1 = cmul(g10, jdc);
+        cacc(r1, g11, joc);
+        zc out = cjmul(jdr, r0);
+        cjacc(out, jor, r1);
+        const double dj2 = dj + dsc, di2 = di + dsr;
+        out = (zp && need) ? c2(0.0, 0.0) : out;
+        out = dg ? c2(dj2, 0.0) : out;
+        if (rnd == 6) flag = valid && up && CH::jneed(cabs2(out), di2, dj2);
+        g = out;
+        w = wn;
+        di = di2;
+        dj = dj2;
+      }
+      if (done || __ballot(flag) == 0) break;
+    }
+    if (sweep == 40 && lane == 0 && P.err) atomicOr(P.err, OCG_ERR_JACOBI);
+    cnt(21, 1.0);
+    cnt(20, double(sweep + 1));
+    cnt(30, double(nr));
+#ifdef OCG_FAST_TRACE
+    if (lane == 0) printf("[jacobi wide] op %d order %d sweeps %d rounds %d\n", trace_op, n, sweep + 1, nr);
+#endif
+  }
+
+  __device__ __forceinline__ bool has_dH() const { return ndh > 0; }
+  template <bool LAST>
+  __device__ OCG_INLINE void zipmat(const LDS int* oh) {
+    using namespace fastp;
+    pf(11);
+    const int nth = uni(oh[kOhNth]);
+    const LDS int* md = PL + uni(oh[kOhMat]);
+    if (nth > 0) {
+      int d0[kDhItTh], d1[kDhItTh], dd[kDhItTh];
+#pragma unroll
+      for (int it = 0; it < kDhItTh; ++it) {
+        const int e = lane + 64 * it, ee = e < nth ? e : nth - 1;
+        if constexpr (LAST) {
+          const i4 v = ld4(md + 4 * ee);
+          d0[it] = v[0]; d1[it] = v[1]; dd[it] = v[2];
+        } else {
+          d0[it] = md[2 * ee]; d1[it] = md[2 * ee + 1]; dd[it] = e;
+        }
+      }
+#pragma unroll
+      for (int it = 0; it < kDhItTh; ++it) {
+        const int e = lane + 64 * it;
+        const int x1 = d0[it] & 0xffff, x2 = unsigned(d0[it]) >> 16, dl = d1[it] & 0xff, dc = (d1[it] >> 8) & 0xff,
+                  t = (d1[it] >> 16) & 1, n = (d1[it] >> 20) & 15;
+        const int dlc = dl > 0 ? dl - 1 : 0;
+        zc v0 = c2(0.0, 0.0), v1 = c2(0.0, 0.0);
+#pragma unroll
+        for (int a = 0; a < kMaxDm; ++a) {
+          const bool in = a < dl;
+          const zc c0 = XS[in ? x1 + a : xsz], c1 = XS[in ? x1 + dl + a : xsz];
+          const zc av = MP[x2 + (a < dlc ? a : dlc) * dc];
+          cacc(v0, c0, av);
+          cacc(v1, c1, av);
+        }
+        double wn = 0.0;
+#pragma unroll
+        for (int m = 0; m < 6; ++m) wn = n == m ? P.dH[m] : wn;
+        const zc r = t == 0 ? v0 : c2(wn * v0.x + v1.x, wn * v0.y + v1.y);
+        if (e < nth) (LAST ? MP : TH)[dd[it]] = r;
+      }
+    }
+    wsync();
+  }
+  __device__ OCG_INLINE void apply_dH() {
+    using namespace fastp;
+    if (!act) return;
+    pf(11);
+    if (lane == 0) {
+      XS[0] = c2(1.0, 0.0);
+      XS[1] = c2(0.0, 0.0);
+    }
+    wsync();
+    for (int o = 0; o < ndh; ++o) {
+      const LDS int* oh = PL + PL[o_dh + o];
+      const int kind = uni(oh[kOhKind]);
+      const bool zip = kind != kOpGaugeL;
+      trace_op = 100 + o;
+      if (zip) {
+        if (kind == kOpZipLast) {
+          zipmat<true>(oh);
+          continue;
+        }
+        zipmat<false>(oh);
+      } else {
+        pf(7);
+        matcopy_it<kDhItTh>(oh, uni(oh[kOhNth]));
+        wsync();
+      }
+      decompose<kDhMaxGram>(oh, TH, zip ? kFromleft : kFromright, zip ? OCG_GAUGE_CUTOFF : P.cutoff,
+                            zip ? 1 << 30 : P.maxm, false);
+      if (!zip) {
+        pf(25);
+        const int ns = uni(oh[kOhNs]);
+        if (ns <= 128) neighbour_it<2, kDhMaxGram>(oh, ns, kOpGaugeL);
+        else neighbour_it<kItS, kDhMaxGram>(oh, ns, kOpGaugeL);
+      }
+    }
+    if (lane == 0) TG[thz] = c2(0.0, 0.0);
+    wsync();
+    pf(12);
+  }
+  __device__ OCG_INLINE double site_norm2(int k) const {
+    if (!act) return 0.0;
+    const int a = PL[o_site + k], b = PL[o_site + k + 1];
+    double acc = 0.0;
+    for (int x = a + lane; x < b; x += 64) acc += cabs2(zc(MP[x]));
+    return wsum(acc);
+  }
+  __device__ OCG_INLINE double compact_used() {
+    if (!act) return 0.0;
+    block_offsets();
+    const i4 t = ld4(PL + o_blk + 4 * (nblk - 1));
+    return double(BOF[nblk - 1] + DIM[t[1]] * DIM[t[2]]);
+  }
+
   __device__ OCG_INLINE void neighbour(const LDS int* oh) {
     using namespace fastp;
     pf(25);
@@ -649,7 +837,7 @@
     else if (ns <= 128) neighbour_it<2>(oh, ns, kind);
     else neighbour_it<kItS>(oh, ns, kind);
   }
-  template <int IT>
+  template <int IT, int NB = fastp::kMaxDm>
   __device__ OCG_INLINE void neighbour_it(const LDS int* oh, int ns, int kind) {
     using namespace fastp;
     const LDS int* sl = PL + uni(oh[kOhS]);
@@ -667,7 +855,7 @@
       const int lc = len > 0 ? len - 1 : 0;
       acc[it] = c2(0.0, 0.0);
 #pragma unroll
-      for (int b = 0; b < kMaxDm; ++b) {
+      for (int b = 0; b < NB; ++b) {
         const int bb = b < lc ? b : lc;
         const bool in = b < len;
         const zc a = (kind == kOpGaugeR) ? zc(XS[in ? x1 + b : xsz]) : zc(MP[in ? x1 + b : np]);
diff --git a/optimalcontrolmps_amd/csrc/fast_plan.hpp b/optimalcontrolmps_amd/csrc/fast_plan.hpp
--- a/optimalcontrolmps_amd/csrc/fast_plan.hpp
+++ b/optimalcontrolmps_amd/csrc/fast_plan.hpp
@@ -14,9 +14,10 @@
 struct FastPlanBuild {
   std::vector<int> plan;
   std::string why_not;
+  std::string dh_why_not;
 };
 
-inline FastPlanBuild build_fast_plan(const OcgParams& P, const std::vector<int>& md) {
+inline FastPlanBuild build_fast_plan(const OcgParams& P, const std::vector<int>& md, bool with_dh = true) {
   using namespace ocg::fastp;
   FastPlanBuild out;
   const int L = P.L, p = P.p, Q = P.Q, Q1 = P.Q1;
@@ -334,6 +335,289 @@
       setH(kOhNs, cnt);
     }
   }
+  int zip_tot = 0;
+  std::vector<int> dh_off;
+  {
+    const size_t keep = I.size();
+    const int thmax0 = thmax, xsmax0 = xsmax;
+    auto dh = [&]() -> std::string {
+      const char* no = std::getenv("OCG_NO_FAST_DH");
+      if (no && no[0] && no[0] != '0') return "OCG_NO_FAST_DH";
+      if (!with_dh) return "LDS";
+      std::vector<int> dz(size_t(L + 1) * Q1, 0);
+      auto Dz = [&](int b, int q) { return (b < 0 || b > L || q < 0 || q > Q) ? 0 : dz[size_t(b) * Q1 + q]; };
+      for (int q = 0; q <= Q; ++q) dz[q] = D(0, q);
+      for (int k = 1; k <= L; ++k)
+        for (int q = 0; q <= Q; ++q) {
+          int R = 0;
+          for (int n = 0; n < p; ++n) R += Dz(k - 1, q - n);
+          const int C = k < L ? 2 * D(k, q) : D(k, q);
+          dz[size_t(k) * Q1 + q] = (R == 0 || C == 0) ? 0 : (k < L ? std::min(R, C) : C);
+          if (Dz(k, q) > kDhMaxGram) return "dH: zip-up bond sector above the wide Jacobi's order";
+        }
+      auto lay = [&](int base, auto&& rd, auto&& cd, std::vector<int>& off) {
+        off.assign(size_t(Q1) * p, -1);
+        int t = base;
+        for (int q = 0; q <= Q; ++q)
+          for (int n = 0; n < p && q + n <= Q; ++n) {
+            const int dl = rd(q), dr = cd(q + n);
+            if (dl == 0 || dr == 0) continue;
+            off[size_t(q) * p + n] = t;
+            t += dl * dr;
+          }
+        return t;
+      };
+      std::vector<std::vector<int>> Z(L + 1), H(L + 1);
+      const int zb0 = (np + 2) & ~1;
+      int zb = zb0;
+      for (int k = 1; k <= L; ++k) {
+        const int e1 = lay(zb, [&](int q) { return Dz(k - 1, q); }, [&](int q) { return Dz(k, q); }, Z[k]);
+        const int e2 = lay(zb, [&](int q) { return Dz(k - 1, q); }, [&](int q) { return D(k, q); }, H[k]);
+        zb = std::max(e1, e2);
+      }
+      H[1].assign(size_t(Q1) * p, -1);
+      for (int q = 0; q <= Q; ++q)
+        for (int n = 0; n < p; ++n) H[1][size_t(q) * p + n] = PO(1, q, n);
+      zip_tot = zb - zb0;
+      if (zb > 65535) return "dH: zip layout offset above 16 bits";
+      auto emit_dec = [&](int hpos, const std::vector<int>& R, const std::vector<int>& C, const std::vector<int>& THO,
+                          int newb, auto&& bound, auto&& xdest, auto&& ydest) -> std::string {
+        auto setH = [&](int f, int v) { I[hpos + f] = v; };
+        std::vector<int> sq, secn(Q1, 0), seco(Q1, -1), secside(Q1, 0), secgrp(Q1, -1), secw(Q1, -1), seceoff(Q1, 0);
+        int ngrp = 0, nw = 0, T = 0, maxn = 0, maxdot = 1;
+        for (int q = 0; q <= Q; ++q) {
+          if (R[q] == 0) continue;
+          const int n = std::min(R[q], C[q]);
+          if (n > kDhMaxGram) return "dH: Gram block above the wide Jacobi's order";
+          if (std::max(R[q], C[q]) > kDhMaxDot) return "dH: Gram dot product above the bound";
+          if (n > kMaxGram || (n >= 2 && ngrp >= 4)) {
+            if (nw >= kDhMaxWide) return "dH: too many wide Gram blocks in one decomposition";
+            secw[q] = nw++;
+          } else if (n >= 2) {
+            secgrp[q] = ngrp++;
+            maxn = std::max(maxn, n);
+          }
+          seco[q] = int(sq.size());
+          secn[q] = n; secside[q] = R[q] <= C[q] ? 0 : 1; seceoff[q] = T;
+          sq.push_back(q);
+          T += n;
+          maxdot = std::max(maxdot, std::max(R[q], C[q]));
+        }
+        const int nsec = int(sq.size());
+        if (nsec > 15) return "dH: more than 15 sectors";
+        if (T > 64) return "dH: more than 64 eigenvalues per decomposition";
+        setH(kOhNewBond, newb); setH(kOhDot, maxdot);
+        setH(kOhNsec, nsec); setH(kOhT, T); setH(kOhNgrp, ngrp);
+        setH(kOhMaxr, maxn >= 3 ? 3 : (maxn == 2 ? 1 : 0));
+        for (int g = 0; g < 4; ++g) I[hpos + kOhGrp + 8 * g] = -1;
+        for (int s = 0; s < nsec; ++s) {
+          const int q = sq[s], g = secgrp[q];
+          if (g < 0) continue;
+          int* G = &I[hpos + kOhGrp + 8 * g];
+          G[0] = s; G[1] = secn[q]; G[2] = secside[q]; G[3] = THO[q]; G[4] = R[q]; G[5] = C[q]; G[6] = seceoff[q];
+        }
+        setH(kOhWide, pad());
+        push4(nw, 0, 0, 0);
+        for (int s = 0; s < nsec; ++s) {
+          const int q = sq[s];
+          if (secw[q] < 0) continue;
+          push4(THO[q], R[q], C[q], secside[q]);
+          push4(seceoff[q], secn[q], 0, 0);
+        }
+        setH(kOhO1, pad());
+        int no1 = 0;
+        for (int s = 0; s < nsec; ++s) {
+          const int q = sq[s];
+          if (secn[q] != 1) continue;
+          const bool rowv = secside[q] == 0;
+          push4(THO[q], rowv ? C[q] : R[q], rowv ? 1 : C[q], seceoff[q]);
+          ++no1;
+        }
+        setH(kOhNo1, no1);
+        setH(kOhEq, pad());
+        for (int s = 0; s < nsec; ++s) {
+          const int q = sq[s];
+          for (int i = 0; i < secn[q]; ++i) push4(s, i, seceoff[q], secn[q] | (bound(q) << 8));
+        }
+        setH(kOhSecQ, pad());
+        for (int s = 0; s < nsec; ++s) I.push_back(sq[s] | (seceoff[sq[s]] << 8) | (secn[sq[s]] << 16));
+        setH(kOhF, pad());
+        int nf = 0;
+        bool ok = true;
+        auto pushf = [&](int dest, int q, int j, bool isx, bool scratch, int idx) {
+          const int s = seco[q], n = secn[q], side = secside[q], g = secgrp[q], w = secw[q];
+          const bool exact = isx ? side == 0 : side == 1;
+          const int wb = w >= 0 ? 66 + 64 * w : (g >= 0 ? 16 * g : 64), ws = w >= 0 ? 8 : 4;
+          int w1;
+          if (exact) w1 = wb + (n >= 2 ? ws * idx : 0);
+          else if (isx) w1 = (THO[q] + idx * C[q]) | (n << 16) | (1 << 21);
+          else w1 = (THO[q] + idx) | (n << 16) | (C[q] << 21);
+          if (dest < 0 || dest > 65535 || j > 15 || C[q] > 255 || THO[q] + idx * C[q] > 65535) ok = false;
+          push4(dest | (s << 16) | (j << 20) | (isx ? 1 << 24 : 0) | (scratch ? 1 << 25 : 0), w1,
+                seceoff[q] | (n << 8) | (exact ? 1 << 12 : 0) | (w >= 0 ? 1 << 13 : 0), wb);
+          ++nf;
+        };
+        for (int q = 0; q <= Q; ++q) {
+          if (R[q] == 0) continue;
+          const int jb = bound(q);
+          for (int row = 0; row < R[q]; ++row)
+            for (int j = 0; j < jb; ++j) {
+              bool scr = false;
+              const int d = xdest(q, row, j, scr);
+              pushf(d, q, j, true, scr, row);
+            }
+          for (int j = 0; j < jb; ++j)
+            for (int col = 0; col < C[q]; ++col) {
+              bool scr = false;
+              const int d = ydest(q, j, col, scr);
+              pushf(d, q, j, false, scr, col);
+            }
+        }
+        if (!ok) return "dH: factor descriptor overflow";
+        if (nf > kDhMaxF) return "dH: factor list above the bound";
+        setH(kOhNf, nf);
+        return "";
+      };
+      std::vector<int> coff(Q1, 0);
+      for (int k = 1; k <= L; ++k) {
+        const bool last = k == L;
+        std::vector<int> R(Q1, 0), C(Q1, 0), THO(Q1 + 1, 0);
+        std::vector<std::vector<int>> RS(Q1, std::vector<int>(p, -1));
+        for (int q = 0; q <= Q; ++q) {
+          for (int n = 0; n < p; ++n)
+            if (Dz(k - 1, q - n) > 0) { RS[q][n] = R[q]; R[q] += Dz(k - 1, q - n); }
+          C[q] = last ? D(k, q) : 2 * D(k, q);
+          if (R[q] == 0 || C[q] == 0) { R[q] = 0; C[q] = 0; }
+          THO[q + 1] = THO[q] + R[q] * C[q];
+        }
+        const int nth = THO[Q1];
+        if (nth > 64 * kDhItTh) return "dH: zip-up matricisation above the unrolled maximum";
+        if (!last) thmax = std::max(thmax, nth);
+        const int hpos = pad();
+        dh_off.push_back(hpos);
+        I.resize(I.size() + kOpHdr, 0);
+        I[hpos + kOhKind] = last ? kOpZipLast : kOpZip;
+        I[hpos + kOhK] = k; I[hpos + kOhDir] = 0; I[hpos + kOhNth] = nth;
+        I[hpos + kOhMat] = pad();
+        for (int q = 0; q <= Q; ++q) {
+          if (R[q] == 0) continue;
+          const int dc = D(k, q);
+          for (int n = 0; n < p; ++n) {
+            if (RS[q][n] < 0) continue;
+            const int ql = q - n, dl = D(k - 1, ql);
+            for (int ap = 0; ap < Dz(k - 1, ql); ++ap)
+              for (int col = 0; col < C[q]; ++col) {
+                const int t = last ? 1 : (col >= dc ? 1 : 0), c = last ? col : col - t * dc;
+                const int x1 = coff[ql] + ap * 2 * dl, x2 = PO(k, ql, n) + c;
+                const int e = THO[q] + (RS[q][n] + ap) * C[q] + col;
+                const int dest = last ? H[k][size_t(ql) * p + n] + ap * dc + c : e;
+                if (PO(k, ql, n) < 0 || dl > kMaxDm || x1 > 65535 || dest < 0 || dest > 65535)
+                  return "dH: zip-up descriptor overflow";
+                if (last) {
+                  push4(x1 | (x2 << 16), dl | (dc << 8) | (t << 16) | (n << 20), dest, 0);
+                } else {
+                  I.push_back(x1 | (x2 << 16));
+                  I.push_back(dl | (dc << 8) | (t << 16) | (n << 20));
+                }
+              }
+          }
+        }
+        if (last) break;
+        std::vector<int> ys(Q1, 0);
+        int ys_tot = 0;
+        for (int q = 0; q <= Q; ++q) { ys[q] = ys_tot; ys_tot += Dz(k, q) * C[q]; }
+        const std::string w = emit_dec(
+            hpos, R, C, THO, k, [&](int q) { return Dz(k, q); },
+            [&](int q, int row, int j, bool& scr) {
+              int n = p - 1;
+              while (RS[q][n] < 0 || RS[q][n] > row) --n;
+              scr = false;
+              return Z[k][size_t(q - n) * p + n] + (row - RS[q][n]) * Dz(k, q) + j;
+            },
+            [&](int q, int j, int col, bool& scr) {
+              scr = true;
+              return ys[q] + j * C[q] + col;
+            });
+        if (!w.empty()) return w;
+        coff = ys;
+        xsmax = std::max(xsmax, std::max(ys_tot, 2));
+      }
+      for (int k = L; k >= 2; --k) {
+        std::vector<int> R(Q1, 0), C(Q1, 0), THO(Q1 + 1, 0);
+        std::vector<std::vector<int>> CS(Q1, std::vector<int>(p, -1));
+        for (int q = 0; q <= Q; ++q) {
+          R[q] = Dz(k - 1, q);
+          for (int n = 0; n < p; ++n)
+            if (D(k, q + n) > 0) { CS[q][n] = C[q]; C[q] += D(k, q + n); }
+          if (R[q] == 0 || C[q] == 0) { R[q] = 0; C[q] = 0; }
+          THO[q + 1] = THO[q] + R[q] * C[q];
+        }
+        const int nth = THO[Q1];
+        if (nth > 64 * kDhItTh) return "dH: sweep matricisation above the unrolled maximum";
+        thmax = std::max(thmax, nth);
+        const int hpos = pad();
+        dh_off.push_back(hpos);
+        I.resize(I.size() + kOpHdr, 0);
+        I[hpos + kOhKind] = kOpGaugeL;
+        I[hpos + kOhK] = k; I[hpos + kOhDir] = 1; I[hpos + kOhNth] = nth;
+        I[hpos + kOhMat] = pad();
+        for (int q = 0; q <= Q; ++q) {
+          if (R[q] == 0) continue;
+          for (int a = 0; a < R[q]; ++a)
+            for (int n = 0; n < p; ++n) {
+              if (CS[q][n] < 0) continue;
+              for (int c = 0; c < D(k, q + n); ++c) I.push_back(H[k][size_t(q) * p + n] + a * D(k, q + n) + c);
+            }
+        }
+        std::vector<int> xs(Q1, 0);
+        int xs_tot = 0;
+        for (int q = 0; q <= Q; ++q) { xs[q] = xs_tot; xs_tot += R[q] * D(k - 1, q); }
+        const std::string w = emit_dec(
+            hpos, R, C, THO, k - 1, [&](int q) { return D(k - 1, q); },
+            [&](int q, int row, int j, bool& scr) {
+              scr = true;
+              return xs[q] + row * D(k - 1, q) + j;
+            },
+            [&](int q, int j, int col, bool& scr) {
+              int n = p - 1;
+              while (CS[q][n] < 0 || CS[q][n] > col) --n;
+              scr = false;
+              return PO(k, q, n) + j * D(k, q + n) + (col - CS[q][n]);
+            });
+        if (!w.empty()) return w;
+        xsmax = std::max(xsmax, xs_tot);
+        I[hpos + kOhS] = pad();
+        int cnt = 0;
+        for (int ql = 0; ql <= Q; ++ql)
+          for (int n = 0; n < p && ql + n <= Q; ++n) {
+            const int qq = ql + n, ho = H[k - 1][size_t(ql) * p + n], zo = Z[k - 1][size_t(ql) * p + n];
+            const int dl = Dz(k - 2, ql), dr = D(k - 1, qq), dm = Dz(k - 1, qq);
+            if (dl == 0 || dr == 0) continue;
+            if (ho < 0 || zo < 0) return "dH: internal: sweep neighbour outside its layouts";
+            for (int a = 0; a < dl; ++a)
+              for (int j = 0; j < dr; ++j) {
+                const int x1 = zo + a * dm, x2 = xs[qq] + j, len = R[qq] == 0 ? 0 : dm;
+                if (x1 > 65535 || x2 > 65535 || len > kDhMaxGram) return "dH: product descriptor overflow";
+                push4(x1 | (x2 << 16), len | (dr << 16), ho + a * dr + j, 0);
+                ++cnt;
+              }
+          }
+        if (cnt > 64 * kItS) return "dH: gauge product above the unrolled maximum";
+        I[hpos + kOhNs] = cnt;
+      }
+      return "";
+    };
+    out.dh_why_not = L >= 2 ? dh() : "dH: fewer than two sites";
+    if (!out.dh_why_not.empty()) {
+      I.resize(keep);
+      thmax = thmax0;
+      xsmax = xsmax0;
+      zip_tot = 0;
+      dh_off.clear();
+    }
+  }
+  const int o_dh = pad();
+  for (int o : dh_off) I.push_back(o);
   int zc_off = 0;
   auto take = [&](int n) { const int o = zc_off; zc_off += (n + 1) & ~1; return o; };
   I[kHNp] = np;
@@ -344,10 +628,12 @@
   I[kHSiteN] = o_siten;
   I[kHNops] = int(ops.size());
   for (size_t i = 0; i < ops.size(); ++i) I[kHOps + int(i)] = op_off[i];
+  I[kHDhN] = int(dh_off.size());
+  I[kHDhOps] = o_dh;
   I[kHZMps] = take(np + 1);
+  I[kHZTg] = take(std::max(thmax + 1, zip_tot));
   I[kHZTh] = take(thmax + 1);
-  I[kHZTg] = take(thmax + 1);
-  I[kHZW] = take(65);
+  I[kHZW] = take(dh_off.empty() ? 65 : 66 + 64 * kDhMaxWide);
   I[kHZX] = take(xsmax + 1);
   I[kHThZ] = thmax;
   I[kHXsZ] = xsmax;
@@ -360,11 +646,16 @@
   if (I.size() > 65535) return fail("plan too large");
   if (std::getenv("OCG_FAST_DUMP")) {
     std::fprintf(stderr, "[fast plan] np %d nblk %d ints %zu zc %d\n", np, nblk, I.size(), zc_off);
-    for (size_t i = 0; i < ops.size(); ++i) {
-      const int* h = &I[op_off[i]];
+    std::fprintf(stderr, "[fast plan] dH ops %zu zip %d th %d xs %d %s\n", dh_off.size(), zip_tot, thmax, xsmax,
+                 out.dh_why_not.c_str());
+    std::vector<int> all(op_off);
+    all.insert(all.end(), dh_off.begin(), dh_off.end());
+    for (size_t i = 0; i < all.size(); ++i) {
+      const int* h = &I[all[i]];
       std::fprintf(stderr, "[fast plan] op %zu kind %d k %d nth %d nsec %d T %d ngrp %d maxr %d dot %d no1 %d nf %d ns %d\n",
                    i, h[kOhKind], h[kOhK], h[kOhNth], h[kOhNsec], h[kOhT], h[kOhNgrp], h[kOhMaxr], h[kOhDot],
                    h[kOhNo1], h[kOhNf], h[kOhNs]);
+      if (h[kOhWide]) std::fprintf(stderr, "[fast plan]   wide passes %d\n", I[h[kOhWide]]);
     }
   }
   out.plan = I;
diff --git a/optimalcontrolmps_amd/csrc/kernels.hpp b/optimalcontrolmps_amd/csrc/kernels.hpp
--- a/optimalcontrolmps_amd/csrc/kernels.hpp
+++ b/optimalcontrolmps_amd/csrc/kernels.hpp
@@ -9,6 +9,7 @@
 __device__ __forceinline__ int* flat(LDS int* p) { return (int*)p; }
 __device__ __forceinline__ zc* flat(lzp p) { return (zc*)(double*)p.p; }
 __device__ __forceinline__ bool fast_on(const OcgParams& P) { return P.fplan != nullptr && !P.imag; }
+__device__ __forceinline__ bool fast_dh_on(const OcgParams& P) { return fast_on(P) && P.fplan[fastp::kHDhN] > 0; }
 __device__ __forceinline__ void publish_flag_wt(int* flag, int epoch, int* progress) {
   if (threadIdx.x < 64) {
 #ifndef OCG_EMU
@@ -137,6 +138,21 @@
   c.load_tables(gf, gb, md);
   int i = blockIdx.x;
   if (i >= n) return;
+  if (fast_dh_on(P)) {
+    FastChain f(P, smem + P.fast_off, P.fplan, c.PROF);
+    __syncthreads();
+    f.init(P.fplan, gf, gb);
+    f.load(SLOT_D(pool, P, in[i]), SLOT_X(pool, P, in[i]));
+    const double b0 = 16.0 * f.compact_used();
+    f.apply_dH();
+    const double n2 = f.site_norm2(1);
+    f.store(SLOT_D(pool, P, outs[i]), SLOT_X(pool, P, outs[i]));
+    const double b = b0 + 16.0 * f.compact_used();
+    if (threadIdx.x == 0 && norms) norms[i] = sqrt(n2);
+    __syncthreads();
+    flush_stats(c, stats, b, 8.0 * b, 0.0);
+    return;
+  }
   c.load(SLOT_D(pool, P, in[i]), SLOT_X(pool, P, in[i]));
   const double b0 = 16.0 * c.mps_used();
   c.apply_dH();
@@ -221,8 +237,7 @@
     __hip_atomic_fetch_add(progress, 1, __ATOMIC_RELAXED, __HIP_MEMORY_SCOPE_AGENT);
   }
 }
-template <int NT>
-__device__ OCG_INLINE bool await_flag(Chain<NT>& c, const int* flag, int epoch, int* err, const int* progress) {
+__device__ inline OCG_INLINE bool await_flag_at(LDS int* word, const int* flag, int epoch, int* err, const int* progress) {
   if (threadIdx.x == 0) {
     int ok = 1;
     long spins = 0;
@@ -241,15 +256,19 @@
       }
     }
     __atomic_thread_fence(__ATOMIC_ACQUIRE);
-    c.ISCAL[15] = ok;
+    *word = ok;
   }
   __syncthreads();
-  const int ok = c.ISCAL[15];
+  const int ok = *word;
   __syncthreads();
   return ok != 0;
 }
-
-template <int NT>
+template <int NT>
+__device__ OCG_INLINE bool await_flag(Chain<NT>& c, const int* flag, int epoch, int* err, const int* progress) {
+  return await_flag_at(&c.ISCAL[15], flag, epoch, err, progress);
+}
+
+template <int NT, bool DH = false>
 __device__ OCG_INLINE void body_pipeline(char* smem, OcgParams P, const zc* gf, const zc* gb, const int* md,
                                          Pool pool, int slot_init, int slot_target, int psi_base0, int xi_base0,
                                          int xih_base0, const double* u0, int N, const int* rows, int nrows,
@@ -271,7 +290,7 @@
   c.load_tables(gf, gb, md);
   int* const progress = flags + 2 * N;
   double bytes = 0, flops = 0, nsteps = 0;
-  const bool fo = fast_on(P);
+  const bool fo = DH || fast_on(P), fd = DH || fast_dh_on(P);
   FastChain f(P, smem + P.fast_off, P.fplan, c.PROF);
   if (fo && b < 2) {
     __syncthreads();
@@ -287,8 +306,10 @@
     f.store(SLOT_D(pool, P, base + t), SLOT_X(pool, P, base + t), true);
     for (int s = 0; s + 1 < N; ++s) {
       const int tn = fwd ? t + 1 : t - 1;
-      f.step(u[t], u[tn], fwd, s + 2 == N);
-      publish_flag_wt(fl + t, epoch, progress);
+      const bool last = s + 2 == N;
+      if (last) publish_flag_wt(fl + t, epoch, progress);
+      f.step(u[t], u[tn], fwd, last);
+      if (!last) publish_flag_wt(fl + t, epoch, progress);
       f.store(SLOT_D(pool, P, base + tn), SLOT_X(pool, P, base + tn), true);
       t = tn;
     }
@@ -299,6 +320,42 @@
     flush_stats(c, stats, bytes, flops, nsteps);
     return;
   }
+  if (fd) {
+    __syncthreads();
+    f.init(P.fplan, gf, gb);
+    __syncthreads();
+    const bool row = b >= 2 + nxw;
+    const int r = b - 2 - nxw;
+    if (row && r >= nrows) return;
+    const int i = row ? rows[r] : 0;
+    for (int t = row ? i : N - 1 - (b - 2); t >= 0; t -= nxw) {
+      if (!await_flag_at(f.FLG, flags + (row ? 0 : N) + t, epoch, err, progress)) return;
+      const int src = (row ? psi_base : xi_base) + t;
+      f.load(SLOT_D(pool, P, src), SLOT_X(pool, P, src));
+      f.apply_dH();
+      if (row) break;
+      f.store(SLOT_D(pool, P, xih_base + t), SLOT_X(pool, P, xih_base + t));
+    }
+    if (row) {
+      const double n2 = f.site_norm2(1);
+      if (threadIdx.x == 0) rnorm0[(size_t)kc * nrows + r] = sqrt(n2);
+      int k = kc * rbase[nrows] + rbase[r];
+      f.store(SLOT_D(rs, P, k), SLOT_X(rs, P, k));
+      __syncthreads();
+      f.load(SLOT_D(rs, P, k), SLOT_X(rs, P, k));
+      for (int j = i + 1; j + 1 < N; ++j) {
+        f.step(u[j - 1], u[j], 1, false);
+        ++k;
+        f.store(SLOT_D(rs, P, k), SLOT_X(rs, P, k));
+      }
+      nsteps = N - 2 - i;
+    }
+    f.model_totals(bytes, flops);
+    __syncthreads();
+    flush_stats(c, stats, bytes, flops, nsteps);
+    return;
+  }
+  if constexpr (!DH) {
   if (b < 2) {
     const int fwd = (b == 0) ? 1 : 0;
     const int base = fwd ? psi_base : xi_base;
@@ -360,6 +417,7 @@
   double mb, mf;
   c.model_totals(mb, mf);
   flush_stats(c, stats, bytes + mb, flops + mf, nsteps);
+  }
 }
 
 template <int NT>
diff --git a/optimalcontrolmps_amd/csrc/ocmps.hip b/optimalcontrolmps_amd/csrc/ocmps.hip
--- a/optimalcontrolmps_amd/csrc/ocmps.hip
+++ b/optimalcontrolmps_amd/csrc/ocmps.hip
@@ -70,6 +70,15 @@
   extern __shared__ __align__(16) char smem[];
   ocg::body_pipeline<NT>(smem, P, gf, gb, md, pool, slot_init, slot_target, psi_base, xi_base, xih_base, u, N, rows,
                          nrows, rbase, rs, rnorm, flags, epoch, err, nxw, stats, K, cs);
+}
+__global__ __launch_bounds__(NT) void k_pipeline_dh(OcgParams P, const zc* gf, const zc* gb, const int* md, Pool pool,
+                                                    int slot_init, int slot_target, int psi_base, int xi_base,
+                                                    int xih_base, const double* u, int N, const int* rows, int nrows,
+                                                    const int* rbase, Pool rs, double* rnorm, int* flags, int epoch,
+                                                    int* err, int nxw, double* stats, int K, int cs) {
+  extern __shared__ __align__(16) char smem[];
+  ocg::body_pipeline<NT, true>(smem, P, gf, gb, md, pool, slot_init, slot_target, psi_base, xi_base, xih_base, u, N,
+                               rows, nrows, rbase, rs, rnorm, flags, epoch, err, nxw, stats, K, cs);
 }
 
 __global__ __launch_bounds__(NT) void k_row_overlaps(OcgParams P, const zc* gf, const zc* gb, const int* md,
@@ -186,6 +195,8 @@
     }
     return q;
   }
+  bool fast_dh = false;
+  OcgParams Pd() const { return fast_dh ? Pa() : Pn(); }
   OcgParams Pn() const {
     OcgParams q = P;
     q.fplan = nullptr;
@@ -445,6 +456,7 @@
   HIPCHK(c, hipFuncSetAttribute((const void*)k_hessian_rows, hipFuncAttributeMaxDynamicSharedMemorySize, bytes));
   HIPCHK(c, hipFuncSetAttribute((const void*)k_steps, hipFuncAttributeMaxDynamicSharedMemorySize, bytes));
   HIPCHK(c, hipFuncSetAttribute((const void*)k_pipeline, hipFuncAttributeMaxDynamicSharedMemorySize, bytes));
+  HIPCHK(c, hipFuncSetAttribute((const void*)k_pipeline_dh, hipFuncAttributeMaxDynamicSharedMemorySize, bytes));
   HIPCHK(c, hipFuncSetAttribute((const void*)k_row_overlaps, hipFuncAttributeMaxDynamicSharedMemorySize, bytes));
   HIPCHK(c, hipFuncSetAttribute((const void*)k_row_overlaps_w, hipFuncAttributeMaxDynamicSharedMemorySize, bytes));
   return 0;
@@ -495,6 +507,7 @@
                     "): configuration exceeds the single-workgroup engine (see DESIGN.md §Scope)");
   c->P.fplan = nullptr;
   c->P.fast_off = 0;
+  c->fast_dh = false;
   c->P.oplan = nullptr;
   c->P.ovl_bytes = 0;
   c->P.ovl_dh_bytes = 0;
@@ -509,7 +522,11 @@
     return 0;
   }
   const int off = (l.bytes + 255) & ~255;
-  const int fbytes = ocg_host::fast_lds_bytes(fb.plan, c->P);
+  int fbytes = ocg_host::fast_lds_bytes(fb.plan, c->P);
+  if (size_t(off + fbytes) > limit && fb.dh_why_not.empty()) {
+    fb = ocg_host::build_fast_plan(c->P, c->md, false);
+    fbytes = ocg_host::fast_lds_bytes(fb.plan, c->P);
+  }
   if (size_t(off + fbytes) > limit) {
     c->fast_why = "LDS";
     return 0;
@@ -520,6 +537,10 @@
   HIPCHK(c, hipStreamSynchronize(c->stream));
   c->P.fplan = c->d_fplan;
   c->P.fast_off = off;
+  c->fast_dh = fb.dh_why_not.empty();
+  if (std::getenv("OCG_FAST_DUMP"))
+    std::fprintf(stderr, "[fast plan] LDS general %d fast %d dH %s\n", l.bytes, fbytes,
+                 c->fast_dh ? "on" : fb.dh_why_not.c_str());
   c->P.nplan = 0;
   c->P.plan_pe = 0;
   c->P.lds_bytes = off + fbytes;
@@ -1029,7 +1050,7 @@
   idx.insert(idx.end(), outs.begin(), outs.end());
   HIPCHK(c, hipMemcpyAsync(c->d_idx, idx.data(), sizeof(int) * 2 * n, hipMemcpyHostToDevice, c->stream));
   if (int rc = begin_kernel(c)) return rc;
-  const OcgParams Pn = c->Pn();
+  const OcgParams Pn = c->Pd();
   hipLaunchKernelGGL(k_apply_dH, dim3(n), dim3(NT), Pn.lds_bytes, c->stream, Pn, c->d_gf, c->d_gb, c->d_md, c->pool,
                      c->d_idx, c->d_idx + n, n, norms ? c->d_norms : nullptr, c->d_stats + 2 * 3);
   if (int rc = end_kernel(c, 2)) return rc;
@@ -1275,7 +1296,7 @@
     in.insert(in.end(), outs.begin(), outs.end());
     HIPCHK(c, hipMemcpyAsync(c->d_idx2, in.data(), sizeof(int) * 2 * nrows, hipMemcpyHostToDevice, c->stream));
     if (int rc = begin_kernel(c)) return rc;
-    const OcgParams Pn = c->Pn();
+    const OcgParams Pn = c->Pd();
     hipLaunchKernelGGL(k_apply_dH, dim3(nrows), dim3(NT), Pn.lds_bytes, c->stream, Pn, c->d_gf, c->d_gb, c->d_md,
                        c->pool, c->d_idx2, c->d_idx2 + nrows, nrows, c->d_rnorm, c->d_stats + 2 * 3);
     if (int rc = end_kernel(c, 2)) return rc;
@@ -1487,7 +1508,8 @@
     return e ? std::atoi(e) : 8;
   }();
   const OcgParams Pl = (share_k > 0 && K >= share_k) ? c->P2() : c->Pa();
-  hipLaunchKernelGGL(k_pipeline, dim3(K * (2 + nxw + nrows)), dim3(NT), Pl.lds_bytes, c->stream, Pl, c->d_gf,
+  hipLaunchKernelGGL(c->fast_dh ? k_pipeline_dh : k_pipeline, dim3(K * (2 + nxw + nrows)), dim3(NT), Pl.lds_bytes,
+                     c->stream, Pl, c->d_gf,
                      c->d_gb, c->d_md, c->pool, c->slot_init(), c->slot_target(), c->psi_base(), c->xi_base(),
                      c->xih_base(), c->d_u, N, d_rows, nrows, d_rbase, c->rs, c->d_prn, c->d_flags, epoch, c->d_err,
                      nxw, c->d_stats + 5 * 3, K, cs);
```

Result: no change. 25650 (median of 6 runs) (+0.8%).
